# ekarpp/lumo

Measured on AMD Instinct MI355X. Metric: Mrays/s, higher is better.
Workload: dtype f64

## Files before the change

lumo_amd/csrc/device/dscene.h:

```cpp
#pragma once
#include <hip/hip_runtime.h>

#include "../../../include/lumo_amd.h"
#include "../common/lmath.h"
#include "../common/rng.h"
#include "../common/vec.h"
#include "../common/wbvh.h"

#ifndef LUMO_WHILE_WHILE
#define LUMO_WHILE_WHILE 1
#endif

namespace lumo {
namespace dev {

constexpr double DINF = __builtin_huge_val();
constexpr int NS = 4;
constexpr double Y_INTEGRAL = 106.856895;
constexpr double SVI = 253.819;

struct alignas(16) DKd {
    union {
        double point;
        struct {
            int32_t first, count;
        } leaf;
    } u;
    int32_t meta;
    int32_t left;
};
constexpr int TV_STRIDE = 10;

struct DBvh {
    double bmin[3], bmax[3];
    int32_t escape, first, count, left;
};

struct DObj {
    double bmin[3], bmax[3];
    int32_t kd_root, tri_base, item_base, tx;
    __device__ __forceinline__ int type() const { return tx & 3; }
    __device__ __forceinline__ int xform() const { return (tx >> 2) - 1; }
};
__device__ __forceinline__ double obj_radius(const DObj& o) { return o.bmin[0]; }
__device__ __forceinline__ double obj_radius(const lumo_object& o) { return o.radius; }

struct DScene {
    const double* vertices;
    const double* tv;
    const DKd* kdp;
    const double* normals;
    const double* uvs;
    const lumo_triangle* tris;
    const lumo_kd_node* kd;
    const int32_t* kd_items;
    const lumo_object* objs;
    const DObj* tobjs;
    const DBvh* onodes;
    const int32_t* oitems;
    const lumo_object* lights;
    const DObj* tlights;
    const DBvh* lnodes;
    const int32_t* litems;
    const double* alias_prob;
    const int32_t* alias_idx;
    const double* alias_pdf;
    const lumo_material* mats;
    const double* dense;
    const lumo_transform* xforms;
    const lumo_texture* textures;
    const lumo_spectrum* texels;
    const lumo_normal_map* nmaps;
    const double* ntexels;
    const lumo_perlin* perlin;
    int32_t n_onodes, n_lnodes, n_lights, n_shadow, stack_class, full, n_objs, pad_n;
    const char* hot;
    uint32_t hot_bytes;
    uint32_t off_onodes, off_oitems, off_lnodes, off_litems, off_objs, off_lights, off_kd_items, off_tris, off_xforms,
        off_tv, off_kdp, off_tobjs, off_tlights;
    const char* top;
    uint32_t top_bytes, off_top_onodes, off_top_lnodes, off_top_oitems, off_top_tobjs;
    int32_t top_onodes, top_lnodes;
    const DBvh* onodes_lds;
    const DBvh* lnodes_lds;
    int32_t n_onodes_lds, n_lnodes_lds;
    int32_t kst_n, kst_stride;
    int32_t* kst_node;
    double* kst_ts;
    int32_t kst_cfg;
    uint32_t top_shm;
    uint32_t off_top_kd;
    int32_t top_kd_lo, top_kd_n;
    const DKd* kd_lds;
    int32_t accel, w_oroot, w_lroot, wn_lds;
    double w_maxabs;
    const wbvh::Node* wnodes;
    const double* wtv;
    const int32_t* w_oblas;
    const int32_t* w_lblas;
    const wbvh::Node* wnodes_lds;
    uint32_t off_wnodes, off_wtv, off_woblas, off_wlblas;
    uint32_t off_top_wnodes;
    int32_t top_wnodes;
};

__device__ __forceinline__ DScene stage_top_lds(const DScene& sc, char* lds) {
    const uint4* src = reinterpret_cast<const uint4*>(sc.top);
    uint4* dst = reinterpret_cast<uint4*>(lds);
    for (uint32_t i = threadIdx.x; i < sc.top_bytes / 16; i += blockDim.x) dst[i] = src[i];
    __syncthreads();
    DScene v = sc;
    v.onodes_lds = reinterpret_cast<const DBvh*>(lds + sc.off_top_onodes);
    v.lnodes_lds = reinterpret_cast<const DBvh*>(lds + sc.off_top_lnodes);
    v.n_onodes_lds = sc.top_onodes;
    v.n_lnodes_lds = sc.top_lnodes;
    v.oitems = reinterpret_cast<const int32_t*>(lds + sc.off_top_oitems);
    v.tobjs = reinterpret_cast<const DObj*>(lds + sc.off_top_tobjs);
    v.kd_lds = reinterpret_cast<const DKd*>(lds + sc.off_top_kd);
    v.wnodes_lds = reinterpret_cast<const wbvh::Node*>(lds + sc.off_top_wnodes);
    v.wn_lds = sc.top_wnodes;
    v.kst_n = sc.kst_cfg;
    if (sc.kst_cfg > 0) {
        char* base = lds + ((sc.top_bytes + 15u) & ~15u);
        v.kst_stride = (int32_t)blockDim.x;
        v.kst_ts = reinterpret_cast<double*>(base) + threadIdx.x;
        v.kst_node = reinterpret_cast<int32_t*>(base + (size_t)8 * sc.kst_cfg * blockDim.x) + threadIdx.x;
    }
    return v;
}

__device__ __forceinline__ DScene stage_scene_lds(const DScene& sc, char* lds) {
    const uint4* src = reinterpret_cast<const uint4*>(sc.hot);
    uint4* dst = reinterpret_cast<uint4*>(lds);
    for (uint32_t i = threadIdx.x; i < sc.hot_bytes / 16; i += blockDim.x) dst[i] = src[i];
    __syncthreads();
    DScene v = sc;
    v.onodes = reinterpret_cast<const DBvh*>(lds + sc.off_onodes);
    v.oitems = reinterpret_cast<const int32_t*>(lds + sc.off_oitems);
    v.lnodes = reinterpret_cast<const DBvh*>(lds + sc.off_lnodes);
    v.litems = reinterpret_cast<const int32_t*>(lds + sc.off_litems);
    v.objs = reinterpret_cast<const lumo_object*>(lds + sc.off_objs);
    v.lights = reinterpret_cast<const lumo_object*>(lds + sc.off_lights);
    v.kd_items = reinterpret_cast<const int32_t*>(lds + sc.off_kd_items);
    v.tris = reinterpret_cast<const lumo_triangle*>(lds + sc.off_tris);
    v.xforms = reinterpret_cast<const lumo_transform*>(lds + sc.off_xforms);
    v.tv = reinterpret_cast<const double*>(lds + sc.off_tv);
    v.kdp = reinterpret_cast<const DKd*>(lds + sc.off_kdp);
    v.tobjs = reinterpret_cast<const DObj*>(lds + sc.off_tobjs);
    v.tlights = reinterpret_cast<const DObj*>(lds + sc.off_tlights);
    if (sc.accel) {
        v.wnodes = reinterpret_cast<const wbvh::Node*>(lds + sc.off_wnodes);
        v.wtv = reinterpret_cast<const double*>(lds + sc.off_wtv);
        v.w_oblas = reinterpret_cast<const int32_t*>(lds + sc.off_woblas);
        v.w_lblas = reinterpret_cast<const int32_t*>(lds + sc.off_wlblas);
    }
    return v;
}

struct Counters {
    uint32_t aabb, kd, tri;
    uint32_t resolved;
};

struct Ray {
    V3 o, d;
};
__device__ __forceinline__ Ray ray_new(V3 o, V3 d) { return Ray{o, normalize(d)}; }

struct RayX {
    V3 o, d, inv, wi, shear;
    int kz;
};
__device__ __forceinline__ V3 perm_kz(int kz, V3 v) {
    return kz == 0 ? V3{v.y, v.z, v.x} : (kz == 1 ? V3{v.z, v.x, v.y} : v);
}
__device__ __forceinline__ RayX rayx(const Ray& r) {
    RayX x;
    x.o = r.o;
    x.d = r.d;
    x.inv = 1.0 / r.d;
    const V3 wa = vabs(r.d);
    x.kz = (wa.x > wa.y && wa.x > wa.z) ? 0 : (wa.y > wa.z ? 1 : 2);
    x.wi = perm_kz(x.kz, r.d);
    x.shear = V3{-x.wi.x, -x.wi.y, 0.0} / x.wi.z;
    return x;
}

struct DColor {
    double s[NS];
};
__device__ __forceinline__ DColor cfill(double v) { return DColor{{v, v, v, v}}; }
__device__ __forceinline__ DColor operator+(DColor a, const DColor& b) {
#pragma unroll
    for (int i = 0; i < NS; ++i) a.s[i] = a.s[i] + b.s[i];
    return a;
}
__device__ __forceinline__ DColor operator-(DColor a, const DColor& b) {
#pragma unroll
    for (int i = 0; i < NS; ++i) a.s[i] = a.s[i] - b.s[i];
    return a;
}
__device__ __forceinline__ DColor operator*(DColor a, const DColor& b) {
#pragma unroll
    for (int i = 0; i < NS; ++i) a.s[i] = a.s[i] * b.s[i];
    return a;
}
__device__ __forceinline__ DColor operator*(DColor a, double v) {
#pragma unroll
    for (int i = 0; i < NS; ++i) a.s[i] = a.s[i] * v;
    return a;
}
__device__ __forceinline__ DColor operator*(double v, DColor a) {
#pragma unroll
    for (int i = 0; i < NS; ++i) a.s[i] = v * a.s[i];
    return a;
}
__device__ __forceinline__ DColor operator/(DColor a, const DColor& b) {
#pragma unroll
    for (int i = 0; i < NS; ++i) a.s[i] = b.s[i] == 0.0 ? 0.0 : a.s[i] / b.s[i];
    return a;
}
__device__ __forceinline__ DColor operator/(DColor a, double v) {
#pragma unroll
    for (int i = 0; i < NS; ++i) a.s[i] = v == 0.0 ? 0.0 : a.s[i] / v;
    return a;
}
__device__ __forceinline__ double cmean(const DColor& c) {
    double sum = 0.0;
#pragma unroll
    for (int i = 0; i < NS; ++i) sum += c.s[i];
    return sum / NS;
}

__device__ __forceinline__ double wl_sample_one(double v) {
    const double x = 0.85691062 - SVI * v * 0.0072;
    return 538.0 - 138.888889 * (0.5 * lm_log1p((2.0 * x) / (1.0 - x)));
}
__device__ __forceinline__ void wl_sample(double u, double* L) {
#pragma unroll
    for (int i = 0; i < NS; ++i) {
        double v = u + (double)i / (double)NS;
        v = v > 1.0 ? v - 1.0 : v;
        L[i] = wl_sample_one(v);
    }
}
__device__ __forceinline__ double wl_pdf_one(double l) {
    if (l < 360.0 || l > 830.0) return 0.0;
    const double c = lm_cosh(0.0072 * (l - 538.05));
    return 1.0 / (SVI * (c * c));
}
__device__ __forceinline__ DColor wl_pdf(const double* L) {
    DColor c;
#pragma unroll
    for (int i = 0; i < NS; ++i) c.s[i] = wl_pdf_one(L[i]);
    if (L[1] == 0.0 && L[2] == 0.0 && L[3] == 0.0) c.s[0] /= (double)NS;
    return c;
}
__device__ __forceinline__ double dense_one(const double* v, double lambda) {
    const double STEP = (830.0 - 360.0) / (95.0 - 1.0);
    const double fb = ceil((lambda - 360.0) / STEP);
    int b1 = fb > 0.0 ? (int)fmin(fb, 1e9) : 0;
    const double l1 = 360.0 + STEP * (double)b1;
    if (lambda == 0.0) return 0.0;
    if (b1 > 94) b1 = 94;
    if (lambda == l1) return v[b1];
    const int b0 = b1 == 0 ? 0 : b1 - 1;
    const double l0 = l1 - STEP;
    const double x1 = (lambda - l0) / STEP;
    const double x0 = 1.0 - x1;
    return v[b0] * x0 + v[b1] * x1;
}
__device__ __forceinline__ DColor dense_sample(const double* v, const double* L) {
    DColor c;
#pragma unroll
    for (int i = 0; i < NS; ++i) c.s[i] = dense_one(v, L[i]);
    return c;
}
__device__ __forceinline__ double spec_one(const lumo_spectrum& s, double lambda) {
    const float l = (float)lambda;
    const float x = s.c0 * l * l + s.c1 * l + s.c2;
    const float sig = 0.5f + x / (2.0f * sqrtf(1.0f + x * x));
    return (double)(s.scale * sig);
}
__device__ __forceinline__ DColor spec_sample(const lumo_spectrum& s, const double* L) {
    DColor c;
#pragma unroll
    for (int i = 0; i < NS; ++i) c.s[i] = spec_one(s, L[i]);
    return c;
}
__device__ __forceinline__ double luminance(const DScene& sc, const DColor& c, const double* L) {
    const DColor pdf = wl_pdf(L);
    return cmean(dense_sample(sc.dense + 95 * 1, L) * c / pdf) / Y_INTEGRAL;
}
__device__ __forceinline__ void dense_three(const double* v, double lambda, double* out) {
    const double STEP = (830.0 - 360.0) / (95.0 - 1.0);
    const double fb = ceil((lambda - 360.0) / STEP);
    int b1 = fb > 0.0 ? (int)fmin(fb, 1e9) : 0;
    const double l1 = 360.0 + STEP * (double)b1;
    if (lambda == 0.0) {
        out[0] = out[1] = out[2] = 0.0;
        return;
    }
    if (b1 > 94) b1 = 94;
    if (lambda == l1) {
        for (int k = 0; k < 3; ++k) out[k] = v[95 * k + b1];
        return;
    }
    const int b0 = b1 == 0 ? 0 : b1 - 1;
    const double l0 = l1 - STEP;
    const double x1 = (lambda - l0) / STEP;
    const double x0 = 1.0 - x1;
    for (int k = 0; k < 3; ++k) out[k] = v[95 * k + b0] * x0 + v[95 * k + b1] * x1;
}
__device__ __forceinline__ V3 color_xyz(const DScene& sc, const DColor& c, const double* L) {
    const DColor pdf = wl_pdf(L);
    DColor cx, cy, cz;
#pragma unroll
    for (int i = 0; i < NS; ++i) {
        double o[3];
        dense_three(sc.dense, L[i], o);
        cx.s[i] = o[0];
        cy.s[i] = o[1];
        cz.s[i] = o[2];
    }
    return V3{cmean(cx * c / pdf), cmean(cy * c / pdf), cmean(cz * c / pdf)} / Y_INTEGRAL;
}

__device__ __forceinline__ uint32_t sat_u32(double x) { return x != x || x <= 0.0 ? 0u : (x >= 4294967295.0 ? 4294967295u : (uint32_t)x); }
__device__ __forceinline__ uint64_t sat_u64(double x) {
    return x != x || x <= 0.0 ? 0ull : (x >= 18446744073709551615.0 ? ~0ull : (uint64_t)x);
}
struct Bilin {
    uint32_t i00, i10, i01, i11;
    double wx, wy;
};
__device__ __forceinline__ Bilin bilin(int32_t width, int32_t height, V2 uv) {
    const double w = (double)width, h = (double)height;
    const V2 xy{uv.x * w, (1.0 - uv.y) * h};
    const V2 xoyo{floor(xy.x - 0.5), floor(xy.y - 0.5)};
    const V2 x1y1{xy.x - xoyo.x - 0.5, xy.y - xoyo.y - 0.5};
    const uint32_t W = (uint32_t)width, H = (uint32_t)height;
    const uint32_t xo = sat_u32(xoyo.x + w) % W, yo = sat_u32(xoyo.y + h) % H;
    const uint32_t xi = (xo + 1) % W, yi = (yo + 1) % H;
    return Bilin{xo + yo * W, xi + yo * W, xo + yi * W, xi + yi * W, 1.0 - x1y1.x, 1.0 - x1y1.y};
}
__device__ __forceinline__ DColor image_at(const DScene& sc, const lumo_texture& T, V2 uv, const double* L) {
    const Bilin b = bilin(T.width, T.height, uv);
    const lumo_spectrum* tx = sc.texels + T.first;
    const DColor y0 = spec_sample(tx[b.i00], L) * b.wx + spec_sample(tx[b.i10], L) * (1.0 - b.wx);
    const DColor y1 = spec_sample(tx[b.i01], L) * b.wx + spec_sample(tx[b.i11], L) * (1.0 - b.wx);
    return y0 * b.wy + y1 * (1.0 - b.wy);
}
__device__ __forceinline__ V3 vfract(V3 v) { return V3{v.x - trunc(v.x), v.y - trunc(v.y), v.z - trunc(v.z)}; }
__device__ double perlin_noise(const lumo_perlin& P, V3 p) {
    const V3 w0 = vfract(p);
    const V3 fl{floor(p.x), floor(p.y), floor(p.z)};
    auto smoother = [](double x) { return ((6.0 * x - 15.0) * x + 10.0) * x * x * x; };
    const V3 w{smoother(w0.x), smoother(w0.y), smoother(w0.z)};
    const uint64_t bx = sat_u64(fl.x), by = sat_u64(fl.y), bz = sat_u64(fl.z);
    double acc = 0.0;
    for (int c = 0; c < 8; ++c) {
        const int i = c >> 2, j = (c >> 1) & 1, k = c & 1;
        const int hsh = P.perm[0][(bx + i) % 256] ^ P.perm[1][(by + j) % 256] ^ P.perm[2][(bz + k) % 256];
        const V3 nrm{P.lattice[hsh][0], P.lattice[hsh][1], P.lattice[hsh][2]};
        const V3 idx{(double)i, (double)j, (double)k};
        const V3 widx{2.0 * w.x * idx.x + 1.0 - w.x - idx.x, 2.0 * w.y * idx.y + 1.0 - w.y - idx.y,
                      2.0 * w.z * idx.z + 1.0 - w.z - idx.z};
        acc = acc + widx.x * widx.y * widx.z * dot(nrm, w - idx);
    }
    return acc;
}
__device__ __forceinline__ double powi6(double x) {
    const double x2 = x * x;
    return x2 * (x2 * x2);
}
__device__ DColor tex_at(const DScene& sc, int tex, const lumo_spectrum& solid, V2 uv, const double* L) {
    if (tex < 0) return spec_sample(solid, L);
    for (;;) {
        const lumo_texture& T = sc.textures[tex];
        if (T.kind == LUMO_TEX_SOLID) return spec_sample(T.spec, L);
        if (T.kind == LUMO_TEX_IMAGE) return image_at(sc, T, uv, L);
        if (T.kind == LUMO_TEX_CHECKERBOARD) {
            const V2 uvs{uv.x * T.scale, uv.y * T.scale};
            tex = sat_u64(floor(uvs.x) + floor(uvs.y)) % 2 == 0 ? T.first : T.second;
            continue;
        }
        if (T.kind == LUMO_TEX_MARBLE) {
            const lumo_perlin& P = sc.perlin[T.first];
            V3 p = 4.0 * V3{fabs(uv.x), fabs(uv.y), 0.0};
            double turb = 0.0;
            double gain = 1.0;
            for (int d = 0; d < 6; ++d) {
                turb = turb + gain * fabs(perlin_noise(P, p));
                p = 2.0 * p;
                gain = gain * 0.5;
            }
            const double scaled = 1.0 - powi6(0.5 + 0.5 * lm_sin(60.0 * uv.x + 20.0 * turb));
            return spec_sample(T.spec, L) * scaled;
        }
        const double cr = 2.0 * (uv.x - 0.75), ci = 2.0 * (uv.y - 0.5);
        double zr = 0.0, zi = 0.0;
        int depth = 0;
        while (depth < 256 && zr * zr + zi * zi < 4096.0) {
            const double nr = zr * zr - zi * zi + cr;
            const double ni = zr * zi + zi * zr + ci;
            zr = nr;
            zi = ni;
            depth++;
        }
        return cfill(depth == 256 ? 1.0 : 0.0);
    }
}
__device__ __forceinline__ V3 nmap_at(const DScene& sc, const lumo_normal_map& M, V2 uv) {
    const Bilin b = bilin(M.width, M.height, uv);
    const double* t = sc.ntexels + 3 * (size_t)M.first;
    auto n = [&](uint32_t i) { return V3{t[3 * i], t[3 * i + 1], t[3 * i + 2]}; };
    auto lerp = [](V3 n0, V3 n1, double v) { return normalize(n0 * v + n1 * (1.0 - v)); };
    return lerp(lerp(n(b.i00), n(b.i10), b.wx), lerp(n(b.i01), n(b.i11), b.wx), b.wy);
}

struct DHit {
    double t;
    int material;
    V3 p, err, ns, ng;
    V2 uv;
    bool backface;
};
__device__ __forceinline__ V2 wrap_uv(V2 uv) {
    const V2 f{rfract(uv.x), rfract(uv.y)};
    return V2{f.x < 0.0 ? f.x + 1.0 : f.x, f.y < 0.0 ? f.y + 1.0 : f.y};
}
__device__ __forceinline__ V3 ray_origin(const DHit& h, bool outside) {
    const V3 ne = h.ng;
    const double scaled_err = dot(h.err, vabs(ne));
    const V3 offset = outside ? ne * scaled_err : (-ne) * scaled_err;
    const V3 xi = h.p + offset;
    auto mv = [](double v, double n) { return n > 0.0 ? next_float(v) : (n < 0.0 ? previous_float(v) : v); };
    return V3{mv(xi.x, offset.x), mv(xi.y, offset.y), mv(xi.z, offset.z)};
}
__device__ __forceinline__ Ray spawn(const DHit& h, V3 wi) { return ray_new(ray_origin(h, dot(wi, h.ng) >= 0.0), wi); }

__device__ __forceinline__ V3 ld3(const double* p) { return V3{p[0], p[1], p[2]}; }

__device__ __forceinline__ void slab(const double* bmin, const double* bmax, V3 o, V3 inv, double& ts, double& te) {
    const V3 ro_min = (ld3(bmin) - o) * inv;
    const V3 ro_max = (ld3(bmax) - o) * inv;
    ts = max_element(vmin(ro_min, ro_max));
    te = min_element(vmax(ro_max, ro_min)) * (1.0 + 2.0 * gamma_n(3));
}

__device__ __forceinline__ double tri_hit_t_at(const double* tv, const RayX& r, double t_min, double t_max,
                                               Counters& C) {
    C.tri++;
    const V3 A = ld3(tv), B = ld3(tv + 3), Cv = ld3(tv + 6);
    const int kz = r.kz;
    const V3 wi = r.wi;
    V3 at = perm_kz(kz, A - r.o), bt = perm_kz(kz, B - r.o), ct = perm_kz(kz, Cv - r.o);
    const V3 shear = r.shear;
    at = at + shear * at.z;
    bt = bt + shear * bt.z;
    ct = ct + shear * ct.z;
    const V3 e = V3{bt.x * ct.y - bt.y * ct.x, ct.x * at.y - ct.y * at.x, at.x * bt.y - at.y * bt.x};
    if (min_element(e) < 0.0 && max_element(e) > 0.0) return DINF;
    const double det = dot(e, V3{1.0, 1.0, 1.0});
    if (det == 0.0) return DINF;
    const double t_scaled = dot(e, V3{at.z, bt.z, ct.z}) / wi.z;
    const bool b1 = det < 0.0 && (t_scaled > t_min * det || t_scaled < t_max * det);
    const bool b2 = det > 0.0 && (t_scaled < t_min * det || t_scaled > t_max * det);
    if (b1 || b2) return DINF;
    return t_scaled / det;
}
__device__ __forceinline__ double tri_hit_t(const DScene& sc, int ti, const RayX& r, double t_min, double t_max,
                                            Counters& C) {
    return tri_hit_t_at(sc.tv + TV_STRIDE * ti, r, t_min, t_max, C);
}

template <bool FULL>
__device__ bool tri_hit_geo_at(const DScene& sc, const double* tv, int ti, const RayX& r, double t_min, double t_max,
                               DHit& out) {
    const V3 A = ld3(tv), B = ld3(tv + 3), Cv = ld3(tv + 6);
    const int kz = r.kz;
    const V3 wi = r.wi;
    V3 at = perm_kz(kz, A - r.o), bt = perm_kz(kz, B - r.o), ct = perm_kz(kz, Cv - r.o);
    const V3 shear = r.shear;
    at = at + shear * at.z;
    bt = bt + shear * bt.z;
    ct = ct + shear * ct.z;
    const V3 e = V3{bt.x * ct.y - bt.y * ct.x, ct.x * at.y - ct.y * at.x, at.x * bt.y - at.y * bt.x};
    if (min_element(e) < 0.0 && max_element(e) > 0.0) return false;
    const double det = dot(e, V3{1.0, 1.0, 1.0});
    if (det == 0.0) return false;
    const double t_scaled = dot(e, V3{at.z, bt.z, ct.z}) / wi.z;
    const bool b1 = det < 0.0 && (t_scaled > t_min * det || t_scaled < t_max * det);
    const bool b2 = det > 0.0 && (t_scaled < t_min * det || t_scaled > t_max * det);
    if (b1 || b2) return false;
    const double t = t_scaled / det;
    const double max_z_v = rmax(rmax(fabs(at.z), fabs(bt.z)), fabs(ct.z));
    const double delta_z = gamma_n(3) * max_z_v;
    const double max_y_v = rmax(rmax(fabs(at.y), fabs(bt.y)), fabs(ct.y));
    const double delta_y = gamma_n(5) * (max_y_v + max_z_v);
    const double max_x_v = rmax(rmax(fabs(at.x), fabs(bt.x)), fabs(ct.x));
    const double delta_x = gamma_n(5) * (max_x_v + max_z_v);
    const double delta_e = 2.0 * (gamma_n(2) * max_x_v * max_y_v + delta_y * max_x_v + delta_x * max_y_v);
    const double max_e = rmax(rmax(fabs(e.x), fabs(e.y)), fabs(e.z));
    const double delta_t = 3.0 * (gamma_n(3) * max_e * max_z_v + delta_e * max_z_v + delta_z * max_e) / fabs(det);
    if (t <= t_min + delta_t) return false;
    out.t = t;
    if (!FULL) return true;
    const V3 bary = e / det;
    const lumo_triangle T = sc.tris[ti];
    const V3 ng = normalize(cross(B - A, Cv - A));
    V3 ns = ng;
    if (T.n[0] >= 0)
        ns = normalize(bary.x * ld3(sc.normals + 3 * T.n[0]) + bary.y * ld3(sc.normals + 3 * T.n[1]) +
                       bary.z * ld3(sc.normals + 3 * T.n[2]));
    const V3 xi = bary.x * A + bary.y * B + bary.z * Cv;
    V2 ta{0, 0}, tb{1, 0}, tc{1, 1};
    if (T.t[0] >= 0) {
        ta = V2{sc.uvs[2 * T.t[0]], sc.uvs[2 * T.t[0] + 1]};
        tb = V2{sc.uvs[2 * T.t[1]], sc.uvs[2 * T.t[1] + 1]};
        tc = V2{sc.uvs[2 * T.t[2]], sc.uvs[2 * T.t[2] + 1]};
    }
    const V2 uv = bary.x * ta + bary.y * tb + bary.z * tc;
    out.err = gamma_n(7) * V3{dot(vabs(bary * V3{A.x, B.x, Cv.x}), V3{1, 1, 1}),
                              dot(vabs(bary * V3{A.y, B.y, Cv.y}), V3{1, 1, 1}),
                              dot(vabs(bary * V3{A.z, B.z, Cv.z}), V3{1, 1, 1})};
    out.t = t;
    out.material = T.material;
    out.backface = dot(r.d, ng) > 0.0;
    out.p = xi;
    out.ns = ns;
    out.ng = ng;
    out.uv = wrap_uv(uv);
    return true;
}
template <bool FULL>
__device__ __forceinline__ bool tri_hit_geo(const DScene& sc, int ti, const RayX& r, double t_min, double t_max,
                                            DHit& out) {
    return tri_hit_geo_at<FULL>(sc, sc.tv + TV_STRIDE * ti, ti, r, t_min, t_max, out);
}

#ifdef LUMO_NOINLINE_KD
#define KD_INLINE __noinline__
#else
#define KD_INLINE
#endif
template <bool KL>
__device__ __forceinline__ void kst_push(const DScene& sc, int* st_node, double* st_ts, int k, int node, double t) {
    if (KL && k < sc.kst_n) {
        sc.kst_node[k * sc.kst_stride] = node;
        sc.kst_ts[k * sc.kst_stride] = t;
    } else {
        st_node[k] = node;
        st_ts[k] = t;
    }
}
template <bool KL>
__device__ __forceinline__ int kst_node(const DScene& sc, const int* st_node, int k) {
    return (KL && k < sc.kst_n) ? sc.kst_node[k * sc.kst_stride] : st_node[k];
}
template <bool KL>
__device__ __forceinline__ double kst_t(const DScene& sc, const double* st_ts, int k) {
    return (KL && k < sc.kst_n) ? sc.kst_ts[k * sc.kst_stride] : st_ts[k];
}

template <bool KL>
__device__ __forceinline__ DKd kd_at(const DScene& sc, int i) {
    if (KL) {
        const uint32_t k = (uint32_t)(i - sc.top_kd_lo);
        if (k < (uint32_t)sc.top_kd_n) return sc.kd_lds[k];
    }
    return sc.kdp[i];
}

template <bool GEO, int STK, bool KL = false>
__device__ KD_INLINE double kd_traverse(const DScene& sc, const DObj& ob, const RayX& r, double t_min, double t_max,
                              int* idx_out, Counters& C) {
    const double origin[3] = {r.o.x, r.o.y, r.o.z};
    const double inv_dir[3] = {r.inv.x, r.inv.y, r.inv.z};
    int st_node[STK];
    double st_ts[STK];
    int sp = 0;
    double t_hit = DINF;
    int curr = ob.kd_root;
    int idx = -1;
    double ts, te;
    C.aabb++;
    slab(ob.bmin, ob.bmax, r.o, r.inv, ts, te);
    double t_start = rmax(ts, t_min), t_end = rmin(te, t_max);
    const double t_end0 = t_end;
    for (;;) {
        if (t_hit < t_start) break;
        DKd node = kd_at<KL>(sc, curr);
#if LUMO_WHILE_WHILE
        while ((node.meta & 3) != 3) {
            C.kd++;
            const int ax = node.meta & 3;
            const double point = node.u.point;
            const int right = node.meta >> 2;
            const double t_split = (point - origin[ax]) * inv_dir[ax];
            const bool left_first = origin[ax] < point || (origin[ax] == point && inv_dir[ax] <= 0.0);
            const int first = left_first ? node.left : right;
            const int second = left_first ? right : node.left;
            if (t_split > t_end || t_split <= 0.0) {
                curr = first;
            } else if (t_split < t_start) {
                curr = second;
            } else {
                curr = first;
                kst_push<KL>(sc, st_node, st_ts, sp, second, t_split);
                t_end = t_split;
                sp++;
            }
            node = kd_at<KL>(sc, curr);
        }
#endif
        const int axis = node.meta & 3;
        if (axis == 3) {
            const int first = node.u.leaf.first, count = node.u.leaf.count;
            for (int k = 0; k < count; ++k) {
                const int i = sc.kd_items[ob.item_base + first + k];
                const double t = tri_hit_t(sc, ob.tri_base + i, r, t_min, t_end, C);
                if (GEO) {
                    if (t < t_end) {
                        t_end = t;
                        t_hit = t;
                        idx = i;
                    }
                } else if (t < t_end) {
                    return t;
                }
            }
            if (sp == 0) break;
            sp--;
            curr = kst_node<KL>(sc, st_node, sp);
            t_start = kst_t<KL>(sc, st_ts, sp);
            t_end = sp == 0 ? t_end0 : kst_t<KL>(sc, st_ts, sp - 1);
        } else {
            C.kd++;
            const int ax = axis;
            const double point = node.u.point;
            const int right = node.meta >> 2;
            const double t_split = (point - origin[ax]) * inv_dir[ax];
            const bool left_first = origin[ax] < point || (origin[ax] == point && inv_dir[ax] <= 0.0);
            const int first = left_first ? node.left : right;
            const int second = left_first ? right : node.left;
            if (t_split > t_end || t_split <= 0.0) {
                curr = first;
            } else if (t_split < t_start) {
                curr = second;
            } else {
                curr = first;
                kst_push<KL>(sc, st_node, st_ts, sp, second, t_split);
                t_end = t_split;
                sp++;
            }
        }
    }
    if (GEO) {
        *idx_out = idx;
        return idx < 0 ? DINF : t_hit;
    }
    return DINF;
}

__device__ __forceinline__ V3 xrow3(const double* m, int r, V3 v) { return V3{m[4 * r], m[4 * r + 1], m[4 * r + 2]}; }
__device__ __forceinline__ V3 xf_apply(const double* m, V3 v, double w) {
    const V4 in{v.x, v.y, v.z, w};
    const V4 o{dot4(V4{m[0], m[1], m[2], m[3]}, in), dot4(V4{m[4], m[5], m[6], m[7]}, in),
               dot4(V4{m[8], m[9], m[10], m[11]}, in), dot4(V4{m[12], m[13], m[14], m[15]}, in)};
    return project(o);
}
__device__ __forceinline__ V3 xf_abs_apply(const double* m, V3 v, double w) {
    const V4 in{v.x, v.y, v.z, w};
    auto r = [&](int i) { return V4{fabs(m[4 * i]), fabs(m[4 * i + 1]), fabs(m[4 * i + 2]), fabs(m[4 * i + 3])}; };
    return project(V4{dot4(r(0), in), dot4(r(1), in), dot4(r(2), in), dot4(r(3), in)});
}
__device__ __forceinline__ V3 m3_apply(const double* n, V3 v) {
    return V3{dot(V3{n[0], n[1], n[2]}, v), dot(V3{n[3], n[4], n[5]}, v), dot(V3{n[6], n[7], n[8]}, v)};
}
__device__ __forceinline__ RayX ray_local(const lumo_transform& T, const RayX& r) {
    return rayx(Ray{xf_apply(T.inv, r.o, 1.0), xf_apply(T.inv, r.d, 0.0)});
}
__device__ void instance_fix_hit(const lumo_transform& T, int material_override, DHit& h) {
    h.ns = normalize(m3_apply(T.nrm, h.ns));
    h.ng = normalize(m3_apply(T.nrm, h.ng));
    const V3 e3 = vabs(h.err), p3 = vabs(h.p);
    V3 err = gamma_n(3) * xf_abs_apply(T.m, p3, 1.0);
    if (!(e3.x == 0.0 && e3.y == 0.0 && e3.z == 0.0))
        err = err + (gamma_n(3) + 1.0) * xf_abs_apply(T.m, e3, 0.0);
    h.err = err;
    if (material_override >= 0) h.material = material_override;
    h.p = xf_apply(T.m, h.p, 1.0);
}

struct EF {
    double v, lo, hi;
};
__device__ __forceinline__ EF ef(double x) { return EF{x, x, x}; }
__device__ __forceinline__ EF ef_add(EF a, EF b) { return EF{a.v + b.v, previous_float(a.lo + b.lo), next_float(a.hi + b.hi)}; }
__device__ __forceinline__ EF ef_sub(EF a, EF b) { return EF{a.v - b.v, previous_float(a.lo - b.hi), next_float(a.hi - b.lo)}; }
__device__ __forceinline__ EF ef_mul(EF a, EF b) {
    const double p0 = a.lo * b.lo, p1 = a.lo * b.hi, p2 = a.hi * b.lo, p3 = a.hi * b.hi;
    return EF{a.v * b.v, previous_float(rmin(rmin(rmin(p0, p1), p2), p3)), next_float(rmax(rmax(rmax(p0, p1), p2), p3))};
}
__device__ __forceinline__ EF ef_div(EF a, EF b) {
    if (b.lo < 0.0 && b.hi > 0.0) return EF{a.v / b.v, -DINF, DINF};
    const double d0 = a.lo / b.lo, d1 = a.lo / b.hi, d2 = a.hi / b.lo, d3 = a.hi / b.hi;
    return EF{a.v / b.v, previous_float(rmin(rmin(rmin(d0, d1), d2), d3)), next_float(rmax(rmax(rmax(d0, d1), d2), d3))};
}
template <bool FULL, class OB>
__device__ bool sphere_hit(const OB& ob, const RayX& r, double t_min, double t_max, DHit& out) {
    const double radius = obj_radius(ob);
    const EF dx = ef(r.d.x), dy = ef(r.d.y), dz = ef(r.d.z), ox = ef(r.o.x), oy = ef(r.o.y), oz = ef(r.o.z);
    const EF radius2 = ef_mul(ef(radius), ef(radius));
    const EF a = ef_add(ef_add(ef_mul(dx, dx), ef_mul(dy, dy)), ef_mul(dz, dz));
    const EF b = ef_mul(ef(2.0), ef_add(ef_add(ef_mul(dx, ox), ef_mul(dy, oy)), ef_mul(dz, oz)));
    const EF c = ef_sub(ef_add(ef_add(ef_mul(ox, ox), ef_mul(oy, oy)), ef_mul(oz, oz)), radius2);
    const double disc = b.v * b.v - 4.0 * a.v * c.v;
    if (disc < 0.0) return false;
    const double sd = sqrt(disc);
    const EF root{sd, previous_float(sqrt(disc)), next_float(sqrt(disc))};
    const EF nb{-b.v, -b.lo, -b.hi};
    const EF a2 = ef_mul(ef(2.0), a);
    EF t0 = ef_div(ef_sub(nb, root), a2), t1 = ef_div(ef_add(nb, root), a2);
    if (t0.v > t1.v) {
        const EF tmp = t0;
        t0 = t1;
        t1 = tmp;
    }
    if (t0.hi >= t_max || t1.lo <= t_min) return false;
    EF t = t0;
    if (!(t0.lo > t_min)) {
        if (t1.hi >= t_max) return false;
        t = t1;
    }
    out.t = t.v;
    if constexpr (!FULL) {
        return true;
    } else {
    V3 xi = r.o + t.v * r.d;
    xi = xi * radius / length(xi);
    const V3 ni = xi / radius;
    out.err = gamma_n(5) * vabs(xi);
    out.material = ob.material;
    out.backface = dot(r.d, ni) > 0.0;
    out.p = xi;
    out.ns = ni;
    out.ng = ni;
    out.uv = wrap_uv(V2{(lm_atan2(-ni.z, ni.x) + PI) / (2.0 * PI), lm_acos(-ni.y) / PI});
    return true;
    }
}
__device__ double sphere_hit_t(const DObj& ob, const RayX& r, double t_min, double t_max) {
    const double a = dot(r.d, r.d);
    const double b = 2.0 * dot(r.d, r.o);
    const double radius = obj_radius(ob);
    const double c = dot(r.o, r.o) - radius * radius;
    const double disc = b * b - 4.0 * a * c;
    if (disc < 0.0) return DINF;
    const double root = sqrt(disc);
    double t0 = (-b - root) / (2.0 * a), t1 = (-b + root) / (2.0 * a);
    if (t0 > t1) {
        const double tmp = t0;
        t0 = t1;
        t1 = tmp;
    }
    if (t0 >= t_max || t1 <= t_min) return DINF;
    if (t0 > t_min) return t0;
    if (t1 >= t_max) return DINF;
    return t1;
}
constexpr int PRIM_SPHERE = -2;

template <int STK, int FX, bool KL = false>
__device__ __forceinline__ double shape_hit_t(const DScene& sc, const DObj& ob, const RayX& r, double t_min,
                                              double t_max, Counters& C) {
    if constexpr (FX) {
        if (ob.type() == LUMO_OBJ_TRIANGLE) return tri_hit_t(sc, ob.tri_base, r, t_min, t_max, C);
        if (ob.type() == LUMO_OBJ_SPHERE) return sphere_hit_t(ob, r, t_min, t_max);
    }
    return kd_traverse<false, STK, KL>(sc, ob, r, t_min, t_max, nullptr, C);
}
template <int STK, int FX, bool KL = false>
__device__ __forceinline__ double object_hit_t(const DScene& sc, const DObj& ob, const RayX& r, double t_min,
                                               double t_max, Counters& C) {
    if constexpr (FX) {
        if (ob.xform() >= 0)
            return shape_hit_t<STK, FX, KL>(sc, ob, ray_local(sc.xforms[ob.xform()], r), t_min, t_max, C);
    }
    return shape_hit_t<STK, FX, KL>(sc, ob, r, t_min, t_max, C);
}

template <int STK, int FX, bool KL = false>
__device__ __forceinline__ int shape_hit_tri(const DScene& sc, const DObj& ob, const RayX& r, double t_min,
                                             double t_max, Counters& C, DHit& out) {
    if constexpr (FX) {
        if (ob.type() == LUMO_OBJ_TRIANGLE) {
            C.tri++;
            return tri_hit_geo<false>(sc, ob.tri_base, r, t_min, t_max, out) ? ob.tri_base : -1;
        }
        if (ob.type() == LUMO_OBJ_SPHERE) return sphere_hit<false>(ob, r, t_min, t_max, out) ? PRIM_SPHERE : -1;
    }
    int idx = -1;
    kd_traverse<true, STK, KL>(sc, ob, r, t_min, t_max, &idx, C);
    if (idx < 0) return -1;
    C.tri++;
    if (!tri_hit_geo<false>(sc, ob.tri_base + idx, r, t_min, t_max, out)) return -1;
    return ob.tri_base + idx;
}
template <int STK, int FX, bool KL = false>
__device__ __forceinline__ int object_hit_tri(const DScene& sc, const DObj& ob, const RayX& r, double t_min,
                                              double t_max, Counters& C, DHit& out) {
    if constexpr (FX) {
        if (ob.xform() >= 0)
            return shape_hit_tri<STK, FX, KL>(sc, ob, ray_local(sc.xforms[ob.xform()], r), t_min, t_max, C, out);
    }
    return shape_hit_tri<STK, FX, KL>(sc, ob, r, t_min, t_max, C, out);
}

template <int FX>
__device__ void object_record(const DScene& sc, const lumo_object& ob, int tri, const RayX& r, DHit& h) {
    if constexpr (!FX) {
        tri_hit_geo<true>(sc, tri, r, 0.0, DINF, h);
        if (ob.type == LUMO_OBJ_RECTANGLE) h.uv = wrap_uv(V2{dot(ld3(ob.b0), h.p), dot(ld3(ob.b1), h.p)});
    } else {
        const RayX rl = ob.xform < 0 ? r : ray_local(sc.xforms[ob.xform], r);
        if (ob.type == LUMO_OBJ_SPHERE)
            sphere_hit<true>(ob, rl, 0.0, DINF, h);
        else
            tri_hit_geo<true>(sc, tri, rl, 0.0, DINF, h);
        if (ob.type == LUMO_OBJ_RECTANGLE) h.uv = wrap_uv(V2{dot(ld3(ob.b0), h.p), dot(ld3(ob.b1), h.p)});
        if (ob.xform >= 0) instance_fix_hit(sc.xforms[ob.xform], ob.material_override, h);
    }
}

template <bool GEO, int STK, int FX, bool TOP = false>
__device__ int bvh_traverse(const DScene& sc, const DBvh* nodes, int n_nodes, const int32_t* items,
                            const DObj* objs, const RayX& r, double t_min, double t_max, Counters& C,
                            double* t_found = nullptr, const DBvh* nodes_lds = nullptr, int n_lds = 0) {
    if (n_nodes == 0) return -1;
    const V3 inv_dir = r.inv;
    int curr = 0, idx = -1;
    double tt = t_max;
#if LUMO_WHILE_WHILE
    for (;;) {
        int count = 0;
        while (curr >= 0) {
            const DBvh& node = (TOP && curr < n_lds) ? nodes_lds[curr] : nodes[curr];
            double ts, te;
            C.aabb++;
            slab(node.bmin, node.bmax, r.o, inv_dir, ts, te);
            ts = rmax(ts, t_min);
            te = rmin(te, tt);
            if (ts <= te) {
                count = node.count;
                if (count == 0) {
                    curr = node.left;
                    continue;
                }
                break;
            }
            curr = node.escape;
        }
        if (curr < 0) break;
        const DBvh& node = (TOP && curr < n_lds) ? nodes_lds[curr] : nodes[curr];
        {
#else
    while (curr >= 0) {
        const DBvh& node = (TOP && curr < n_lds) ? nodes_lds[curr] : nodes[curr];
        double ts, te;
        C.aabb++;
        slab(node.bmin, node.bmax, r.o, inv_dir, ts, te);
        ts = rmax(ts, t_min);
        te = rmin(te, tt);
        if (ts <= te) {
            const int count = node.count;
            if (count == 0) {
                curr = node.left;
                continue;
            }
#endif
            for (int k = 0; k < count; ++k) {
                const int i = items[node.first + k];
                const double t = object_hit_t<STK, FX, TOP>(sc, objs[i], r, t_min, tt, C);
                if (GEO) {
                    if (t < tt) {
                        tt = t;
                        idx = i;
                    }
                } else if (t < tt) {
                    if (t_found) *t_found = t;
                    return i;
                }
            }
        }
        curr = node.escape;
    }
    return idx;
}

template <int STK, int FX, bool TOP = false>
__device__ __forceinline__ double bvh_hit_t(const DScene& sc, const DBvh* nodes, int n, const int32_t* items,
                                            const DObj* objs, const RayX& r, double t_min, double t_max,
                                            Counters& C, const DBvh* nodes_lds = nullptr, int n_lds = 0) {
    double t = DINF;
    const int idx = bvh_traverse<false, STK, FX, TOP>(sc, nodes, n, items, objs, r, t_min, t_max, C, &t, nodes_lds, n_lds);
    if (idx < 0) return DINF;
    return t;
}

struct HitRef {
    double t;
    int kind, obj, tri;
};

constexpr int WL_STK = wbvh::LIGHT_KD_STACK;
template <int STK>
constexpr int kd_stk() {
    return STK == 0 ? WL_STK : STK;
}

struct WHit {
    double t;
    int32_t tri, obj;
};

typedef __attribute__((address_space(1))) const uint4 g_uint4;
typedef __attribute__((address_space(3))) const uint4 l_uint4;
template <bool TOP>
__device__ __forceinline__ void wnode_load(const DScene& sc, int32_t i, wbvh::Node& nd) {
    uint4 v[8];
#if defined(__HIP_DEVICE_COMPILE__)
    if constexpr (TOP) {
        if (i < sc.wn_lds) {
            extern __shared__ __attribute__((aligned(16))) char lds_scene[];
            l_uint4* p = (l_uint4*)(lds_scene + sc.off_top_wnodes) + 8 * i;
#pragma unroll
            for (int k = 0; k < 8; ++k) v[k] = p[k];
        } else {
            g_uint4* p = (g_uint4*)sc.wnodes + 8 * (size_t)i;
#pragma unroll
            for (int k = 0; k < 8; ++k) v[k] = p[k];
        }
    } else
#endif
    {
        const uint4* p = reinterpret_cast<const uint4*>(sc.wnodes) + 8 * (size_t)i;
#pragma unroll
        for (int k = 0; k < 8; ++k) v[k] = p[k];
    }
    __builtin_memcpy(&nd, v, sizeof(nd));
}

struct RayW {
    float inv[3], clo[3], chi[3];
};
__device__ __forceinline__ float f32_up(double x) {
    const float f = (float)x;
    return (double)f < x ? nextafterf(f, __builtin_huge_valf()) : f;
}
__device__ __forceinline__ float f32_down(double x) {
    const float f = (float)x;
    return (double)f > x ? nextafterf(f, -__builtin_huge_valf()) : f;
}
__device__ __forceinline__ RayW rayw(const RayX& r, double M) {
    RayW w;
    const double o[3] = {r.o.x, r.o.y, r.o.z}, inv[3] = {r.inv.x, r.inv.y, r.inv.z};
#pragma unroll
    for (int a = 0; a < 3; ++a) {
        const double e = (M + fabs(o[a])) * fabs(inv[a]);
        if (e <= 1e36) {
            w.inv[a] = (float)inv[a];
            const double c = -(o[a] * inv[a]), E = e * 0x1p-23;
            const float lo = f32_down(c - E), hi = f32_up(c + E);
            w.clo[a] = inv[a] >= 0.0 ? lo : hi;
            w.chi[a] = inv[a] >= 0.0 ? hi : lo;
        } else {
            w.inv[a] = 0.0f;
            w.clo[a] = -__builtin_huge_valf();
            w.chi[a] = __builtin_huge_valf();
        }
    }
    return w;
}
constexpr float WREL_LO = 1.0f - 0x1p-21f, WREL_HI = 1.0f + 0x1p-21f;
#ifndef LUMO_WIDE_ANY_SORT
#define LUMO_WIDE_ANY_SORT 0
#endif
__device__ __forceinline__ bool wslab32(const wbvh::Node& nd, int i, const RayW& w, float tmin, float tmax, float& k) {
    float ts, te;
#pragma unroll
    for (int a = 0; a < 3; ++a) {
        const float t0 = fmaf(nd.lo[a][i], w.inv[a], w.clo[a]);
        const float t1 = fmaf(nd.hi[a][i], w.inv[a], w.chi[a]);
        const float lo = fminf(t0, t1), hi = fmaxf(t0, t1);
        ts = a == 0 ? lo : fmaxf(ts, lo);
        te = a == 0 ? hi : fminf(te, hi);
    }
    k = fmaxf(ts * WREL_LO, tmin);
    return k <= fminf(te * WREL_HI, tmax);
}

template <bool BY_T = true>
__device__ __forceinline__ void wcx(float& ka, int32_t& ra, bool& ha, float& kb, int32_t& rb, bool& hb) {
    const bool sw = hb && (!ha || (BY_T && ka > kb));
    const float k = sw ? kb : ka;
    kb = sw ? ka : kb;
    ka = k;
    const int32_t x = sw ? rb : ra;
    rb = sw ? ra : rb;
    ra = x;
    const bool f = sw ? hb : ha;
    hb = sw ? ha : hb;
    ha = f;
}

template <class OB>
__device__ __forceinline__ double wide_sphere_t(const OB& ob, const lumo_transform* xforms, RayX rw, double t_min,
                                                double t_max) {
    const RayX rl = ob.xform() >= 0 ? ray_local(xforms[ob.xform()], rw) : rw;
    DHit g;
    return sphere_hit<false>(ob, rl, t_min, t_max, g) ? g.t : DINF;
}
template <class OB>
__device__ __noinline__ double wide_sphere_t_call(const OB& ob, const lumo_transform* xforms, RayX rw, double t_min,
                                                  double t_max) {
    return wide_sphere_t(ob, xforms, rw, t_min, t_max);
}
__device__ __noinline__ RayX wide_inst_ray_call(const lumo_transform* xforms, int x, RayX rw) {
    return ray_local(xforms[x], rw);
}

#ifndef LUMO_WIDE_NOINLINE
#define LUMO_WIDE_NOINLINE 0
#endif
#if LUMO_WIDE_NOINLINE
#define WIDE_INLINE __noinline__
#else
#define WIDE_INLINE
#endif
template <bool ANY, int FX, bool TOP, bool OC = false>
__device__ WIDE_INLINE WHit wide_walk(const DScene& sc, int32_t root, const DObj* objs, const int32_t* blas,
                                      const RayX& rw, double t_min, double t_max, Counters& C,
                                      double t_stop = -DINF) {
    WHit h{t_max, -1, -1};
    if (root == wbvh::NONE) return h;
    int32_t st_ref[wbvh::STACK];
    float st_t[wbvh::STACK];
    int sp = 0;
    bool top_ok = false;
    int32_t top_ref = 0;
    float top_t = 0.0f;
    auto push = [&](int32_t ref, float t) {
        if (top_ok) {
            st_ref[sp] = top_ref;
            st_t[sp] = top_t;
            sp++;
        }
        top_ok = true;
        top_ref = ref;
        top_t = t;
    };
    RayX r = rw;
    const double wM = sc.w_maxabs;
    RayW w = rayw(rw, wM);
    const float tmin32 = f32_down(t_min);
    float tmax32 = f32_up(t_max);
    int inst = -1;
    int32_t cur = root;
    auto pop = [&]() -> bool {
        for (;;) {
            int32_t x;
            float xt;
            if (top_ok) {
                top_ok = false;
                x = top_ref;
                xt = top_t;
            } else {
                if (sp == 0) return false;
                --sp;
                x = st_ref[sp];
                xt = st_t[sp];
            }
            if (FX && x == wbvh::MARK) {
                r = rw;
                w = rayw(rw, wM);
                inst = -1;
                continue;
            }
            if (!ANY && (double)xt > h.t) continue;
            cur = x;
            return true;
        }
    };
    for (;;) {
        while (cur >= 0) {
            wbvh::Node nd;
            wnode_load<TOP>(sc, cur, nd);
            C.kd++;
            const int n = nd.n;
            C.aabb += n;
            float k0, k1, k2, k3;
            bool h0 = wslab32(nd, 0, w, tmin32, tmax32, k0);
            bool h1 = wslab32(nd, 1, w, tmin32, tmax32, k1);
            bool h2 = wslab32(nd, 2, w, tmin32, tmax32, k2) && n > 2;
            bool h3 = wslab32(nd, 3, w, tmin32, tmax32, k3) && n > 3;
            int32_t r0 = nd.ref[0], r1 = nd.ref[1], r2 = nd.ref[2], r3 = nd.ref[3];
            if (!ANY || LUMO_WIDE_ANY_SORT) {
                wcx(k0, r0, h0, k1, r1, h1);
                wcx(k2, r2, h2, k3, r3, h3);
                wcx(k0, r0, h0, k2, r2, h2);
                wcx(k1, r1, h1, k3, r3, h3);
                wcx(k1, r1, h1, k2, r2, h2);
            } else {
                wcx<false>(k0, r0, h0, k1, r1, h1);
                wcx<false>(k2, r2, h2, k3, r3, h3);
                wcx<false>(k0, r0, h0, k2, r2, h2);
                wcx<false>(k1, r1, h1, k3, r3, h3);
                wcx<false>(k1, r1, h1, k2, r2, h2);
            }
            if (!h0) {
                if (!pop()) return h;
                continue;
            }
            if (h3) push(r3, k3);
            if (h2) push(r2, k2);
            if (h1) push(r1, k1);
            cur = r0;
        }
        const int cnt = wbvh::leaf_count(cur), first = wbvh::leaf_first(cur);
        if (FX && cnt == 0) {
            const DObj& ob = objs[first];
            if (ob.type() == LUMO_OBJ_SPHERE) {
                const double gt = OC ? wide_sphere_t_call(ob, sc.xforms, rw, t_min, h.t)
                                     : wide_sphere_t(ob, sc.xforms, rw, t_min, h.t);
                if (gt < h.t) {
                    h = WHit{gt, PRIM_SPHERE, first};
                    if (ANY || h.t < t_stop) return h;
                    tmax32 = f32_up(h.t);
                }
            } else {
                push(wbvh::MARK, -__builtin_huge_valf());
                r = OC ? wide_inst_ray_call(sc.xforms, ob.xform(), rw) : ray_local(sc.xforms[ob.xform()], rw);
                w = rayw(r, wM);
                inst = first;
                cur = blas[first];
                continue;
            }
        } else {
            for (int k = 0; k < cnt; ++k) {
                const double* tv = sc.wtv + wbvh::TV * (size_t)(first + k);
                C.tri++;
                DHit g;
                if (tri_hit_geo_at<false>(sc, tv, -1, r, t_min, h.t, g) && g.t < h.t) {
                    const int32_t* ids = reinterpret_cast<const int32_t*>(tv + 9);
                    h = WHit{g.t, ids[0], inst >= 0 ? inst : ids[1]};
                    if (ANY || h.t < t_stop) return h;
                    tmax32 = f32_up(h.t);
                }
            }
        }
        if (!pop()) return h;
    }
}

template <int FX, bool TOP, bool OC = false>
__device__ HitRef wide_scene_hit(const DScene& sc, const RayX& r, Counters& C) {
    HitRef h{DINF, 0, -1, -1};
    const WHit o = wide_walk<false, FX, TOP, OC>(sc, sc.w_oroot, sc.tobjs, sc.w_oblas, r, 0.0, DINF, C);
    if (o.obj >= 0) h = HitRef{o.t, 1, o.obj, o.tri};
    const WHit l = wide_walk<false, FX, TOP, OC>(sc, sc.w_lroot, sc.tlights, sc.w_lblas, r, 0.0, h.t, C);
    if (l.obj >= 0) h = HitRef{l.t, 2, l.obj, l.tri};
    return h;
}

template <int FX, bool TOP, bool OC = false>
__device__ __forceinline__ bool wide_occluded(const DScene& sc, const RayX& r, double t_max, Counters& C) {
    if (wide_walk<true, FX, TOP, OC>(sc, sc.w_oroot, sc.tobjs, sc.w_oblas, r, 0.0, t_max, C).t < t_max) return true;
    return wide_walk<true, FX, TOP, OC>(sc, sc.w_lroot, sc.tlights, sc.w_lblas, r, 0.0, t_max, C).t < t_max;
}
template <int STK, int FX, bool TOP = false, bool OC = false>
__device__ HitRef scene_hit(const DScene& sc, const RayX& r, Counters& C) {
    if constexpr (STK == 0) {
        return wide_scene_hit<FX, TOP, OC>(sc, r, C);
    } else {
    HitRef h{DINF, 0, -1, -1};
    double t_max = DINF;
    DHit g;
    int oi = bvh_traverse<true, STK, FX, TOP>(sc, sc.onodes, sc.n_onodes, sc.oitems, sc.tobjs, r, 0.0, t_max, C, nullptr,
                                              sc.onodes_lds, sc.n_onodes_lds);
    if (oi >= 0) {
        const int tri = object_hit_tri<STK, FX, TOP>(sc, sc.tobjs[oi], r, 0.0, t_max, C, g);
        if (tri != -1) {
            h = HitRef{g.t, 1, oi, tri};
            t_max = g.t;
        }
    }
    const int li = bvh_traverse<true, STK, FX, TOP>(sc, sc.lnodes, sc.n_lnodes, sc.litems, sc.tlights, r, 0.0, t_max, C,
                                                    nullptr, sc.lnodes_lds, sc.n_lnodes_lds);
    if (li >= 0) {
        const int tri = object_hit_tri<STK, FX, TOP>(sc, sc.tlights[li], r, 0.0, t_max, C, g);
        if (tri != -1) h = HitRef{g.t, 2, li, tri};
    }
    return h;
    }
}

template <int FX>
__device__ __forceinline__ void hit_record(const DScene& sc, const HitRef& hr, const RayX& r, DHit& h) {
    const lumo_object& ob = hr.kind == 1 ? sc.objs[hr.obj] : sc.lights[hr.obj];
    object_record<FX>(sc, ob, hr.tri, r, h);
}

template <int STK, int FX, bool TOP = false>
__device__ bool scene_hit_light(const DScene& sc, const RayX& r, int light, DHit& lh, Counters& C) {
    if constexpr (STK == 0) {
        const int tri = object_hit_tri<kd_stk<STK>(), FX, false>(sc, sc.tlights[light], r, 0.0, DINF, C, lh);
        if (tri == -1 || wide_occluded<FX, TOP>(sc, r, lh.t - EPSILON, C)) return false;
        object_record<FX>(sc, sc.lights[light], tri, r, lh);
        return true;
    } else {
    const int tri = object_hit_tri<STK, FX, TOP>(sc, sc.tlights[light], r, 0.0, DINF, C, lh);
    if (tri == -1) return false;
    const double t_max = lh.t - EPSILON;
    if (bvh_hit_t<STK, FX, TOP>(sc, sc.onodes, sc.n_onodes, sc.oitems, sc.tobjs, r, 0.0, t_max, C, sc.onodes_lds,
                                sc.n_onodes_lds) < t_max)
        return false;
    if (bvh_hit_t<STK, FX, TOP>(sc, sc.lnodes, sc.n_lnodes, sc.litems, sc.tlights, r, 0.0, t_max, C, sc.lnodes_lds,
                                sc.n_lnodes_lds) < t_max)
        return false;
    object_record<FX>(sc, sc.lights[light], tri, r, lh);
    return true;
    }
}

template <int STK, int FX, bool TOP = false, bool OC = false>
__device__ int scene_hit_light_tri(const DScene& sc, const RayX& r, int light, Counters& C) {
    DHit lh;
    if constexpr (STK == 0) {
        const int tri = object_hit_tri<kd_stk<STK>(), FX, false>(sc, sc.tlights[light], r, 0.0, DINF, C, lh);
        if (tri == -1 || wide_occluded<FX, TOP, OC>(sc, r, lh.t - EPSILON, C)) return -1;
        return tri;
    } else {
    const int tri = object_hit_tri<STK, FX, TOP>(sc, sc.tlights[light], r, 0.0, DINF, C, lh);
    if (tri == -1) return -1;
    const double t_max = lh.t - EPSILON;
    if (bvh_hit_t<STK, FX, TOP>(sc, sc.onodes, sc.n_onodes, sc.oitems, sc.tobjs, r, 0.0, t_max, C, sc.onodes_lds,
                                sc.n_onodes_lds) < t_max)
        return -1;
    if (bvh_hit_t<STK, FX, TOP>(sc, sc.lnodes, sc.n_lnodes, sc.litems, sc.tlights, r, 0.0, t_max, C, sc.lnodes_lds,
                                sc.n_lnodes_lds) < t_max)
        return -1;
    return tri;
    }
}

struct Onb {
    V3 u, v, w;
};
__device__ __forceinline__ Onb onb_new(V3 w) {
    const double sgn = rsignum(w.z);
    const double a = -1.0 / (sgn + w.z);
    const double b = w.x * w.y * a;
    return Onb{V3{1.0 + sgn * w.x * w.x * a, sgn * b, -sgn * w.x}, V3{b, sgn + w.y * w.y * a, -w.y}, w};
}
__device__ __forceinline__ V3 onb_world(const Onb& o, V3 v) { return v.x * o.u + v.y * o.v + v.z * o.w; }
__device__ __forceinline__ V3 onb_local(const Onb& o, V3 v) { return V3{dot(v, o.u), dot(v, o.v), dot(v, o.w)}; }

struct Mf {
    double a;
    const double* eta;
    const double* k;
};
__device__ __forceinline__ Mf mf_of(const DScene& sc, const lumo_material& m) {
    return Mf{m.roughness, sc.dense + 95 * m.eta_idx, sc.dense + 95 * m.k_idx};
}
__device__ __forceinline__ bool mf_delta(const Mf& d) { return (d.a + d.a) / 2.0 < 1e-3; }
__device__ __forceinline__ bool mf_specular(const Mf& d) { return (d.a + d.a) / 2.0 < 0.01; }
__device__ __forceinline__ double sq(double x) { return x * x; }
__device__ __forceinline__ double pow5(double x) {
    const double x2 = x * x;
    const double x4 = x2 * x2;
    return x * x4;
}
__device__ __forceinline__ double clampd(double x, double lo, double hi) {
    if (x < lo) x = lo;
    if (x > hi) x = hi;
    return x;
}
__device__ __forceinline__ double schlick(double f0, double f90, double c) { return f0 + (f90 - f0) * pow5(1.0 - c); }
__device__ __forceinline__ void cs_phi(V3 w, double& cp, double& sp) {
    const double st = sqrt(rmax(1.0 - w.z * w.z, 0.0));
    cp = st == 0.0 ? 1.0 : clampd(w.x / st, -1.0, 1.0);
    sp = st == 0.0 ? 0.0 : clampd(w.y / st, -1.0, 1.0);
}
__device__ __forceinline__ double tan2_theta(V3 w) { return rmax(1.0 - w.z * w.z, 0.0) / (w.z * w.z); }
__device__ __forceinline__ bool is_inf(double x) { return x == DINF || x == -DINF; }
__device__ double mf_D(const Mf& d, V3 wh) {
    const double tan2 = tan2_theta(wh);
    if (is_inf(tan2)) return 0.0;
    const double cos4 = sq(wh.z * wh.z);
    if (cos4 < EPSILON * EPSILON) return 0.0;
    double cp, sp;
    cs_phi(wh, cp, sp);
    const double e = tan2 * (sq(cp / d.a) + sq(sp / d.a));
    return 1.0 / (PI * (d.a * d.a) * cos4 * sq(1.0 + e));
}
__device__ double mf_Lambda(const Mf& d, V3 w) {
    const double tan2 = tan2_theta(w);
    if (is_inf(tan2)) return 0.0;
    double cp, sp;
    cs_phi(w, cp, sp);
    const double alpha2 = sq(d.a * cp) + sq(d.a * sp);
    return (sqrt(rmax(1.0 + alpha2 * tan2, 0.0)) - 1.0) / 2.0;
}
__device__ __forceinline__ bool chi(V3 wo, V3 wh) { return rsignum(wh.z) * dot(wo, wh) * wo.z > EPSILON; }
__device__ __forceinline__ double mf_G(const Mf& d, V3 wo, V3 wi, V3 wh) {
    return chi(wo, wh) ? 1.0 / (1.0 + mf_Lambda(d, wo) + mf_Lambda(d, wi)) : 0.0;
}
__device__ __forceinline__ double mf_G1(const Mf& d, V3 wo, V3 wh) {
    return chi(wo, wh) ? 1.0 / (1.0 + mf_Lambda(d, wo)) : 0.0;
}
__device__ __forceinline__ double mf_normal_pdf(const Mf& d, V3 wh, V3 wo) {
    return rmax(mf_G1(d, wo, wh) * mf_D(d, wh) * fabs(dot(wh, wo)) / fabs(wo.z), 0.0);
}
__device__ V3 mf_sample_normal(const Mf& d, V3 wo, V2 u) {
    V3 ws = normalize(V3{wo.x * d.a, wo.y * d.a, wo.z});
    if (ws.z < 0.0) ws = -ws;
    const V3 t1 = (1.0 - ws.z < EPSILON) ? V3{1.0, 0.0, 0.0} : normalize(cross(ws, V3{0.0, 0.0, 1.0}));
    const V3 t2 = cross(t1, ws);
    const double r = sqrt(u.x);
    const double theta = 2.0 * PI * u.y;
    const double x = r * lm_cos(theta);
    const double h = sqrt(rmax(1.0 - x * x, 0.0));
    const double lerp = (1.0 + ws.z) / 2.0;
    const double y = (1.0 - lerp) * h + lerp * r * lm_sin(theta);
    const V3 wm{x, y, sqrt(rmax(1.0 - x * x - y * y, 0.0))};
    const V3 w = wm.x * t1 + wm.y * t2 + wm.z * ws;
    return normalize(V3{d.a * w.x, d.a * w.y, rmax(w.z, EPSILON)});
}
__device__ double fresnel_real(V3 wo, V3 wh, double eta) {
    double c = dot(wo, wh);
    const double e = c < 0.0 ? 1.0 / eta : eta;
    c = fabs(c);
    const double sin2_i = (1.0 - c * c) / (e * e);
    if (sin2_i >= 1.0) return 1.0;
    const double ci = sqrt(rmax(1.0 - sin2_i, 0.0));
    const double rpa = (e * c - ci) / (e * c + ci);
    const double rpe = (c - e * ci) / (c + e * ci);
    return (rpa * rpa + rpe * rpe) / 2.0;
}
struct Cx {
    double re, im;
};
__device__ __forceinline__ Cx cmul(Cx a, Cx b) { return Cx{a.re * b.re - a.im * b.im, a.re * b.im + a.im * b.re}; }
__device__ __forceinline__ double cnorm2(Cx a) { return a.re * a.re + a.im * a.im; }
__device__ __forceinline__ Cx cdivf(Cx a, double v) { return v == 0.0 ? Cx{NAN, NAN} : Cx{a.re / v, a.im / v}; }
__device__ __forceinline__ Cx cdiv(Cx a, Cx b) {
    if (b.re == 0.0 && b.im == 0.0) return Cx{NAN, NAN};
    return cdivf(cmul(a, Cx{b.re, -b.im}), cnorm2(b));
}
__device__ double fresnel_complex(V3 wo, V3 wh, double n, double k) {
    const Cx eta{n, k};
    const double c = clampd(dot(wo, wh), 0.0, 1.0);
    const double sin2_o = 1.0 - c * c;
    const Cx e2 = cmul(eta, eta);
    const Cx sin2_i = (e2.re == 0.0 && e2.im == 0.0)
                          ? Cx{NAN, NAN}
                          : cdivf(Cx{sin2_o * e2.re, sin2_o * -e2.im}, cnorm2(e2));
    const Cx z{1.0 - sin2_i.re, -sin2_i.im};
    const double rn = sqrt(sqrt(cnorm2(z)));
    const double half = lm_atan2(z.im, z.re) / 2.0;
    const Cx ci{rn * lm_cos(half), rn * lm_sin(half)};
    const Cx ec{eta.re * c, eta.im * c};
    const Cx rpa = cdiv(Cx{ec.re - ci.re, ec.im - ci.im}, Cx{ec.re + ci.re, ec.im + ci.im});
    const Cx eci = cmul(eta, ci);
    const Cx rpe = cdiv(Cx{c - eci.re, -eci.im}, Cx{c + eci.re, eci.im});
    return (cnorm2(rpa) + cnorm2(rpe)) / 2.0;
}
__device__ double fresnel_at(const Mf& d, V3 wo, V3 wh, double wl) {
    const double eta = dense_one(d.eta, wl);
    const double k = dense_one(d.k, wl);
    if (k == 0.0) return eta == 0.0 ? 0.0 : fresnel_real(wo, wh, eta);
    return fresnel_complex(wo, wh, eta, k);
}
__device__ __forceinline__ DColor fresnel(const Mf& d, V3 wo, V3 wh, const double* L) {
    DColor c;
    for (int i = 0; i < NS; ++i) c.s[i] = fresnel_at(d, wo, wh, L[i]);
    return c;
}
__device__ __forceinline__ bool reflect_about(V3 wo, V3 n, V3& wi) {
    const V3 w = 2.0 * (n * dot(wo, n) / length_squared(n)) - wo;
    if (!(w.z * wo.z > 0.0)) return false;
    wi = w;
    return true;
}
__device__ __forceinline__ bool refract_about(double eta, V3 wo, V3 no, V3& wi) {
    const bool flip = dot(no, wo) < 0.0;
    const double cos_to = flip ? -dot(no, wo) : dot(no, wo);
    const double er = flip ? 1.0 / eta : eta;
    const V3 n = flip ? -no : no;
    const double sin2_ti = (1.0 - cos_to * cos_to) / (er * er);
    if (sin2_ti >= 1.0) return false;
    const double cos_ti = sqrt(rmax(1.0 - sin2_ti, 0.0));
    const V3 w = -wo / er + (cos_to / er - cos_ti) * n;
    if (w.z * wo.z > 0.0) return false;
    wi = w;
    return true;
}
__device__ DColor reflect_coeff(const Mf& d, V3 wo, V3 wi, const double* L) {
    const V3 wh = normalize(wi + wo);
    return mf_D(d, wh) * fresnel(d, wo, wh, L) * mf_G(d, wo, wi, wh) / (4.0 * fabs(wo.z) * fabs(wi.z));
}
__device__ __forceinline__ double cos_hemisphere_pdf(V3 wo, V3 wi) {
    if (!(wo.z * wi.z > 0.0)) return 0.0;
    return wi.z > 0.0 ? wi.z / PI : 0.0;
}
__device__ __forceinline__ bool standard_kind(int k) {
    return k == LUMO_MAT_LAMBERTIAN || k == LUMO_MAT_MF_DIFFUSE || k == LUMO_MAT_MF_CONDUCTOR ||
           k == LUMO_MAT_MF_DIELECTRIC;
}

template <int FX>
__device__ __forceinline__ V3 mapped_ns(const DScene& sc, const lumo_material& m, const DHit& h) {
    if constexpr (FX >= 2) {
        if (m.normal_map >= 0) return normalize(onb_world(onb_new(h.ns), nmap_at(sc, sc.nmaps[m.normal_map], h.uv)));
    }
    return h.ns;
}
template <int FX>
__device__ __forceinline__ DColor mat_kd(const DScene& sc, const lumo_material& m, V2 uv, const double* L) {
    if constexpr (FX >= 2) return tex_at(sc, m.albedo_tex, m.albedo, uv, L);
    return spec_sample(m.albedo, L);
}
template <int FX>
__device__ __forceinline__ DColor mat_ks(const DScene& sc, const lumo_material& m, V2 uv, const double* L) {
    if constexpr (FX >= 2) return tex_at(sc, m.ks_tex, m.ks, uv, L);
    return spec_sample(m.ks, L);
}
template <int FX>
__device__ __forceinline__ DColor mat_tf(const DScene& sc, const lumo_material& m, V2 uv, const double* L) {
    if constexpr (FX >= 2) return tex_at(sc, m.tf_tex, m.tf, uv, L);
    return spec_sample(m.tf, L);
}

template <int FX>
__device__ bool bsdf_sample(const DScene& sc, const lumo_material& m, const DHit& h, V3 wo, double* L,
                            double rand_u, V2 rs, V3& wi) {
    if constexpr (!FX) {
        if (m.kind != LUMO_MAT_LAMBERTIAN || h.backface) return false;
        wi = onb_world(onb_new(h.ns), square_to_cos_hemisphere(rs));
        return true;
    }
    if (!standard_kind(m.kind)) return false;
    const Onb uvw = onb_new(mapped_ns<FX>(sc, m, h));
    const V3 o = onb_local(uvw, wo);
    if (h.backface && m.kind != LUMO_MAT_MF_DIELECTRIC) return false;
    V3 w;
    if (m.kind == LUMO_MAT_LAMBERTIAN) {
        w = square_to_cos_hemisphere(rs);
    } else {
        const Mf d = mf_of(sc, m);
        if (m.kind == LUMO_MAT_MF_DIFFUSE) {
            const double pr = schlick(0.04, 1.0, o.z);
            const double ps = 1.0 - pr;
            if (rand_u < pr / (pr + ps)) {
                if (!reflect_about(o, mf_delta(d) ? V3{0.0, 0.0, 1.0} : mf_sample_normal(d, o, rs), w)) return false;
            } else {
                w = square_to_cos_hemisphere(rs);
            }
        } else if (m.kind == LUMO_MAT_MF_CONDUCTOR) {
            if (mf_delta(d)) {
                w = V3{-o.x, -o.y, o.z};
            } else if (!reflect_about(o, mf_sample_normal(d, o, rs), w)) {
                return false;
            }
        } else {
            if (!(m.flags & LUMO_MATF_CONSTANT_ETA)) {
                L[1] = 0.0;
                L[2] = 0.0;
                L[3] = 0.0;
            }
            const double wl = L[0];
            const double eta = dense_one(d.eta, wl);
            const V3 wh = (eta == 1.0 || mf_delta(d)) ? V3{0.0, 0.0, 1.0} : mf_sample_normal(d, o, rs);
            const double pr = fresnel_at(d, o, wh, wl);
            const double pt = 1.0 - pr;
            const bool ok = rand_u < pr / (pr + pt) ? reflect_about(o, wh, w) : refract_about(eta, o, wh, w);
            if (!ok) return false;
        }
    }
    wi = onb_world(uvw, w);
    return true;
}
template <int FX>
__device__ double bsdf_pdf(const DScene& sc, const lumo_material& m, const DHit& h, V3 wo, V3 wi, const double* L) {
    if constexpr (!FX) {
        if (m.kind != LUMO_MAT_LAMBERTIAN) return 0.0;
        if (!(dot(h.ng, wi) * dot(h.ng, wo) >= 0.0)) return 0.0;
        const Onb uvw = onb_new(h.ns);
        return cos_hemisphere_pdf(onb_local(uvw, wo), onb_local(uvw, wi));
    }
    if (!standard_kind(m.kind)) return 0.0;
    const bool reflection = dot(h.ng, wi) * dot(h.ng, wo) >= 0.0;
    const Onb uvw = onb_new(mapped_ns<FX>(sc, m, h));
    const V3 o = onb_local(uvw, wo), i = onb_local(uvw, wi);
    if (!reflection && m.kind != LUMO_MAT_MF_DIELECTRIC) return 0.0;
    if (m.kind == LUMO_MAT_LAMBERTIAN) return cos_hemisphere_pdf(o, i);
    const Mf d = mf_of(sc, m);
    if (m.kind == LUMO_MAT_MF_DIFFUSE) {
        if (!(i.z * o.z > 0.0)) return 0.0;
        const V3 wh = normalize(o + i);
        const double pr = schlick(0.04, 1.0, o.z);
        const double ps = 1.0 - pr;
        const double p_ref = mf_delta(d) ? (1.0 - wh.z < EPSILON ? 1.0 : 0.0)
                                         : mf_normal_pdf(d, wh, o) / (4.0 * fabs(dot(o, wh)));
        return pr * p_ref + ps * cos_hemisphere_pdf(o, i);
    }
    if (m.kind == LUMO_MAT_MF_CONDUCTOR) {
        if (!(i.z * o.z > 0.0)) return 0.0;
        V3 wh = normalize(o + i);
        if (wh.z < 0.0) wh = -wh;
        if (mf_delta(d)) return 1.0 - wh.z < EPSILON ? 1.0 : 0.0;
        return mf_normal_pdf(d, wh, o) / (4.0 * fabs(dot(o, wh)));
    }
    const double wl = L[0];
    const double eta = dense_one(d.eta, wl);
    const double er = reflection ? 1.0 : (o.z < 0.0 ? 1.0 / eta : eta);
    V3 wh = eta == 1.0 ? V3{0.0, 0.0, 1.0} : normalize(o + i * er);
    if (wh.z < 0.0) wh = -wh;
    const double hwo = dot(o, wh), hwi = dot(i, wh);
    if (hwo == 0.0 || hwi == 0.0) return 0.0;
    if (hwo * o.z < 0.0 || hwi * i.z < 0.0) return 0.0;
    const double pr = fresnel_at(d, o, wh, wl);
    const double pt = 1.0 - pr;
    const bool flat = eta == 1.0 || mf_delta(d);
    if (reflection && flat) return 1.0 - wh.z < EPSILON ? pr / (pr + pt) : 0.0;
    if (reflection) return mf_normal_pdf(d, wh, o) / (4.0 * fabs(hwo)) * pr / (pr + pt);
    if (flat) return 1.0 - wh.z < EPSILON ? pt / (pr + pt) : 0.0;
    return mf_normal_pdf(d, wh, o) * fabs(hwi) / sq(hwi + hwo / er) * pt / (pr + pt);
}
template <int FX>
__device__ DColor bsdf_f(const DScene& sc, const lumo_material& m, const DHit& h, V3 wo, V3 wi, const double* L,
                         bool importance = false) {
    if constexpr (!FX) {
        if (m.kind != LUMO_MAT_LAMBERTIAN) return cfill(0.0);
        if (!(dot(h.ng, wi) * dot(h.ng, wo) >= 0.0) || h.backface) return cfill(0.0);
        return spec_sample(m.albedo, L) / PI;
    }
    if (!standard_kind(m.kind)) return cfill(0.0);
    const bool reflection = dot(h.ng, wi) * dot(h.ng, wo) >= 0.0;
    const Onb uvw = onb_new(mapped_ns<FX>(sc, m, h));
    const V3 o = onb_local(uvw, wo), i = onb_local(uvw, wi);
    if ((!reflection || h.backface) && m.kind != LUMO_MAT_MF_DIELECTRIC) return cfill(0.0);
    if (m.kind == LUMO_MAT_LAMBERTIAN) return spec_sample(m.albedo, L) / PI;
    const Mf d = mf_of(sc, m);
    if (m.kind == LUMO_MAT_MF_DIFFUSE) {
        const V3 wh = normalize(o + i);
        const DColor F = fresnel(d, o, wh, L);
        const DColor fr = mf_D(d, wh) * F * mf_G(d, o, i, wh) / (4.0 * fabs(o.z) * fabs(i.z));
        const double r2 = sq(d.a);
        const double fd90 = 0.5 * r2 + 2.0 * sq(wh.z) * r2;
        const double fd = schlick(1.0, fd90, o.z) * schlick(1.0, fd90, i.z) * (1.0 + r2 * (1.0 / 1.51 - 1.0));
        return fr * mat_ks<FX>(sc, m, h.uv, L) + mat_kd<FX>(sc, m, h.uv, L) * (cfill(1.0) - F) * fd / PI;
    }
    if (m.kind == LUMO_MAT_MF_CONDUCTOR) {
        const DColor ks = mat_ks<FX>(sc, m, h.uv, L);
        if (mf_delta(d)) return ks * fresnel(d, o, V3{0.0, 0.0, 1.0}, L) / fabs(i.z);
        return ks * reflect_coeff(d, o, i, L);
    }
    const double eta = dense_one(d.eta, L[0]);
    const double er = reflection ? 1.0 : (o.z < 0.0 ? 1.0 / eta : eta);
    const bool flat = eta == 1.0 || mf_delta(d);
    V3 wh = flat ? V3{0.0, 0.0, 1.0} : normalize(i * er + o);
    if (reflection) {
        const DColor ks = mat_ks<FX>(sc, m, h.uv, L);
        if (flat) return ks * fresnel(d, o, wh, L) / fabs(i.z);
        return ks * reflect_coeff(d, o, i, L);
    }
    const DColor F = fresnel(d, o, wh, L);
    if (wh.z < 0.0) wh = -wh;
    const double scale = importance ? 1.0 : er * er;
    const DColor tf = mat_tf<FX>(sc, m, h.uv, L);
    if (flat) return tf * (cfill(1.0) - F) / (scale * fabs(i.z));
    const double hwo = dot(wh, o), hwi = dot(wh, i);
    return tf * mf_D(d, wh) * (cfill(1.0) - F) * mf_G(d, o, i, wh) / scale * fabs(hwi * hwo / (i.z * o.z)) /
           sq(er * hwi + hwo);
}
__device__ __forceinline__ double shading_cosine(const lumo_material& m, V3 wi, V3 ns) {
    return standard_kind(m.kind) ? fabs(dot(ns, wi)) : 1.0;
}
template <int FX>
__device__ __forceinline__ bool mat_is_specular(const lumo_material& m) {
    if constexpr (!FX) return false;
    if (m.kind == LUMO_MAT_MF_DIELECTRIC) return true;
    if (m.kind == LUMO_MAT_MF_CONDUCTOR) return (m.roughness + m.roughness) / 2.0 < 0.01;
    return false;
}
template <int FX>
__device__ __forceinline__ bool mat_is_delta(const DScene& sc, const lumo_material& m, const double* L) {
    if constexpr (!FX) return false;
    if (m.kind == LUMO_MAT_MF_CONDUCTOR) return (m.roughness + m.roughness) / 2.0 < 1e-3;
    if (m.kind == LUMO_MAT_MF_DIELECTRIC)
        return (m.roughness + m.roughness) / 2.0 < 1e-3 || dense_one(sc.dense + 95 * m.eta_idx, L[0]) == 1.0;
    return false;
}
template <int FX>
__device__ __forceinline__ DColor emit(const DScene& sc, const lumo_material& m, const double* L, bool backface, V2 uv) {
    if (m.kind != LUMO_MAT_LIGHT) return cfill(0.0);
    if (!m.two_sided && backface) return cfill(0.0);
    return m.scale * mat_kd<FX>(sc, m, uv, L) * dense_sample(sc.dense + 95 * m.illuminant, L);
}

__device__ __forceinline__ int sample_light(const DScene& sc, double u) {
    const double x = u * (double)sc.n_lights;
    const double fl = floor(x);
    const int idx = fl > 0.0 ? (int)fl : 0;
    const double fr = rfract(x);
    return fr < sc.alias_prob[idx] ? idx : sc.alias_idx[idx];
}
__device__ __forceinline__ V3 shape_sample_on(const DScene& sc, const lumo_object& L, V2 rs) {
    if (L.type == LUMO_OBJ_TRIANGLE) {
        const double* tv = sc.tv + TV_STRIDE * L.tri_base;
        const V3 A = ld3(tv), B = ld3(tv + 3), Cv = ld3(tv + 6);
        const double gam = 1.0 - sqrt(1.0 - rs.x);
        const double beta = rs.y * (1.0 - gam);
        return A + beta * (B - A) + gam * (Cv - A);
    }
    return ld3(L.origin) + rs.x * ld3(L.b0) + rs.y * ld3(L.b1);
}
__device__ __forceinline__ double shape_pdf(const lumo_object& L, V3 xo, V3 wi, V3 xi, V3 ng) {
    if (L.type == LUMO_OBJ_SPHERE) {
        const double radius2 = L.radius * L.radius;
        const double d2 = length_squared(xo);
        if (!(d2 < radius2)) {
            const double cos_theta_max = sqrt(rmax(1.0 - radius2 / d2, 0.0));
            return 1.0 / (2.0 * PI * (1.0 - cos_theta_max));
        }
    }
    const double p_area = 1.0 / L.area;
    return p_area * distance_squared(xo, xi) / fabs(dot(ng, wi));
}
__device__ V3 shape_sample_towards(const DScene& sc, const lumo_object& L, V3 xo, V2 rs) {
    if (L.type != LUMO_OBJ_SPHERE) return normalize(shape_sample_on(sc, L, rs) - xo);
    const double d2 = length_squared(xo);
    const double radius2 = L.radius * L.radius;
    V3 xi;
    if (d2 < radius2) {
        const V3 p = L.radius * square_to_sphere(rs);
        xi = p * L.radius / length(p);
    } else {
        const Onb uvw = onb_new(-normalize(xo));
        const double d = sqrt(d2);
        const double cos_theta_max = sqrt(rmax(1.0 - radius2 / d2, 0.0));
        const double cos_theta = (1.0 - rs.x) + rs.x * cos_theta_max;
        const double sin_theta = sqrt(rmax(1.0 - cos_theta * cos_theta, 0.0));
        const double phi = 2.0 * PI * rs.y;
        const double ds = d * cos_theta - sqrt(rmax(radius2 - d2 * sin_theta * sin_theta, 0.0));
        const double cos_alpha = (d2 + radius2 - ds * ds) / (2.0 * d * L.radius);
        const double sin_alpha = sqrt(rmax(1.0 - cos_alpha * cos_alpha, 0.0));
        const V3 ngl{lm_cos(phi) * sin_alpha, lm_sin(phi) * sin_alpha, cos_alpha};
        xi = normalize(onb_world(uvw, -ngl)) * L.radius;
    }
    return normalize(xi - xo);
}
template <int FX>
__device__ V3 light_sample_towards(const DScene& sc, const lumo_object& L, V3 xo, V2 rs) {
    if constexpr (!FX) return normalize(ld3(L.origin) + rs.x * ld3(L.b0) + rs.y * ld3(L.b1) - xo);
    if (L.xform < 0) return shape_sample_towards(sc, L, xo, rs);
    const lumo_transform& T = sc.xforms[L.xform];
    const V3 xl = xf_apply(T.inv, xo, 1.0);
    const V3 dl = shape_sample_towards(sc, L, xl, rs);
    return normalize(xf_apply(T.m, dl, 0.0));
}
template <int FX>
__device__ double light_pdf(const DScene& sc, const lumo_object& L, const RayX& ri, V3 xi, V3 ng) {
    if constexpr (!FX) {
        const double p_area = 1.0 / L.area;
        return p_area * distance_squared(ri.o, xi) / fabs(dot(ng, ri.d));
    }
    if (L.xform < 0) return shape_pdf(L, ri.o, ri.d, xi, ng);
    const lumo_transform& T = sc.xforms[L.xform];
    const M3 N{V3{T.nrm[0], T.nrm[1], T.nrm[2]}, V3{T.nrm[3], T.nrm[4], T.nrm[5]}, V3{T.nrm[6], T.nrm[7], T.nrm[8]}};
    const M3 nti = m3_transpose(m3_inv(N));
    const V3 ng_l = normalize(m3_mul_vec(nti, ng));
    const V3 xi_l = xf_apply(T.inv, xi, 1.0);
    const V3 xo_l = xf_apply(T.inv, ri.o, 1.0);
    const V3 wi_l = normalize(xf_apply(T.inv, ri.d, 0.0));
    const double pdf_l = shape_pdf(L, xo_l, wi_l, xi_l, ng_l);
    const double height = fabs(dot(ng, xf_apply(T.m, ng_l, 0.0)));
    const M3 m3{V3{T.m[0], T.m[1], T.m[2]}, V3{T.m[4], T.m[5], T.m[6]}, V3{T.m[8], T.m[9], T.m[10]}};
    const double jacobian = fabs(m3_det(m3)) / height;
    const double sa_conv = distance_squared(ri.o, xi) * fabs(dot(wi_l, ng_l)) /
                           (distance_squared(xo_l, xi_l) * fabs(dot(ri.d, ng)));
    return pdf_l * sa_conv / jacobian;
}

}
}
```

lumo_amd/csrc/device/pt.h:

```cpp
#pragma once
#include "state.h"

namespace lumo {
namespace dev {

template <int STK, int LDS, int FX>
__global__ __launch_bounds__(LDS == 2 ? TOP_BLOCK : BLOCK, LUMO_WALK_WAVES) void k_closest(DScene sc0, Paths S,
                                                                                             const int32_t* queue,
                                                                                             uint32_t tail_below) {
    extern __shared__ __attribute__((aligned(16))) char lds_scene[];
    const uint32_t count = S.counts[CNT_CUR];
    if (count < tail_below) return;
    if (count <= blockIdx.x * blockDim.x) return;
    const DScene sc = LDS == 1 ? stage_scene_lds(sc0, lds_scene) : (LDS == 2 ? stage_top_lds(sc0, lds_scene) : sc0);
    Counters C{0, 0, 0};
    for (uint32_t q = blockIdx.x * blockDim.x + threadIdx.x; q < count; q += gridDim.x * blockDim.x) {
        const int s = queue[q];
        const RayX r = rayx(Ray{ldv3(S.ro, s), ldv3(S.rd, s)});
        const HitRef h = scene_hit<STK, FX, LDS == 2>(sc, r, C);
        S.hit_t[s] = h.t;
        S.hit_kind[s] = h.kind;
        S.hit_obj[s] = h.obj;
        S.hit_tri[s] = h.tri;
        S.queries[s] += 1;
    }
    flush_counters(C, S.tcount);
}


__device__ __forceinline__ V3 qv3(const QState& Q, int k, size_t q) { return V3{Q.D(k, q), Q.D(k + 1, q), Q.D(k + 2, q)}; }
__device__ __forceinline__ void qv3(const QState& Q, int k, size_t q, V3 v) {
    Q.D(k, q) = v.x;
    Q.D(k + 1, q) = v.y;
    Q.D(k + 2, q) = v.z;
}
__device__ __forceinline__ DColor qc(const QState& Q, int k, size_t q) {
    return DColor{{Q.D(k, q), Q.D(k + 1, q), Q.D(k + 2, q), Q.D(k + 3, q)}};
}
__device__ __forceinline__ void qc(const QState& Q, int k, size_t q, const DColor& c) {
    for (int i = 0; i < NS; ++i) Q.D(k + i, q) = c.s[i];
}

template <int STK, int LDS, int FX>
__global__ __launch_bounds__(LDS == 2 ? TOP_BLOCK : BLOCK, LUMO_CLOSEST_WAVES) void k_closest_q(DScene sc0, Paths S,
                                                                                               QState cur,
                                                                                               uint32_t skip_below) {
    extern __shared__ __attribute__((aligned(16))) char lds_scene[];
    const uint32_t count = S.counts[CNT_CUR];
    if (count < skip_below) return;
    if (count <= blockIdx.x * blockDim.x) return;
    const DScene sc = LDS == 1 ? stage_scene_lds(sc0, lds_scene) : (LDS == 2 ? stage_top_lds(sc0, lds_scene) : sc0);
    const HitQ hq = S.hq;
    Counters C{0, 0, 0};
    for (uint32_t w0 = wave_fetch(S.counts + CNT_FETCH_C); w0 < count; w0 = wave_fetch(S.counts + CNT_FETCH_C)) {
        const uint32_t q0 = w0 + lane_id();
        if (q0 >= count) continue;
        const uint32_t q = hq.perm ? hq.perm[q0] : q0;
        const RayX r = rayx(Ray{qv3(cur, QD_O, q), qv3(cur, QD_D, q)});
        const HitRef h = scene_hit<STK, FX, LDS == 2>(sc, r, C);
        hq.t[q] = h.t;
        hq.i[q] = h.kind;
        hq.i[hq.cap + q] = h.obj;
        hq.i[2 * hq.cap + q] = h.tri;
    }
    flush_counters(C, S.tcount);
}

__device__ __forceinline__ void put_record(const ShadowQ& Q, int b, size_t r, const Ray& ri, const DColor& f, double pdf,
                                           double cosv) {
    Q.D(b + 0, r) = ri.o.x;
    Q.D(b + 1, r) = ri.o.y;
    Q.D(b + 2, r) = ri.o.z;
    Q.D(b + 3, r) = ri.d.x;
    Q.D(b + 4, r) = ri.d.y;
    Q.D(b + 5, r) = ri.d.z;
    for (int k = 0; k < NS; ++k) Q.D(b + 6 + k, r) = f.s[k];
    Q.D(b + 10, r) = pdf;
    Q.D(b + 11, r) = cosv;
}

template <int FX>
__device__ __forceinline__ DColor record_f(const DScene& sc, const lumo_material& m, const DHit& ho, V3 wo, V3 w,
                                           const double* L, double pdf) {
    if (LUMO_SKIP_DEAD && pdf == 0.0) return cfill(0.0);
    return bsdf_f<FX>(sc, m, ho, wo, w, L);
}

template <int FX>
__device__ __forceinline__ bool nee_pair(const DScene& sc, const ShadowQ& sq, size_t r, const DHit& ho,
                                         const lumo_material& m, V3 wo, double* L, Xorshift& rng) {
    const int li = sample_light(sc, xs_float(rng));
    const lumo_object& Lo = sc.lights[li];
    sq.D(SD_PDFL, r) = sc.alias_pdf[li];
    sq.I(SI_LIGHT, r) = li;
    {
        const V2 rs = xs_vec2(rng);
        const V3 w = light_sample_towards<FX>(sc, Lo, ho.p, rs);
        const double pdf = bsdf_pdf<FX>(sc, m, ho, wo, w, L);
        put_record(sq, SD_LO, r, spawn(ho, w), record_f<FX>(sc, m, ho, wo, w, L, pdf), pdf, shading_cosine(m, w, ho.ns));
    }
    const double ru = xs_float(rng);
    const V2 rsq = xs_vec2(rng);
    V3 w;
    const bool ok = bsdf_sample<FX>(sc, m, ho, wo, L, ru, rsq, w);
    sq.I(SI_BVALID, r) = ok ? 1 : 0;
    if (ok) {
        const double pdf = bsdf_pdf<FX>(sc, m, ho, wo, w, L);
        put_record(sq, SD_BO, r, spawn(ho, w), record_f<FX>(sc, m, ho, wo, w, L, pdf), pdf, shading_cosine(m, w, ho.ns));
    }
    return ok;
}
constexpr int NEE_DRAWS = 6;

__device__ __forceinline__ int hit_material(const DScene& sc, int kind, int obj, int tri) {
    const lumo_object& ob = kind == 1 ? sc.objs[obj] : sc.lights[obj];
    int mat = ob.type == LUMO_OBJ_SPHERE ? ob.material : sc.tris[tri].material;
    if (ob.xform >= 0 && ob.material_override >= 0) mat = ob.material_override;
    return mat;
}
__device__ __forceinline__ uint32_t block_by_material(const DScene& sc, const HitQ& hq, uint32_t base, uint32_t count) {
    constexpr int NK = 8, NW = BLOCK / 64;
    __shared__ uint32_t cnt[NK][NW];
    __shared__ uint32_t order[BLOCK];
    const uint32_t q0 = base + threadIdx.x;
    const bool live = q0 < count;
    int k = 0;
    if (live) {
        const int kind = hq.i[q0];
        if (kind != 0) k = 1 + sc.mats[hit_material(sc, kind, hq.i[hq.cap + q0], hq.i[2 * hq.cap + q0])].kind % (NK - 1);
    }
    const int lane = lane_id(), w = threadIdx.x >> 6;
    uint32_t rank = 0;
#pragma unroll
    for (int b = 0; b < NK; ++b) {
        const uint64_t m = __ballot(live && k == b);
        if (live && k == b) rank = mbcnt64(m);
        if (lane == 0) cnt[b][w] = (uint32_t)__popcll(m);
    }
    __syncthreads();
    if (threadIdx.x == 0) {
        uint32_t t = 0;
        for (int b = 0; b < NK; ++b)
            for (int i = 0; i < (int)(blockDim.x >> 6); ++i) {
                const uint32_t c = cnt[b][i];
                cnt[b][i] = t;
                t += c;
            }
    }
    __syncthreads();
    const uint32_t rem = count > base ? count - base : 0u, n = rem < blockDim.x ? rem : blockDim.x;
    if (live) order[cnt[k][w] + rank] = q0;
    __syncthreads();
    const uint32_t q = threadIdx.x < n ? order[threadIdx.x] : count;
    __syncthreads();
    return q;
}

template <int FX, bool SPLIT>
__global__ __launch_bounds__(BLOCK, FX == 0 ? LUMO_SHADE_WAVES_LEAN : LUMO_SHADE_WAVES) void k_shade_q(DScene sc, Paths S, Tasks T, QState cur, QState nxt,
                                                                      uint32_t skip_below) {
    const uint32_t count = S.counts[CNT_CUR];
    if (count < skip_below) return;
    const int ns = sc.n_shadow;
    const HitQ hq = S.hq;
    const ShadowQ sq = S.sq;
    for (uint32_t base = blockIdx.x * blockDim.x; base < count; base += gridDim.x * blockDim.x) {
        const uint32_t q = block_by_material(sc, hq, base, count);
        const bool live = q < count;
        int slot = 0, task = 0, key = 0;
        uint32_t depth = 0, flags = 0, queries = 0;
        double L[NS] = {0.0, 0.0, 0.0, 0.0};
        DColor gathered = cfill(0.0), radiance = cfill(0.0);
        Xorshift rng{0, 0};
        Ray ro{V3{0, 0, 0}, V3{0, 0, 0}};
        DHit ho;
        lumo_material m{};
        V3 wo{0, 0, 0}, wi{0, 0, 0};
        bool sampled = false, resolve = false, alive = false;
        if (live) {
            slot = cur.I(QI_SLOT, q);
            task = cur.I(QI_TASK, q);
            depth = (uint32_t)cur.I(QI_DEPTH, q);
            flags = (uint32_t)cur.I(QI_FLAGS, q);
            queries = (uint32_t)cur.I(QI_QUERIES, q) + 1u;
            ro = Ray{qv3(cur, QD_O, q), qv3(cur, QD_D, q)};
            gathered = qc(cur, QD_G, q);
            radiance = qc(cur, QD_R, q);
            if (flags & QF_PENDING) radiance = radiance + qc(cur, QD_P, q);
            for (int i = 0; i < NS; ++i) L[i] = cur.D(QD_L + i, q);
            rng = Xorshift{cur.R(0, q), cur.R(1, q)};
            const int kind = hq.i[q];
            if (kind != 0) {
                const HitRef hr{hq.t[q], kind, hq.i[hq.cap + q], hq.i[2 * hq.cap + q]};
                hit_record<FX>(sc, hr, rayx(ro), ho);
                m = sc.mats[ho.material];
                wo = -ro.d;
                const double rand_u = xs_float(rng);
                const V2 rsq = xs_vec2(rng);
                sampled = bsdf_sample<FX>(sc, m, ho, wo, L, rand_u, rsq, wi);
                if (!sampled) {
                    if (flags & QF_SPECULAR) radiance = radiance + gathered * emit<FX>(sc, m, L, ho.backface, ho.uv);
                } else {
                    resolve = !mat_is_delta<FX>(sc, m, L);
                    if (resolve) key = m.kind % NB;
                }
            }
        }
        const uint32_t sp = key * sq.seg + block_slot_bucket(resolve, key, S.counts + CNT_BUCKET0);
        if (resolve) {
            uint32_t n_sh = 0;
            if constexpr (SPLIT) {
                for (int k = 0; k < 3; ++k) {
                    sq.HD(SH_P + k, sp) = (&ho.p.x)[k];
                    sq.HD(SH_E + k, sp) = (&ho.err.x)[k];
                    sq.HD(SH_NS + k, sp) = (&ho.ns.x)[k];
                    sq.HD(SH_NG + k, sp) = (&ho.ng.x)[k];
                    sq.HD(SH_WO + k, sp) = (&wo.x)[k];
                }
                sq.HD(SH_UV, sp) = ho.uv.x;
                sq.HD(SH_UV + 1, sp) = ho.uv.y;
                sq.HI(SHI_MAT, sp) = ho.material;
                sq.HI(SHI_BACK, sp) = ho.backface ? 1 : 0;
                for (int i = 0; i < ns; ++i) {
                    const size_t r = (size_t)i * sq.hcap + sp;
                    sq.HR(0, r) = rng.hi;
                    sq.HR(1, r) = rng.lo;
                    for (int k = 0; k < NEE_DRAWS; ++k) xs_step(rng);
                }
                n_sh = (uint32_t)ns;
            } else {
                for (int i = 0; i < ns; ++i)
                    n_sh += 1u + (nee_pair<FX>(sc, sq, (size_t)i * sq.hcap + sp, ho, m, wo, L, rng) ? 1u : 0u);
            }
            for (int k = 0; k < NS; ++k) {
                sq.HD(SH_G + k, sp) = gathered.s[k];
                sq.HD(SH_L + k, sp) = L[k];
            }
            sq.HI(SHI_SLOT, sp) = slot;
            queries += n_sh;
        }
        Ray rn = ro;
        if (sampled) {
            rn = spawn(ho, wi);
            const V3 wi2 = rn.d;
            const double p_scatter = bsdf_pdf<FX>(sc, m, ho, wo, wi2, L);
            if (!(p_scatter <= 0.0)) {
                const DColor bsdf = bsdf_f<FX>(sc, m, ho, wo, wi2, L);
                gathered = gathered * (bsdf * shading_cosine(m, wi2, ho.ns) / p_scatter);
                bool cont = true;
                if ((int)depth >= RR_DEPTH) {
                    const double lum = luminance(sc, gathered, L);
                    const double rr_prob = rmin(lum / T.delta[task], 1.0);
                    if (xs_float(rng) > rr_prob)
                        cont = false;
                    else
                        gathered = gathered / rr_prob;
                }
                alive = cont;
            }
        }
        const uint32_t np = block_slot(alive, S.counts + CNT_NEXT);
        if (alive) {
            qv3(nxt, QD_O, np, rn.o);
            qv3(nxt, QD_D, np, rn.d);
            qc(nxt, QD_G, np, gathered);
            qc(nxt, QD_R, np, radiance);
            for (int i = 0; i < NS; ++i) nxt.D(QD_L + i, np) = L[i];
            nxt.R(0, np) = rng.hi;
            nxt.R(1, np) = rng.lo;
            nxt.I(QI_SLOT, np) = slot;
            nxt.I(QI_TASK, np) = task;
            nxt.I(QI_DEPTH, np) = (int32_t)(depth + 1);
            nxt.I(QI_FLAGS, np) = (mat_is_specular<FX>(m) ? QF_SPECULAR : 0) | (resolve ? QF_PENDING : 0);
            nxt.I(QI_QUERIES, np) = (int32_t)queries;
        }
        if (resolve) {
            sq.HI(SHI_NEXT, sp) = alive ? (int32_t)np : -1;
            if (!alive)
                for (int k = 0; k < NS; ++k) sq.HD(SH_R + k, sp) = radiance.s[k];
        }
        if (live && !alive) {
            for (int i = 0; i < NS; ++i) S.lam[4 * slot + i] = L[i];
            S.depth[slot] = depth;
            S.queries[slot] = queries;
            if (!resolve) stc(S.rad, slot, radiance);
        }
    }
}

__device__ __forceinline__ RayX shadow_ray(const ShadowQ& Q, int b, size_t r) {
    return rayx(Ray{V3{Q.D(b, r), Q.D(b + 1, r), Q.D(b + 2, r)}, V3{Q.D(b + 3, r), Q.D(b + 4, r), Q.D(b + 5, r)}});
}
template <int FX>
__device__ __forceinline__ DColor shadow_mis(const DScene& sc, const ShadowQ& Q, int b, size_t r, bool li_mode,
                                             uint32_t p, const RayX& ri, int li, const DHit& hi) {
    DColor out = cfill(0.0);
    const lumo_object& Lo = sc.lights[li];
    const double p_lig = light_pdf<FX>(sc, Lo, ri, hi.p, hi.ng);
    const double p_sct = Q.D(b + 10, r);
    if (!(p_lig == 0.0 || p_sct == 0.0)) {
        double L[NS];
        for (int k = 0; k < NS; ++k) L[k] = Q.HD(SH_L + k, p);
        const double denom = p_lig * p_lig + p_sct * p_sct;
        const double weight = li_mode ? (p_lig * p_lig) / denom : (p_sct * p_sct) / denom;
        const double p_denom = li_mode ? p_lig : p_sct;
        const lumo_material hm = sc.mats[hi.material];
        const DColor f{{Q.D(b + 6, r), Q.D(b + 7, r), Q.D(b + 8, r), Q.D(b + 9, r)}};
        out = f * cfill(1.0) * emit<FX>(sc, hm, L, hi.backface, hi.uv) * Q.D(b + 11, r) * weight / p_denom;
    }
    return out;
}

template <int STK, int FX, bool TOP = false>
__device__ __forceinline__ DColor shadow_record_q(const DScene& sc, const ShadowQ& Q, int b, size_t r, bool li_mode,
                                                  uint32_t p, Counters& C, bool* visible = nullptr) {
#if LUMO_SKIP_DEAD
    if (Q.D(b + 10, r) == 0.0) {
        C.resolved++;
        return cfill(0.0);
    }
#endif
    const RayX ri = shadow_ray(Q, b, r);
    const int li = Q.I(SI_LIGHT, r);
    DHit hi;
    DColor out = cfill(0.0);
    if (scene_hit_light<STK, FX, TOP>(sc, ri, li, hi, C)) {
        if (visible) *visible = true;
        out = shadow_mis<FX>(sc, Q, b, r, li_mode, p, ri, li, hi);
    }
    return out;
}

__device__ __forceinline__ void deliver_nee(const Paths& S, const ShadowQ& Q, const QState& nxt, uint32_t p,
                                            const DColor& X) {
    const int next = Q.HI(SHI_NEXT, p);
    if (next >= 0) {
        qc(nxt, QD_P, (size_t)next, X);
    } else {
        const DColor R{{Q.HD(SH_R, p), Q.HD(SH_R + 1, p), Q.HD(SH_R + 2, p), Q.HD(SH_R + 3, p)}};
        stc(S.rad, Q.HI(SHI_SLOT, p), R + X);
    }
}

template <int STK, int LDS, int FX, bool NS1>
__global__ __launch_bounds__(LDS == 2 ? TOP_BLOCK : BLOCK, LUMO_SHADOW_WAVES) void k_shadow_q(DScene sc0, Paths S,
                                                                                              QState nxt) {
    extern __shared__ __attribute__((aligned(16))) char lds_scene[];
    const int ns = NS1 ? 1 : sc0.n_shadow;
    uint32_t count = 0;
    if (NS1) {
        for (int b = 0; b < NB; ++b) count += S.counts[CNT_BUCKET0 + b];
    } else {
        for (int k = 0; k < SHQ_CLASSES; ++k) count += S.counts[CNT_SHQ + k];
    }
    if (count <= blockIdx.x * blockDim.x) return;
    const DScene sc = LDS == 1 ? stage_scene_lds(sc0, lds_scene) : (LDS == 2 ? stage_top_lds(sc0, lds_scene) : sc0);
    const ShadowQ Q = S.sq;
    Counters C{0, 0, 0};
    if constexpr (!NS1) {
        for (uint32_t j = blockIdx.x * blockDim.x + threadIdx.x; j < count; j += gridDim.x * blockDim.x) {
            uint32_t k = j;
            int cl = 0;
            for (uint32_t c; k >= (c = S.counts[CNT_SHQ + cl]); ++cl) k -= c;
            const int32_t qv = Q.ql[(size_t)cl * Q.cap + k];
            const size_t r = (size_t)(qv >> 1);
            const int which = qv & 1;
            const int b = which ? SD_BO : SD_LO;
            const DColor x = shadow_record_q<STK, FX, LDS == 2>(sc, Q, b, r, which == 0, (uint32_t)(r % Q.hcap), C);
            for (int k = 0; k < NS; ++k) Q.D(b + 6 + k, r) = x.s[k];
        }
        flush_counters(C, S.tcount + TC_N);
        return;
    }
    for (uint32_t j = blockIdx.x * blockDim.x + threadIdx.x; j < count; j += gridDim.x * blockDim.x) {
        uint32_t lj = j;
        int bk = 0;
        for (;;) {
            const uint32_t c = S.counts[CNT_BUCKET0 + bk] * (uint32_t)ns;
            if (lj < c) break;
            lj -= c;
            bk++;
        }
        const size_t r = (size_t)bk * Q.seg + lj;
        const uint32_t p = (uint32_t)r;
#if LUMO_SHADOW_STATS
        uint32_t pc = 0;
        DColor a, b = cfill(0.0);
        for (int rec = 0; rec < 2; ++rec) {
            if (rec == 1 && !Q.I(SI_BVALID, r)) break;
            const uint32_t c0 = C.aabb + C.kd + C.tri, a0 = C.aabb;
            bool vis = false;
            const DColor x = shadow_record_q<STK, FX, LDS == 2>(sc, Q, rec ? SD_BO : SD_LO, r, rec == 0, p, C, &vis);
            if (rec) b = x; else a = x;
            const uint32_t cost = C.aabb + C.kd + C.tri - c0;
            pc += cost;
            const int env = sc.lights[Q.I(SI_LIGHT, r)].type == LUMO_OBJ_SPHERE;
            const int outc = vis ? 2 : (C.aabb == a0 ? 0 : 1);
            unsigned long long* st = S.tcount + TC_ALL + 18 * (rec * 6 + env * 3 + outc);
            atomicAdd(st, 1ull);
            atomicAdd(st + 1, (unsigned long long)cost);
            const int bin = 31 - __builtin_clz(cost | 1u);
            atomicAdd(st + 2 + (bin > 15 ? 15 : bin), 1ull);
        }
        {
            unsigned long long sum = pc, mx = pc;
            for (int off = 32; off > 0; off >>= 1) {
                sum += __shfl_xor(sum, off);
                const unsigned long long o = __shfl_xor(mx, off);
                mx = o > mx ? o : mx;
            }
            if (lane_id() == 0) {
                atomicAdd(S.tcount + TC_ALL + 216, sum);
                atomicAdd(S.tcount + TC_ALL + 217, 64ull * mx);
            }
        }
#else
        const DColor a = shadow_record_q<STK, FX, LDS == 2>(sc, Q, SD_LO, r, true, p, C);
        const DColor b = Q.I(SI_BVALID, r) ? shadow_record_q<STK, FX, LDS == 2>(sc, Q, SD_BO, r, false, p, C) : cfill(0.0);
#endif
        const DColor single = (cfill(0.0) + a + b) / Q.D(SD_PDFL, r);
        const DColor g{{Q.HD(SH_G, p), Q.HD(SH_G + 1, p), Q.HD(SH_G + 2, p), Q.HD(SH_G + 3, p)}};
        deliver_nee(S, Q, nxt, p, (cfill(0.0) + g * single) / 1.0);
    }
    flush_counters(C, S.tcount + TC_N);
    if (LUMO_SKIP_DEAD) flush_resolved(C.resolved, S.tcount + TC_RESOLVED);
}

template <int FX>
__global__ __launch_bounds__(BLOCK, LUMO_NEE_WAVES) void k_nee_gen(DScene sc, Paths S) {
    const int ns = sc.n_shadow;
    uint32_t pc[NB], paths = 0;
    for (int b = 0; b < NB; ++b) {
        pc[b] = S.counts[CNT_BUCKET0 + b];
        paths += pc[b];
    }
    const uint32_t count = paths * (uint32_t)ns;
    const ShadowQ sq = S.sq;
    uint32_t dead = 0;
    for (uint32_t j0 = blockIdx.x * blockDim.x; j0 < count; j0 += gridDim.x * blockDim.x) {
        const uint32_t j = j0 + threadIdx.x;
        size_t r = 0;
        bool live_l = false, live_b = false;
        int env = 0;
        if (j < count) {
        const int i = (int)(j / paths);
        uint32_t lj = j - (uint32_t)i * paths;
        int bk = 0;
        while (lj >= pc[bk]) lj -= pc[bk++];
        const uint32_t p = bk * sq.seg + lj;
        r = (size_t)i * sq.hcap + p;
        DHit ho;
        ho.t = 0.0;
        ho.p = V3{sq.HD(SH_P, p), sq.HD(SH_P + 1, p), sq.HD(SH_P + 2, p)};
        ho.err = V3{sq.HD(SH_E, p), sq.HD(SH_E + 1, p), sq.HD(SH_E + 2, p)};
        ho.ns = V3{sq.HD(SH_NS, p), sq.HD(SH_NS + 1, p), sq.HD(SH_NS + 2, p)};
        ho.ng = V3{sq.HD(SH_NG, p), sq.HD(SH_NG + 1, p), sq.HD(SH_NG + 2, p)};
        ho.uv = V2{sq.HD(SH_UV, p), sq.HD(SH_UV + 1, p)};
        ho.material = sq.HI(SHI_MAT, p);
        ho.backface = sq.HI(SHI_BACK, p) != 0;
        const V3 wo{sq.HD(SH_WO, p), sq.HD(SH_WO + 1, p), sq.HD(SH_WO + 2, p)};
        double L[NS];
        for (int k = 0; k < NS; ++k) L[k] = sq.HD(SH_L + k, p);
        Xorshift rng{sq.HR(0, r), sq.HR(1, r)};
        const lumo_material m = sc.mats[ho.material];
        const bool ok = nee_pair<FX>(sc, sq, r, ho, m, wo, L, rng);
        live_l = !LUMO_SKIP_DEAD || sq.D(SD_LPS, r) != 0.0;
        live_b = ok && (!LUMO_SKIP_DEAD || sq.D(SD_BPS, r) != 0.0);
        dead += (live_l ? 0u : 1u) + (ok && !live_b ? 1u : 0u);
        env = sc.lights[sq.I(SI_LIGHT, r)].type == LUMO_OBJ_SPHERE ? 1 : 0;
        }
        const int kl = env, kb = 2 + env;
        const uint32_t pl = block_slot_bucket(live_l, kl, S.counts + CNT_SHQ);
        const uint32_t pb = block_slot_bucket(live_b, kb, S.counts + CNT_SHQ);
        if (live_l) sq.ql[(size_t)kl * sq.cap + pl] = (int32_t)(2 * r);
        if (live_b) sq.ql[(size_t)kb * sq.cap + pb] = (int32_t)(2 * r + 1);
    }
    if (LUMO_SKIP_DEAD) flush_resolved(dead, S.tcount + TC_RESOLVED);
}

#ifdef LUMO_MAIN_TU
__global__ __launch_bounds__(BLOCK) void k_nee_fold(Paths S, QState nxt, int ns) {
    uint32_t bc[NB], count = 0;
    for (int b = 0; b < NB; ++b) {
        bc[b] = S.counts[CNT_BUCKET0 + b];
        count += bc[b];
    }
    const ShadowQ Q = S.sq;
    for (uint32_t j = blockIdx.x * blockDim.x + threadIdx.x; j < count; j += gridDim.x * blockDim.x) {
        uint32_t lj = j;
        int bk = 0;
        while (lj >= bc[bk]) lj -= bc[bk++];
        const uint32_t p = bk * Q.seg + lj;
        const DColor g{{Q.HD(SH_G, p), Q.HD(SH_G + 1, p), Q.HD(SH_G + 2, p), Q.HD(SH_G + 3, p)}};
        DColor acc = cfill(0.0);
        int32_t nb = 0;
        for (int i = 0; i < ns; ++i) {
            const size_t r = (size_t)i * Q.hcap + p;
            const bool bv = Q.I(SI_BVALID, r) != 0;
            const bool live_l = !LUMO_SKIP_DEAD || Q.D(SD_LPS, r) != 0.0;
            const bool live_b = bv && (!LUMO_SKIP_DEAD || Q.D(SD_BPS, r) != 0.0);
            const DColor a = live_l ? DColor{{Q.D(SD_LF, r), Q.D(SD_LF + 1, r), Q.D(SD_LF + 2, r), Q.D(SD_LF + 3, r)}}
                                    : cfill(0.0);
            const DColor b = live_b ? DColor{{Q.D(SD_BF, r), Q.D(SD_BF + 1, r), Q.D(SD_BF + 2, r), Q.D(SD_BF + 3, r)}}
                                    : cfill(0.0);
            const DColor single = (cfill(0.0) + a + b) / Q.D(SD_PDFL, r);
            acc = acc + g * single;
            nb += bv ? 1 : 0;
        }
        deliver_nee(S, Q, nxt, p, acc / (double)ns);
        const int next = Q.HI(SHI_NEXT, p);
        if (next >= 0)
            nxt.I(QI_QUERIES, (size_t)next) += nb;
        else
            S.queries[Q.HI(SHI_SLOT, p)] += (uint32_t)nb;
    }
}
#endif


struct NeeRec {
    Ray ray;
    DColor f;
    double pdf, cosv;
};
template <int FX>
__device__ __forceinline__ NeeRec nee_record(const DScene& sc, const lumo_material& m, const DHit& ho, V3 wo, V3 w,
                                             const double* L) {
    const double pdf = bsdf_pdf<FX>(sc, m, ho, wo, w, L);
    return NeeRec{spawn(ho, w), record_f<FX>(sc, m, ho, wo, w, L, pdf), pdf, shading_cosine(m, w, ho.ns)};
}

template <int STK, int FX>
__device__ __forceinline__ DColor shadow_record_r(const DScene& sc, const NeeRec& R, int li, bool li_mode,
                                                  const double* L, Counters& C) {
#if LUMO_SKIP_DEAD
    if (R.pdf == 0.0) {
        C.resolved++;
        return cfill(0.0);
    }
#endif
    const RayX ri = rayx(R.ray);
    DHit hi;
    DColor out = cfill(0.0);
    if (scene_hit_light<STK, FX>(sc, ri, li, hi, C)) {
        const lumo_object& Lo = sc.lights[li];
        const double p_lig = light_pdf<FX>(sc, Lo, ri, hi.p, hi.ng);
        const double p_sct = R.pdf;
        if (!(p_lig == 0.0 || p_sct == 0.0)) {
            const double denom = p_lig * p_lig + p_sct * p_sct;
            const double weight = li_mode ? (p_lig * p_lig) / denom : (p_sct * p_sct) / denom;
            const double p_denom = li_mode ? p_lig : p_sct;
            const lumo_material hm = sc.mats[hi.material];
            out = R.f * cfill(1.0) * emit<FX>(sc, hm, L, hi.backface, hi.uv) * R.cosv * weight / p_denom;
        }
    }
    return out;
}

template <int STK, int FX>
__device__ __forceinline__ DColor shadow_record_lds(const DScene& sc, const Ray& ray, double pdf, const double* fc,
                                                    int cos_at, uint32_t nt, int li, bool li_mode, const double* L,
                                                    Counters& C) {
#if LUMO_SKIP_DEAD
    if (pdf == 0.0) {
        C.resolved++;
        return cfill(0.0);
    }
#endif
    const RayX ri = rayx(ray);
    DHit hi;
    DColor out = cfill(0.0);
    if (scene_hit_light<STK, FX>(sc, ri, li, hi, C)) {
        const lumo_object& Lo = sc.lights[li];
        const double p_lig = light_pdf<FX>(sc, Lo, ri, hi.p, hi.ng);
        const double p_sct = pdf;
        if (!(p_lig == 0.0 || p_sct == 0.0)) {
            const double denom = p_lig * p_lig + p_sct * p_sct;
            const double weight = li_mode ? (p_lig * p_lig) / denom : (p_sct * p_sct) / denom;
            const double p_denom = li_mode ? p_lig : p_sct;
            const lumo_material hm = sc.mats[hi.material];
            const DColor f{{fc[0], fc[nt], fc[2 * nt], fc[3 * nt]}};
            out = f * cfill(1.0) * emit<FX>(sc, hm, L, hi.backface, hi.uv) * fc[cos_at * nt] * weight / p_denom;
        }
    }
    return out;
}

#ifndef LUMO_PARK_NEE
#define LUMO_PARK_NEE 1
#endif
constexpr int PARK_DOUBLES = LUMO_PARK_NEE ? 12 + 9 : 12;

struct PathReg {
    Ray ro;
    DColor g, rad;
    double L[NS];
    Xorshift rng;
    int32_t slot, task;
    uint32_t depth, flags, queries;
};

template <int STK, int FX>
__device__ __forceinline__ bool bounce_path(const DScene& sc, const double* delta, PathReg& P, Counters& Cc,
                                            Counters& Cs) {
    const RayX rx = rayx(P.ro);
    const HitRef hr = scene_hit<STK, FX>(sc, rx, Cc);
    P.queries += 1u;
    if (hr.kind == 0) return false;
    DHit ho;
    hit_record<FX>(sc, hr, rx, ho);
    const lumo_material m = sc.mats[ho.material];
    const V3 wo = -P.ro.d;
    const double rand_u = xs_float(P.rng);
    const V2 rsq = xs_vec2(P.rng);
    V3 wi;
    if (!bsdf_sample<FX>(sc, m, ho, wo, P.L, rand_u, rsq, wi)) {
        if (P.flags & QF_SPECULAR) P.rad = P.rad + P.g * emit<FX>(sc, m, P.L, ho.backface, ho.uv);
        return false;
    }
    const bool resolve = !mat_is_delta<FX>(sc, m, P.L);
    NeeRec RL, RB;
    int li = 0;
    double pdf_light = 1.0;
    bool ok = false;
    const DColor g_nee = P.g;
    if (resolve) {
        li = sample_light(sc, xs_float(P.rng));
        pdf_light = sc.alias_pdf[li];
        const V2 rs = xs_vec2(P.rng);
        RL = nee_record<FX>(sc, m, ho, wo, light_sample_towards<FX>(sc, sc.lights[li], ho.p, rs), P.L);
        const double ru = xs_float(P.rng);
        const V2 rsq2 = xs_vec2(P.rng);
        V3 wb;
        ok = bsdf_sample<FX>(sc, m, ho, wo, P.L, ru, rsq2, wb);
        if (ok) RB = nee_record<FX>(sc, m, ho, wo, wb, P.L);
        P.queries += 1u + (ok ? 1u : 0u);
    }
    const Ray rn = spawn(ho, wi);
    const double p_scatter = bsdf_pdf<FX>(sc, m, ho, wo, rn.d, P.L);
    bool alive = false;
    if (!(p_scatter <= 0.0)) {
        const DColor bsdf = bsdf_f<FX>(sc, m, ho, wo, rn.d, P.L);
        P.g = P.g * (bsdf * shading_cosine(m, rn.d, ho.ns) / p_scatter);
        alive = true;
        if ((int)P.depth >= RR_DEPTH) {
            const double lum = luminance(sc, P.g, P.L);
            const double rr_prob = rmin(lum / delta[P.task], 1.0);
            if (xs_float(P.rng) > rr_prob)
                alive = false;
            else
                P.g = P.g / rr_prob;
        }
    }
    if (resolve) {
        DColor a = cfill(0.0), b = cfill(0.0);
#pragma unroll 1
        for (int k = 0; k < (ok ? 2 : 1); ++k) {
            const NeeRec Rk = k == 0 ? RL : RB;
            const DColor x = shadow_record_r<STK, FX>(sc, Rk, li, k == 0, P.L, Cs);
            if (k == 0)
                a = x;
            else
                b = x;
        }
        const DColor single = (cfill(0.0) + a + b) / pdf_light;
        P.rad = P.rad + (cfill(0.0) + g_nee * single) / 1.0;
    }
    if (alive) {
        P.ro = rn;
        P.flags = mat_is_specular<FX>(m) ? QF_SPECULAR : 0u;
        P.depth += 1u;
    }
    return alive;
}

__device__ __forceinline__ PathReg load_path(const QState& cur, uint32_t q) {
    PathReg P;
    P.slot = cur.I(QI_SLOT, q);
    P.task = cur.I(QI_TASK, q);
    P.depth = (uint32_t)cur.I(QI_DEPTH, q);
    P.flags = (uint32_t)cur.I(QI_FLAGS, q);
    P.queries = (uint32_t)cur.I(QI_QUERIES, q);
    P.ro = Ray{qv3(cur, QD_O, q), qv3(cur, QD_D, q)};
    P.g = qc(cur, QD_G, q);
    P.rad = qc(cur, QD_R, q);
    if (P.flags & QF_PENDING) P.rad = P.rad + qc(cur, QD_P, q);
    for (int i = 0; i < NS; ++i) P.L[i] = cur.D(QD_L + i, q);
    P.rng = Xorshift{cur.R(0, q), cur.R(1, q)};
    return P;
}
__device__ __forceinline__ void store_final(const Paths& S, const PathReg& P) {
    for (int i = 0; i < NS; ++i) S.lam[4 * P.slot + i] = P.L[i];
    S.depth[P.slot] = P.depth;
    S.queries[P.slot] = P.queries;
    stc(S.rad, P.slot, P.rad);
}

#ifndef LUMO_BOUNCE_ARGPTR
#define LUMO_BOUNCE_ARGPTR 0
#endif
template <int STK>
__global__ void k_put_args(BounceArgs a, BounceArgs* out) {
    if (threadIdx.x == 0) *out = a;
}
template <int STK, bool LDS, int FX, bool TAIL>
__global__ __launch_bounds__(BLOCK, TAIL ? 2 : LUMO_BOUNCE_WAVES) void k_bounce_q(
#if LUMO_BOUNCE_ARGPTR
    const BounceArgs* __restrict__ A, uint32_t tail_below, int dyn) {
    const DScene& sc0 = A->sc;
    const Paths& S = A->S;
    const Tasks& T = A->T;
    const QState& cur = A->cur;
    const QState& nxt = A->nxt;
#else
    DScene sc0, Paths S, Tasks T, QState cur, QState nxt, uint32_t tail_below, int dyn) {
#endif
    extern __shared__ __attribute__((aligned(16))) char lds_scene[];
    const uint32_t count = S.counts[CNT_CUR];
    if ((count < tail_below) != TAIL) return;
    if (count <= blockIdx.x * blockDim.x) return;
    const DScene sc = LDS ? stage_scene_lds(sc0, lds_scene) : sc0;
    Counters Cc{0, 0, 0, 0}, Cs{0, 0, 0, 0};
    if constexpr (TAIL) {
        uint32_t tailq = 0;
        for (uint32_t w0 = wave_fetch(S.counts + CNT_FETCH_T); w0 < count; w0 = wave_fetch(S.counts + CNT_FETCH_T)) {
            const uint32_t q = w0 + lane_id();
            if (q >= count) continue;
            PathReg P = load_path(cur, q);
            while (bounce_path<STK, FX>(sc, T.delta, P, Cc, Cs)) tailq++;
            store_final(S, P);
        }
        flush_resolved(tailq, S.tcount + TC_TAILQ);
    } else {
        __shared__ uint32_t first_base;
        double* rb_lds = reinterpret_cast<double*>(lds_scene + (LDS ? (sc0.hot_bytes + 15u) / 16u * 16u : 0u));
        const uint32_t nt = blockDim.x;
        uint32_t base = blockIdx.x * blockDim.x;
#if LUMO_PHASE_CLOCKS
        uint64_t ph[6] = {0, 0, 0, 0, 0, 0}, tc0 = clock64(), tc1 = 0;
        uint64_t lanes[4] = {0, 0, 0, 0};
#define LUMO_PHASE(k) (tc1 = clock64(), ph[k] += tc1 - tc0, tc0 = tc1)
#else
#define LUMO_PHASE(k) ((void)0)
#endif
        if (dyn) {
            if (threadIdx.x == 0) first_base = atomicAdd(S.counts + CNT_FETCH_B, (uint32_t)blockDim.x);
            __syncthreads();
            base = first_base;
        }
        while (base < count) {
            const uint32_t q = base + threadIdx.x;
            const bool live = q < count;
            LUMO_PHASE(3);
            HitRef hr{DINF, 0, -1, -1};
            if (live) hr = scene_hit<STK, FX>(sc, rayx(Ray{qv3(cur, QD_O, q), qv3(cur, QD_D, q)}), Cc);
            LUMO_PHASE(0);
            PathReg P{};
            bool resolve = false, alive = false, ok = false;
            NeeRec RL;
            int li = 0;
            double pdf_light = 1.0;
            DColor g_nee = cfill(0.0);
            Ray rn{V3{0, 0, 0}, V3{0, 0, 0}};
            if (live) {
                P = load_path(cur, q);
                P.queries += 1u;
                if (hr.kind != 0) {
                    DHit ho;
                    hit_record<FX>(sc, hr, rayx(P.ro), ho);
                    const lumo_material m = sc.mats[ho.material];
                    const V3 wo = -P.ro.d;
                    const double rand_u = xs_float(P.rng);
                    const V2 rsq = xs_vec2(P.rng);
                    V3 wi;
                    if (!bsdf_sample<FX>(sc, m, ho, wo, P.L, rand_u, rsq, wi)) {
                        if (P.flags & QF_SPECULAR) P.rad = P.rad + P.g * emit<FX>(sc, m, P.L, ho.backface, ho.uv);
                    } else {
                        resolve = !mat_is_delta<FX>(sc, m, P.L);
                        g_nee = P.g;
                        if (resolve) {
                            li = sample_light(sc, xs_float(P.rng));
                            pdf_light = sc.alias_pdf[li];
                            const V2 rs = xs_vec2(P.rng);
                            RL = nee_record<FX>(sc, m, ho, wo, light_sample_towards<FX>(sc, sc.lights[li], ho.p, rs),
                                                P.L);
                            if (LUMO_PARK_NEE) {
                                double* rl = rb_lds + 12 * nt + threadIdx.x;
                                for (int k = 0; k < 4; ++k) rl[k * nt] = RL.f.s[k];
                                rl[4 * nt] = RL.cosv;
                                for (int k = 0; k < 4; ++k) rl[(5 + k) * nt] = g_nee.s[k];
                            }
                            const double ru = xs_float(P.rng);
                            const V2 rsq2 = xs_vec2(P.rng);
                            V3 wb;
                            ok = bsdf_sample<FX>(sc, m, ho, wo, P.L, ru, rsq2, wb);
                            if (ok) {
                                const NeeRec RB = nee_record<FX>(sc, m, ho, wo, wb, P.L);
                                const double v[12] = {RB.ray.o.x, RB.ray.o.y, RB.ray.o.z, RB.ray.d.x, RB.ray.d.y,
                                                      RB.ray.d.z, RB.f.s[0], RB.f.s[1], RB.f.s[2], RB.f.s[3],
                                                      RB.pdf, RB.cosv};
#pragma unroll
                                for (int k = 0; k < 12; ++k) rb_lds[k * nt + threadIdx.x] = v[k];
                            }
                            P.queries += 1u + (ok ? 1u : 0u);
                        }
                        rn = spawn(ho, wi);
                        const double p_scatter = bsdf_pdf<FX>(sc, m, ho, wo, rn.d, P.L);
                        if (!(p_scatter <= 0.0)) {
                            const DColor bsdf = bsdf_f<FX>(sc, m, ho, wo, rn.d, P.L);
                            P.g = P.g * (bsdf * shading_cosine(m, rn.d, ho.ns) / p_scatter);
                            alive = true;
                            if ((int)P.depth >= RR_DEPTH) {
                                const double lum = luminance(sc, P.g, P.L);
                                const double rr_prob = rmin(lum / T.delta[P.task], 1.0);
                                if (xs_float(P.rng) > rr_prob)
                                    alive = false;
                                else
                                    P.g = P.g / rr_prob;
                            }
                        }
                        P.flags = mat_is_specular<FX>(m) ? QF_SPECULAR : 0u;
                    }
                }
            }
            LUMO_PHASE(1);
            uint32_t next_base = 0;
            const uint32_t np = dyn ? block_slot_fetch(alive, S.counts + CNT_NEXT, S.counts + CNT_FETCH_B, &next_base)
                                    : block_slot(alive, S.counts + CNT_NEXT);
            LUMO_PHASE(5);
            if (alive) {
                qv3(nxt, QD_O, np, rn.o);
                qv3(nxt, QD_D, np, rn.d);
                qc(nxt, QD_G, np, P.g);
                qc(nxt, QD_R, np, P.rad);
                for (int i = 0; i < NS; ++i) nxt.D(QD_L + i, np) = P.L[i];
                nxt.R(0, np) = P.rng.hi;
                nxt.R(1, np) = P.rng.lo;
                nxt.I(QI_SLOT, np) = P.slot;
                nxt.I(QI_TASK, np) = P.task;
                nxt.I(QI_DEPTH, np) = (int32_t)(P.depth + 1u);
                nxt.I(QI_FLAGS, np) = (int32_t)(P.flags | (resolve ? (uint32_t)QF_PENDING : 0u));
                nxt.I(QI_QUERIES, np) = (int32_t)P.queries;
            } else if (live) {
                for (int i = 0; i < NS; ++i) S.lam[4 * P.slot + i] = P.L[i];
                S.depth[P.slot] = P.depth;
                S.queries[P.slot] = P.queries;
                stc(S.rad, P.slot, P.rad);
            }
            LUMO_PHASE(4);
#if LUMO_PHASE_CLOCKS
            lanes[0] += 1;
            lanes[1] += (uint64_t)__popcll(__ballot(live));
            lanes[2] += (uint64_t)__popcll(__ballot(resolve));
            lanes[3] += (uint64_t)__popcll(__ballot(resolve && ok));
#endif
            if (resolve) {
#if LUMO_PARK_NEE
                const double* rl = rb_lds + 12 * nt + threadIdx.x;
                const DColor a = shadow_record_lds<STK, FX>(sc, RL.ray, RL.pdf, rl, 4, nt, li, true, P.L, Cs);
                DColor b = cfill(0.0);
                if (ok) {
                    const double* v = rb_lds + threadIdx.x;
                    const Ray rbr{V3{v[0], v[nt], v[2 * nt]}, V3{v[3 * nt], v[4 * nt], v[5 * nt]}};
                    b = shadow_record_lds<STK, FX>(sc, rbr, v[10 * nt], v + 6 * nt, 5, nt, li, false, P.L, Cs);
                }
                const double pdf_l = sc.alias_pdf[li];
                const DColor g_n{{rl[5 * nt], rl[6 * nt], rl[7 * nt], rl[8 * nt]}};
                const DColor single = (cfill(0.0) + a + b) / pdf_l;
                const DColor X = (cfill(0.0) + g_n * single) / 1.0;
#else
                const DColor a = shadow_record_r<STK, FX>(sc, RL, li, true, P.L, Cs);
                DColor b = cfill(0.0);
                if (ok) {
                    NeeRec RB;
                    const double* v = rb_lds + threadIdx.x;
                    RB.ray = Ray{V3{v[0], v[nt], v[2 * nt]}, V3{v[3 * nt], v[4 * nt], v[5 * nt]}};
                    RB.f = DColor{{v[6 * nt], v[7 * nt], v[8 * nt], v[9 * nt]}};
                    RB.pdf = v[10 * nt];
                    RB.cosv = v[11 * nt];
                    b = shadow_record_r<STK, FX>(sc, RB, li, false, P.L, Cs);
                }
                const DColor single = (cfill(0.0) + a + b) / pdf_light;
                const DColor X = (cfill(0.0) + g_nee * single) / 1.0;
#endif
                if (alive)
                    qc(nxt, QD_P, np, X);
                else
                    stc(S.rad, P.slot, ldc(S.rad, P.slot) + X);
            }
            LUMO_PHASE(2);
            base = dyn ? next_base : base + gridDim.x * blockDim.x;
        }
#if LUMO_PHASE_CLOCKS
        if (lane_id() == 0) {
            for (int k = 0; k < 5; ++k) atomicAdd(S.tcount + TC_ALL + k, (unsigned long long)ph[k]);
            for (int k = 0; k < 4; ++k) atomicAdd(S.tcount + TC_ALL + 5 + k, (unsigned long long)lanes[k]);
            atomicAdd(S.tcount + TC_ALL + 9, (unsigned long long)ph[5]);
        }
#endif
    }
#undef LUMO_PHASE
    flush_counters(Cc, S.tcount);
    flush_counters(Cs, S.tcount + TC_N);
    if (LUMO_SKIP_DEAD) flush_resolved(Cs.resolved, S.tcount + TC_RESOLVED);
}

template <int STK, bool TOP>
__global__ __launch_bounds__(TOP ? TOP_BLOCK : BLOCK) void k_trace(DScene sc0, const double* o, const double* d,
                                                                 const int32_t* light, int n, int any_hit,
                                                                 double* t_out, int32_t* kind_out, int32_t* obj_out,
                                                                 int32_t* prim_out, unsigned long long* tcount) {
    extern __shared__ __attribute__((aligned(16))) char lds_scene[];
    if (n <= (int)(blockIdx.x * blockDim.x)) return;
    const DScene sc = TOP ? stage_top_lds(sc0, lds_scene) : sc0;
    Counters C{0, 0, 0};
    for (int i = blockIdx.x * blockDim.x + threadIdx.x; i < n; i += gridDim.x * blockDim.x) {
        const RayX r = rayx(Ray{ldv3(o, i), ldv3(d, i)});
        if (!any_hit) {
            const HitRef h = scene_hit<STK, true, TOP>(sc, r, C);
            t_out[i] = h.t;
            kind_out[i] = h.kind;
            obj_out[i] = h.obj;
            prim_out[i] = h.tri;
        } else {
            DHit lh;
            const int li = light[i];
            const bool vis = scene_hit_light<STK, true, TOP>(sc, r, li, lh, C);
            t_out[i] = vis ? lh.t : DINF;
            kind_out[i] = vis ? 2 : 0;
            obj_out[i] = vis ? li : -1;
            prim_out[i] = -1;
        }
    }
    flush_counters(C, tcount);
}

}
}
```

lumo_amd/csrc/device/upload.hip:

```cpp
#include <hip/hip_runtime.h>

#include <algorithm>
#include <cmath>
#include <cstdio>
#include <cstring>
#include <deque>
#include <vector>

#include "../host/wbvh.h"
#include "ctx.h"
#include "launch.h"

using namespace lumo;
using namespace lumo::dev;

extern "C" {

lumo_status lumo_scene_upload(void* ctx, const lumo_scene_desc* d) {
    Ctx* c = static_cast<Ctx*>(ctx);
    if (!c || !d) return LUMO_ERR_INVALID;
    if (d->num_lights <= 0 || d->num_light_nodes <= 0 || d->num_dense_spectra < 3 || !d->materials) return LUMO_ERR_INVALID;
    for (int i = 0; i < d->num_materials; ++i) {
        const lumo_material& m = d->materials[i];
        if (m.kind < LUMO_MAT_BLANK || m.kind > LUMO_MAT_MF_DIELECTRIC) return LUMO_ERR_UNSUPPORTED;
        if (m.kind >= LUMO_MAT_MF_DIFFUSE &&
            (m.eta_idx < 0 || m.eta_idx >= d->num_dense_spectra || m.k_idx < 0 || m.k_idx >= d->num_dense_spectra ||
             !(m.roughness > 0.0 && m.roughness <= 1.0)))
            return LUMO_ERR_INVALID;
        if (m.kind == LUMO_MAT_LIGHT && (m.illuminant < 0 || m.illuminant >= d->num_dense_spectra))
            return LUMO_ERR_INVALID;
        for (int t : {m.albedo_tex, m.ks_tex, m.tf_tex})
            if (t < -1 || t >= d->num_textures) return LUMO_ERR_INVALID;
        if (m.normal_map < -1 || m.normal_map >= d->num_normal_maps) return LUMO_ERR_INVALID;
    }
    for (int i = 0; i < d->num_textures; ++i) {
        const lumo_texture& t = d->textures[i];
        const bool ok = t.kind == LUMO_TEX_SOLID || t.kind == LUMO_TEX_MANDELBROT ||
                        (t.kind == LUMO_TEX_IMAGE && t.width > 0 && t.height > 0 && t.first >= 0 &&
                         (int64_t)t.first + (int64_t)t.width * t.height <= d->num_texels) ||
                        (t.kind == LUMO_TEX_CHECKERBOARD && t.first >= 0 && t.first < i && t.second >= 0 && t.second < i) ||
                        (t.kind == LUMO_TEX_MARBLE && t.first >= 0 && t.first < d->num_perlin);
        if (!ok) return LUMO_ERR_INVALID;
    }
    for (int i = 0; i < d->num_normal_maps; ++i) {
        const lumo_normal_map& n = d->normal_maps[i];
        if (!(n.width > 0 && n.height > 0 && n.first >= 0 &&
              (int64_t)n.first + (int64_t)n.width * n.height <= d->num_normal_texels))
            return LUMO_ERR_INVALID;
    }
    for (int i = 0; i < d->num_lights + d->num_objects; ++i) {
        const lumo_object& o = i < d->num_lights ? d->lights[i] : d->objects[i - d->num_lights];
        if (o.type < LUMO_OBJ_KDMESH || o.type > LUMO_OBJ_SPHERE) return LUMO_ERR_UNSUPPORTED;
        if (o.type == LUMO_OBJ_SPHERE && !(o.radius != 0.0 && o.area > 0.0)) return LUMO_ERR_INVALID;
        if (o.xform >= d->num_transforms || (o.xform >= 0 && !d->transforms)) return LUMO_ERR_INVALID;
        if (o.type == LUMO_OBJ_TRIANGLE && (o.tri_base < 0 || o.tri_base >= d->num_triangles)) return LUMO_ERR_INVALID;
    }
    HIPCHK(hipSetDevice(c->device));
    free_scene(*c);
    DScene& s = c->sc;
    lumo_status st = LUMO_OK;
    auto chk = [&](lumo_status x) {
        if (x && !st) st = x;
    };
    chk(upload(*c, d->vertices, (size_t)3 * d->num_vertices, &s.vertices));
    c->sort_lo = V3{0.0, 0.0, 0.0};
    c->sort_scale = V3{0.0, 0.0, 0.0};
    if (d->num_object_nodes > 0 && d->object_nodes) {
        const lumo_bvh_node& r = d->object_nodes[0];
        double lo[3], sc3[3];
        for (int a = 0; a < 3; ++a) {
            lo[a] = r.bmin[a];
            const double ext = r.bmax[a] - r.bmin[a];
            sc3[a] = ext > 0.0 && std::isfinite(ext) ? 8.0 / ext : 0.0;
        }
        c->sort_lo = V3{lo[0], lo[1], lo[2]};
        c->sort_scale = V3{sc3[0], sc3[1], sc3[2]};
    }
    chk(upload(*c, d->normals, (size_t)3 * d->num_normals, &s.normals));
    chk(upload(*c, d->uvs, (size_t)2 * d->num_uvs, &s.uvs));
    chk(upload(*c, d->triangles, (size_t)d->num_triangles, &s.tris));
    chk(upload(*c, d->kd_nodes, (size_t)d->num_kd_nodes, &s.kd));
    chk(upload(*c, d->kd_items, (size_t)d->num_kd_items, &s.kd_items));
    bool bvh_ok = true;
    auto escapes = [&](const lumo_bvh_node* nodes, int n, std::vector<DBvh>& out) {
        out.assign(n > 0 ? n : 0, DBvh{});
        if (n <= 0) return;
        std::vector<int32_t> esc(n, -1);
        for (int i = 0; i < n; ++i) {
            const lumo_bvh_node& b = nodes[i];
            if (b.count == 0) {
                if (i + 1 >= n || (b.right >= n)) {
                    bvh_ok = false;
                    return;
                }
                esc[i + 1] = b.right >= 0 ? b.right : esc[i];
                if (b.right >= 0) esc[b.right] = esc[i];
            }
        }
        std::vector<int32_t> order, at(n, -1);
        order.reserve(n);
        order.push_back(0);
        at[0] = 0;
        for (size_t h = 0; h < order.size(); ++h) {
            const int i = order[h];
            if (nodes[i].count != 0) continue;
            for (const int ch : {i + 1, nodes[i].right}) {
                if (ch < 0) continue;
                if (at[ch] >= 0) {
                    bvh_ok = false;
                    return;
                }
                at[ch] = (int32_t)order.size();
                order.push_back(ch);
            }
        }
        if ((int)order.size() != n) {
            bvh_ok = false;
            return;
        }
        for (int k = 0; k < n; ++k) {
            const int i = order[k];
            DBvh& o = out[k];
            for (int a = 0; a < 3; ++a) {
                o.bmin[a] = nodes[i].bmin[a];
                o.bmax[a] = nodes[i].bmax[a];
            }
            o.escape = esc[i] >= 0 ? at[esc[i]] : -1;
            o.left = nodes[i].count == 0 ? at[i + 1] : -1;
            o.first = nodes[i].first;
            o.count = nodes[i].count;
        }
    };
    std::vector<DBvh> obvh, lbvh;
    escapes(d->object_nodes, d->num_object_nodes, obvh);
    escapes(d->light_nodes, d->num_light_nodes, lbvh);
    if (!bvh_ok) {
        free_scene(*c);
        return LUMO_ERR_INVALID;
    }
    chk(upload(*c, obvh.data(), obvh.size(), &s.onodes));
    chk(upload(*c, d->object_items, (size_t)d->num_object_items, &s.oitems));
    chk(upload(*c, lbvh.data(), lbvh.size(), &s.lnodes));
    chk(upload(*c, d->light_items, (size_t)d->num_light_items, &s.litems));
    chk(upload(*c, d->alias_prob, (size_t)d->num_lights, &s.alias_prob));
    chk(upload(*c, d->alias_idx, (size_t)d->num_lights, &s.alias_idx));
    chk(upload(*c, d->alias_pdf, (size_t)d->num_lights, &s.alias_pdf));
    chk(upload(*c, d->materials, (size_t)d->num_materials, &s.mats));
    chk(upload(*c, d->dense_spectra, (size_t)95 * d->num_dense_spectra, &s.dense));
    chk(upload(*c, d->transforms, (size_t)d->num_transforms, &s.xforms));
    chk(upload(*c, d->textures, (size_t)d->num_textures, &s.textures));
    chk(upload(*c, d->texels, (size_t)d->num_texels, &s.texels));
    chk(upload(*c, d->normal_maps, (size_t)d->num_normal_maps, &s.nmaps));
    chk(upload(*c, d->normal_texels, (size_t)3 * d->num_normal_texels, &s.ntexels));
    chk(upload(*c, d->perlin, (size_t)d->num_perlin, &s.perlin));
    std::vector<double> tv((size_t)TV_STRIDE * d->num_triangles, 0.0);
    for (int i = 0; i < d->num_triangles; ++i)
        for (int k = 0; k < 3; ++k)
            for (int a = 0; a < 3; ++a) tv[(size_t)TV_STRIDE * i + 3 * k + a] = d->vertices[3 * d->triangles[i].v[k] + a];
    std::vector<int32_t> kd_new(d->num_kd_nodes, -1);
    std::vector<DKd> kdp;
    std::vector<std::pair<size_t, size_t>> kd_trees;
    {
        std::vector<int32_t> order;
        auto kid = [&](int i, int which) { return which == 0 ? i + 1 : d->kd_nodes[i].right; };
        auto valid = [&](int i) { return i >= 0 && i < d->num_kd_nodes; };
        auto place_tree = [&](int root) {
            if (!valid(root) || kd_new[root] >= 0) return;
            struct Extent {
                std::vector<std::pair<size_t, size_t>>& v;
                std::vector<int32_t>& o;
                size_t lo;
                ~Extent() { v.emplace_back(lo, o.size()); }
            } extent{kd_trees, order, order.size()};
            int size = 0;
            {
                std::vector<int32_t> st{root};
                while (!st.empty() && size <= 8) {
                    const int i = st.back();
                    st.pop_back();
                    size++;
                    if (!d->kd_nodes[i].leaf) {
                        for (int w = 0; w < 2; ++w)
                            if (valid(kid(i, w))) st.push_back(kid(i, w));
                    }
                }
            }
            std::deque<int32_t> groups{root};
            while (!groups.empty()) {
                const int g = groups.front();
                groups.pop_front();
                if (size > 8)
                    while (order.size() % 8) order.push_back(-1);
                std::deque<int32_t> bfs{g};
                int used = 0;
                while (!bfs.empty()) {
                    const int i = bfs.front();
                    bfs.pop_front();
                    if (used == 8) {
                        groups.push_back(i);
                        continue;
                    }
                    kd_new[i] = (int32_t)order.size();
                    order.push_back(i);
                    used++;
                    if (!d->kd_nodes[i].leaf)
                        for (int w = 0; w < 2; ++w)
                            if (valid(kid(i, w)) && kd_new[kid(i, w)] < 0) bfs.push_back(kid(i, w));
                }
            }
        };
        for (int i = 0; i < d->num_objects; ++i)
            if (d->objects[i].type == LUMO_OBJ_KDMESH || d->objects[i].type == LUMO_OBJ_RECTANGLE) place_tree(d->objects[i].kd_root);
        for (int i = 0; i < d->num_lights; ++i)
            if (d->lights[i].type == LUMO_OBJ_KDMESH || d->lights[i].type == LUMO_OBJ_RECTANGLE) place_tree(d->lights[i].kd_root);
        kdp.assign(order.size(), DKd{});
        for (size_t j = 0; j < order.size(); ++j) {
            const int i = order[j];
            if (i < 0) continue;
            const lumo_kd_node& n = d->kd_nodes[i];
            DKd k{};
            if (n.leaf) {
                k.u.leaf.first = n.first;
                k.u.leaf.count = n.count;
                k.meta = 3;
                k.left = -1;
            } else {
                if (!valid(n.right) || !valid(i + 1) || n.axis < 0 || n.axis > 2 || kd_new[n.right] >= (1 << 29))
                    chk(LUMO_ERR_INVALID);
                k.u.point = n.point;
                k.meta = (kd_new[n.right] << 2) | n.axis;
                k.left = kd_new[i + 1];
            }
            kdp[j] = k;
        }
    }
    auto relaid = [&](const lumo_object* src, int n) {
        std::vector<lumo_object> v(src, src + n);
        for (lumo_object& o : v)
            if ((o.type == LUMO_OBJ_KDMESH || o.type == LUMO_OBJ_RECTANGLE) && o.kd_root >= 0 &&
                o.kd_root < d->num_kd_nodes)
                o.kd_root = kd_new[o.kd_root];
        return v;
    };
    const std::vector<lumo_object> objs_dev = relaid(d->objects, d->num_objects);
    const std::vector<lumo_object> lights_dev = relaid(d->lights, d->num_lights);
    auto trav_view = [](const std::vector<lumo_object>& v) {
        std::vector<DObj> t(v.size());
        for (size_t i = 0; i < v.size(); ++i) {
            const lumo_object& o = v[i];
            DObj& x = t[i];
            for (int a = 0; a < 3; ++a) {
                x.bmin[a] = o.bmin[a];
                x.bmax[a] = o.bmax[a];
            }
            if (o.type == LUMO_OBJ_SPHERE) x.bmin[0] = o.radius;
            x.kd_root = o.kd_root;
            x.tri_base = o.tri_base;
            x.item_base = o.item_base;
            x.tx = ((o.xform + 1) << 2) | o.type;
        }
        return t;
    };
    const std::vector<DObj> tobjs = trav_view(objs_dev), tlights = trav_view(lights_dev);
    chk(upload(*c, objs_dev.data(), objs_dev.size(), &s.objs));
    chk(upload(*c, lights_dev.data(), lights_dev.size(), &s.lights));
    chk(upload(*c, tobjs.data(), tobjs.size(), &s.tobjs));
    chk(upload(*c, tlights.data(), tlights.size(), &s.tlights));
    chk(upload(*c, tv.data(), tv.size(), &s.tv));
    chk(upload(*c, kdp.data(), kdp.size(), &s.kdp));
    wbvh::Accel acc;
    s.accel = 0;
    s.w_oroot = s.w_lroot = wbvh::NONE;
    s.wnodes = s.wnodes_lds = nullptr;
    s.wtv = nullptr;
    s.w_oblas = s.w_lblas = nullptr;
    s.wn_lds = s.top_wnodes = 0;
    s.w_maxabs = 0.0;
    s.off_top_wnodes = 0;
    s.off_wnodes = s.off_wtv = s.off_woblas = s.off_wlblas = 0;
    c->w_nodes = c->w_tris = c->w_stack = c->w_depth = 0;
    if (c->o.accel && !st) {
        acc = wbvh::build_accel(*d);
        if (acc.ok) {
            s.accel = 1;
            s.w_oroot = acc.obj_root;
            s.w_lroot = acc.light_root;
            s.w_maxabs = (double)acc.max_abs;
            chk(upload(*c, acc.nodes.data(), acc.nodes.size(), &s.wnodes));
            chk(upload(*c, acc.tv.data(), acc.tv.size(), &s.wtv));
            chk(upload(*c, acc.obj_blas.data(), acc.obj_blas.size(), &s.w_oblas));
            chk(upload(*c, acc.light_blas.data(), acc.light_blas.size(), &s.w_lblas));
            c->w_nodes = (int)acc.nodes.size();
            c->w_tris = (int)(acc.tv.size() / wbvh::TV);
            c->w_stack = acc.max_stack;
            c->w_depth = acc.depth;
        } else {
            fprintf(stderr, "lumo_amd: the wide accel refused this scene (a light kd tree deeper than %d or a "
                    "walk stack of %d); walking lumo's structures\n", WL_STK, acc.max_stack);
        }
    }
    if (st) {
        free_scene(*c);
        return st;
    }
    s.n_onodes = d->num_object_nodes;
    s.n_lnodes = d->num_light_nodes;
    s.n_lights = d->num_lights;
    s.n_objs = d->num_objects;
    {
        std::vector<char> hot;
        auto put = [&](const void* p, size_t bytes) -> uint32_t {
            const size_t off = (hot.size() + 15) & ~(size_t)15;
            hot.resize(off + ((bytes + 15) & ~(size_t)15), 0);
            if (bytes) std::memcpy(hot.data() + off, p, bytes);
            return (uint32_t)off;
        };
        s.off_onodes = put(obvh.data(), sizeof(DBvh) * obvh.size());
        s.off_oitems = put(d->object_items, sizeof(int32_t) * d->num_object_items);
        s.off_lnodes = put(lbvh.data(), sizeof(DBvh) * lbvh.size());
        s.off_litems = put(d->light_items, sizeof(int32_t) * d->num_light_items);
        s.off_objs = put(objs_dev.data(), sizeof(lumo_object) * objs_dev.size());
        s.off_lights = put(lights_dev.data(), sizeof(lumo_object) * lights_dev.size());
        s.off_kdp = put(kdp.data(), sizeof(DKd) * kdp.size());
        s.off_kd_items = put(d->kd_items, sizeof(int32_t) * d->num_kd_items);
        s.off_tris = put(d->triangles, sizeof(lumo_triangle) * d->num_triangles);
        s.off_tv = put(tv.data(), sizeof(double) * tv.size());
        s.off_xforms = put(d->transforms, sizeof(lumo_transform) * d->num_transforms);
        s.off_tobjs = put(tobjs.data(), sizeof(DObj) * tobjs.size());
        s.off_tlights = put(tlights.data(), sizeof(DObj) * tlights.size());
        if (s.accel) {
            s.off_wnodes = put(acc.nodes.data(), sizeof(wbvh::Node) * acc.nodes.size());
            s.off_wtv = put(acc.tv.data(), sizeof(double) * acc.tv.size());
            s.off_woblas = put(acc.obj_blas.data(), sizeof(int32_t) * acc.obj_blas.size());
            s.off_wlblas = put(acc.light_blas.data(), sizeof(int32_t) * acc.light_blas.size());
        }
        s.hot_bytes = 0;
        if (hot.size() <= 48 * 1024) {
            const char* dp = nullptr;
            chk(upload(*c, hot.data(), hot.size(), &dp));
            if (st) {
                free_scene(*c);
                return st;
            }
            s.hot = dp;
            s.hot_bytes = (uint32_t)hot.size();
        }
    }
    {
        s.top = nullptr;
        s.top_bytes = 0;
        s.top_onodes = s.top_lnodes = 0;
        s.onodes_lds = s.lnodes_lds = nullptr;
        s.n_onodes_lds = s.n_lnodes_lds = 0;
        const size_t cap = std::min((size_t)c->o.top_kb * 1024, c->lds_cu);
        const size_t budget = cap > 256 ? cap - 256 : 0;
        const size_t objs_b = ((sizeof(int32_t) * d->num_object_items + 15) & ~(size_t)15) + sizeof(DObj) * tobjs.size();
        const size_t wobjs_b = ((sizeof(DObj) * tobjs.size() + 15) & ~(size_t)15);
        if (s.accel && s.hot_bytes == 0 && budget >= 4096 && wobjs_b + 16 * sizeof(wbvh::Node) <= budget) {
            std::vector<char> top;
            auto put = [&](const void* p, size_t bytes) -> uint32_t {
                const size_t off = (top.size() + 15) & ~(size_t)15;
                top.resize(off + ((bytes + 15) & ~(size_t)15), 0);
                if (bytes) std::memcpy(top.data() + off, p, bytes);
                return (uint32_t)off;
            };
            s.off_top_oitems = 0;
            s.off_top_tobjs = put(tobjs.data(), sizeof(DObj) * tobjs.size());
            const size_t left = budget - top.size();
            const size_t nw = std::min(acc.nodes.size(), left / sizeof(wbvh::Node));
            s.off_top_wnodes = put(acc.nodes.data(), sizeof(wbvh::Node) * nw);
            s.top_wnodes = (int32_t)nw;
            s.top_onodes = s.top_lnodes = 0;
            s.off_top_onodes = s.off_top_lnodes = 0;
            s.kst_cfg = 0;
            s.top_kd_lo = s.top_kd_n = 0;
            s.off_top_kd = 0;
            const char* dp = nullptr;
            chk(upload(*c, top.data(), top.size(), &dp));
            if (st) {
                free_scene(*c);
                return st;
            }
            s.top = dp;
            s.top_bytes = (uint32_t)top.size();
        } else if (!s.accel && s.hot_bytes == 0 && budget >= 4096 && objs_b + 64 * sizeof(DBvh) <= budget) {
            std::vector<char> top;
            auto put = [&](const void* p, size_t bytes) -> uint32_t {
                const size_t off = (top.size() + 15) & ~(size_t)15;
                top.resize(off + ((bytes + 15) & ~(size_t)15), 0);
                if (bytes) std::memcpy(top.data() + off, p, bytes);
                return (uint32_t)off;
            };
            s.off_top_oitems = put(d->object_items, sizeof(int32_t) * d->num_object_items);
            s.off_top_tobjs = put(tobjs.data(), sizeof(DObj) * tobjs.size());
            size_t left = budget - top.size();
            const size_t no = std::min(obvh.size(), left / sizeof(DBvh));
            s.off_top_onodes = put(obvh.data(), sizeof(DBvh) * no);
            left = budget - top.size();
            const size_t nl = std::min(lbvh.size(), left / sizeof(DBvh));
            s.off_top_lnodes = put(lbvh.data(), sizeof(DBvh) * nl);
            s.top_onodes = (int32_t)no;
            s.top_lnodes = (int32_t)nl;
            const size_t aligned = (top.size() + 15) & ~(size_t)15;
            const size_t lim = std::min(cap, c->lds_block);
            size_t room = lim > aligned + 256 ? lim - aligned - 256 : 0;
            s.kst_cfg = c->o.kd_lds > 0 ? (int32_t)std::min<size_t>((size_t)c->o.kd_lds, room / (12 * (size_t)TOP_BLOCK)) : 0;
            room -= 12 * (size_t)TOP_BLOCK * s.kst_cfg;
            s.top_kd_lo = s.top_kd_n = 0;
            s.off_top_kd = 0;
            size_t big = 0, big_lo = 0;
            for (const auto& tr : kd_trees)
                if (tr.second - tr.first > big) {
                    big = tr.second - tr.first;
                    big_lo = tr.first;
                }
            if (c->o.top_kd && big > 8 && room >= 16 * 64 + 16) {
                const size_t nk = std::min(big, (room - 16) / sizeof(DKd));
                s.off_top_kd = put(kdp.data() + big_lo, sizeof(DKd) * nk);
                s.top_kd_lo = (int32_t)big_lo;
                s.top_kd_n = (int32_t)nk;
            }
            const char* dp = nullptr;
            chk(upload(*c, top.data(), top.size(), &dp));
            if (st) {
                free_scene(*c);
                return st;
            }
            s.top = dp;
            s.top_bytes = (uint32_t)top.size();
        } else {
            s.kst_cfg = 0;
            s.top_kd_lo = s.top_kd_n = 0;
            s.off_top_kd = 0;
        }
        s.kst_n = 0;
        s.top_shm = ((s.top_bytes + 15u) & ~15u) + (uint32_t)(12 * (size_t)TOP_BLOCK * s.kst_cfg);
    }
    int n = d->num_lights, lg = 0;
    while (n > 1) {
        n >>= 1;
        lg++;
    }
    s.n_shadow = lg > 1 ? lg : 1;
    auto bvh_need = [&](const lumo_bvh_node* nodes, int n) {
        std::vector<int> pend(n > 0 ? n : 1, 0);
        int mx = 0;
        for (int i = 0; i < n; ++i) {
            if (nodes[i].count == 0) {
                const int p = pend[i] + (nodes[i].right >= 0 ? 1 : 0);
                if (i + 1 < n) pend[i + 1] = std::max(pend[i + 1], p);
                if (nodes[i].right >= 0 && nodes[i].right < n) pend[nodes[i].right] = std::max(pend[nodes[i].right], pend[i]);
                mx = std::max(mx, p);
            }
        }
        return mx;
    };
    const int need_b = std::max({1, bvh_need(d->object_nodes, d->num_object_nodes),
                                 bvh_need(d->light_nodes, d->num_light_nodes)});
    int need_k = 1;
    {
        std::vector<int> depth(d->num_kd_nodes > 0 ? d->num_kd_nodes : 1, 0);
        for (int i = 0; i < d->num_kd_nodes; ++i) {
            if (!d->kd_nodes[i].leaf) {
                if (i + 1 < d->num_kd_nodes) depth[i + 1] = std::max(depth[i + 1], depth[i] + 1);
                const int r = d->kd_nodes[i].right;
                if (r >= 0 && r < d->num_kd_nodes) depth[r] = std::max(depth[r], depth[i] + 1);
                need_k = std::max(need_k, depth[i] + 1);
            }
        }
    }
    if (need_b > 64 || need_k > 64) {
        free_scene(*c);
        return LUMO_ERR_UNSUPPORTED;
    }
    auto fits = [&](int cls) { return cls >= need_k; };
    s.stack_class = 64;
    for (int cls : STACK_CLASSES)
        if (fits(cls)) {
            s.stack_class = cls;
            break;
        }
    if (c->o.stack_class > 0 && fits(c->o.stack_class)) s.stack_class = c->o.stack_class;
    if (s.accel) s.stack_class = 0;
    bool full = d->num_transforms > 0;
    for (int i = 0; i < d->num_materials; ++i)
        full = full || (d->materials[i].kind != LUMO_MAT_LAMBERTIAN && d->materials[i].kind != LUMO_MAT_LIGHT &&
                        d->materials[i].kind != LUMO_MAT_BLANK);
    for (int i = 0; i < d->num_objects; ++i)
        full = full || (d->objects[i].type != LUMO_OBJ_KDMESH && d->objects[i].type != LUMO_OBJ_RECTANGLE);
    for (int i = 0; i < d->num_lights; ++i) full = full || d->lights[i].type != LUMO_OBJ_RECTANGLE;
    bool textured = false;
    for (int i = 0; i < d->num_materials; ++i) {
        const lumo_material& m = d->materials[i];
        textured = textured || m.albedo_tex >= 0 || m.ks_tex >= 0 || m.tf_tex >= 0 || m.normal_map >= 0;
    }
    full = full || c->o.full_kernels != 0;
    s.full = textured ? 2 : (full ? 1 : 0);
    c->has_scene = true;
    return LUMO_OK;
}

lumo_status lumo_camera_set(void* ctx, const lumo_camera_desc* d) {
    Ctx* c = static_cast<Ctx*>(ctx);
    if (!c || !d) return LUMO_ERR_INVALID;
    if (d->orthographic != 0 && d->orthographic != 1) return LUMO_ERR_INVALID;
    if (d->width <= 0 || d->height <= 0 || !(d->filter_radius > 0.0) || !(d->filter_sigma > 0.0)) return LUMO_ERR_INVALID;
    auto get = [](const double (&a)[2][16]) {
        Xform x;
        M4* ms[2] = {&x.m, &x.inv};
        for (int q = 0; q < 2; ++q) {
            V4* rows[4] = {&ms[q]->y0, &ms[q]->y1, &ms[q]->y2, &ms[q]->y3};
            for (int r = 0; r < 4; ++r) *rows[r] = V4{a[q][4 * r], a[q][4 * r + 1], a[q][4 * r + 2], a[q][4 * r + 3]};
        }
        return x;
    };
    auto m3 = [](const double* a) { return M3{V3{a[0], a[1], a[2]}, V3{a[3], a[4], a[5]}, V3{a[6], a[7], a[8]}}; };
    c->cam.wtc = get(d->world_to_camera);
    c->cam.sctr = get(d->screen_to_raster);
    c->cam.cts = get(d->camera_to_screen);
    c->cam.lens_radius = d->lens_radius;
    c->cam.focal_length = d->focal_length;
    c->cam.wb = m3(d->white_balance);
    c->cam.x2r = m3(d->xyz_to_rgb);
    c->cam.fr = d->filter_radius;
    c->cam.fsig = d->filter_sigma;
    c->cam.width = (double)d->width;
    c->cam.height = (double)d->height;
    c->cam.orthographic = d->orthographic;
    {
        const DCam& k = c->cam;
        V3 p_min3 = xf_pt_inv(k.sctr, V3{0.0, 0.0, 0.0});
        V3 p_max3 = xf_pt_inv(k.sctr, V3{k.width, k.height, 0.0});
        p_min3 = xf_pt_inv(k.cts, p_min3);
        p_max3 = xf_pt_inv(k.cts, p_max3);
        const V2 p_min = V2{p_min3.x, p_min3.y} / (p_min3.z == 0.0 ? 1.0 : p_min3.z);
        const V2 p_max = V2{p_max3.x, p_max3.y} / (p_max3.z == 0.0 ? 1.0 : p_max3.z);
        const V2 pd = p_max - p_min;
        c->cam.image_plane_area = fabs(pd.x * pd.y);
    }
    if ((uint64_t)std::ceil(d->filter_radius - 0.5) != 1) return LUMO_ERR_UNSUPPORTED;
    c->has_camera = true;
    return LUMO_OK;
}

lumo_status lumo_scene_info(void* ctx, lumo_scene_info_t* info) {
    Ctx* c = static_cast<Ctx*>(ctx);
    if (!c || !info) return LUMO_ERR_INVALID;
    if (!c->has_scene) return LUMO_ERR_NO_SCENE;
    info->stack_class = c->sc.stack_class;
    info->lds_bytes = c->o.lds ? (int32_t)c->sc.hot_bytes : 0;
    info->full_kernels = c->sc.full;
    info->n_shadow = c->sc.n_shadow;
    const bool top = c->o.top && c->sc.top_bytes > 0 && !(c->o.lds && c->sc.hot_bytes > 0);
    info->top_bytes = top ? (int32_t)c->sc.top_bytes : 0;
    info->top_object_nodes = c->sc.top_onodes;
    info->top_light_nodes = c->sc.top_lnodes;
    info->top_kd_nodes = top ? c->sc.top_kd_n : 0;
    info->top_shm = top ? (int32_t)c->sc.top_shm : 0;
    info->accel = c->sc.accel;
    info->wide_nodes = c->w_nodes;
    info->wide_tris = c->w_tris;
    info->wide_stack = c->w_stack;
    info->wide_depth = c->w_depth;
    info->top_wide_nodes = top ? c->sc.top_wnodes : 0;
    return LUMO_OK;
}

}
```

Measured before the change: 4921.

## Reuse BVH leaf slab, kd winner error bounds and barycentrics to skip recomputation

BVH leaves holding a single untransformed kd-mesh or rectangle whose bounds equal the leaf's are flagged at upload, so kd traversal reuses the leaf's slab interval instead of recomputing the object box test. The kd traversal also keeps the winning triangle's error bound and edge/determinant values. This avoids re-running the full triangle intersection for the winner and lets hit records be built from the stored barycentrics. It costs extra live registers during traversal and adds template paths that could raise register pressure and lower occupancy.

```diff
diff --git a/lumo_amd/csrc/device/dscene.h b/lumo_amd/csrc/device/dscene.h
--- a/lumo_amd/csrc/device/dscene.h
+++ b/lumo_amd/csrc/device/dscene.h
@@ -10,9 +10,20 @@
 #ifndef LUMO_WHILE_WHILE
 #define LUMO_WHILE_WHILE 1
 #endif
+#ifndef LUMO_REUSE_SLAB
+#define LUMO_REUSE_SLAB 1
+#endif
+#ifndef LUMO_REUSE_ACCEPT
+#define LUMO_REUSE_ACCEPT 1
+#endif
+#ifndef LUMO_REUSE_RECORD
+#define LUMO_REUSE_RECORD 1
+#endif
 
 namespace lumo {
 namespace dev {
+
+constexpr int RM_REC = LUMO_REUSE_ACCEPT ? (LUMO_REUSE_RECORD ? 2 : 1) : 0;
 
 constexpr double DINF = __builtin_huge_val();
 constexpr int NS = 4;
@@ -35,6 +46,7 @@
     double bmin[3], bmax[3];
     int32_t escape, first, count, left;
 };
+constexpr int32_t BVH_SAME_BOX = 1 << 30;
 
 struct DObj {
     double bmin[3], bmax[3];
@@ -449,35 +461,15 @@
     te = min_element(vmax(ro_max, ro_min)) * (1.0 + 2.0 * gamma_n(3));
 }
 
-__device__ __forceinline__ double tri_hit_t_at(const double* tv, const RayX& r, double t_min, double t_max,
-                                               Counters& C) {
+struct TriAcc {
+    V3 e;
+    double det;
+};
+
+template <bool DT, bool ACC>
+__device__ __forceinline__ bool tri_test_at(const double* tv, const RayX& r, double t_min, double t_max, Counters& C,
+                                            double& t_out, TriAcc& acc, double& delta_t) {
     C.tri++;
-    const V3 A = ld3(tv), B = ld3(tv + 3), Cv = ld3(tv + 6);
-    const int kz = r.kz;
-    const V3 wi = r.wi;
-    V3 at = perm_kz(kz, A - r.o), bt = perm_kz(kz, B - r.o), ct = perm_kz(kz, Cv - r.o);
-    const V3 shear = r.shear;
-    at = at + shear * at.z;
-    bt = bt + shear * bt.z;
-    ct = ct + shear * ct.z;
-    const V3 e = V3{bt.x * ct.y - bt.y * ct.x, ct.x * at.y - ct.y * at.x, at.x * bt.y - at.y * bt.x};
-    if (min_element(e) < 0.0 && max_element(e) > 0.0) return DINF;
-    const double det = dot(e, V3{1.0, 1.0, 1.0});
-    if (det == 0.0) return DINF;
-    const double t_scaled = dot(e, V3{at.z, bt.z, ct.z}) / wi.z;
-    const bool b1 = det < 0.0 && (t_scaled > t_min * det || t_scaled < t_max * det);
-    const bool b2 = det > 0.0 && (t_scaled < t_min * det || t_scaled > t_max * det);
-    if (b1 || b2) return DINF;
-    return t_scaled / det;
-}
-__device__ __forceinline__ double tri_hit_t(const DScene& sc, int ti, const RayX& r, double t_min, double t_max,
-                                            Counters& C) {
-    return tri_hit_t_at(sc.tv + TV_STRIDE * ti, r, t_min, t_max, C);
-}
-
-template <bool FULL>
-__device__ bool tri_hit_geo_at(const DScene& sc, const double* tv, int ti, const RayX& r, double t_min, double t_max,
-                               DHit& out) {
     const V3 A = ld3(tv), B = ld3(tv + 3), Cv = ld3(tv + 6);
     const int kz = r.kz;
     const V3 wi = r.wi;
@@ -494,20 +486,36 @@
     const bool b1 = det < 0.0 && (t_scaled > t_min * det || t_scaled < t_max * det);
     const bool b2 = det > 0.0 && (t_scaled < t_min * det || t_scaled > t_max * det);
     if (b1 || b2) return false;
-    const double t = t_scaled / det;
-    const double max_z_v = rmax(rmax(fabs(at.z), fabs(bt.z)), fabs(ct.z));
-    const double delta_z = gamma_n(3) * max_z_v;
-    const double max_y_v = rmax(rmax(fabs(at.y), fabs(bt.y)), fabs(ct.y));
-    const double delta_y = gamma_n(5) * (max_y_v + max_z_v);
-    const double max_x_v = rmax(rmax(fabs(at.x), fabs(bt.x)), fabs(ct.x));
-    const double delta_x = gamma_n(5) * (max_x_v + max_z_v);
-    const double delta_e = 2.0 * (gamma_n(2) * max_x_v * max_y_v + delta_y * max_x_v + delta_x * max_y_v);
-    const double max_e = rmax(rmax(fabs(e.x), fabs(e.y)), fabs(e.z));
-    const double delta_t = 3.0 * (gamma_n(3) * max_e * max_z_v + delta_e * max_z_v + delta_z * max_e) / fabs(det);
-    if (t <= t_min + delta_t) return false;
-    out.t = t;
-    if (!FULL) return true;
-    const V3 bary = e / det;
+    t_out = t_scaled / det;
+    if constexpr (DT) {
+        const double max_z_v = rmax(rmax(fabs(at.z), fabs(bt.z)), fabs(ct.z));
+        const double delta_z = gamma_n(3) * max_z_v;
+        const double max_y_v = rmax(rmax(fabs(at.y), fabs(bt.y)), fabs(ct.y));
+        const double delta_y = gamma_n(5) * (max_y_v + max_z_v);
+        const double max_x_v = rmax(rmax(fabs(at.x), fabs(bt.x)), fabs(ct.x));
+        const double delta_x = gamma_n(5) * (max_x_v + max_z_v);
+        const double delta_e = 2.0 * (gamma_n(2) * max_x_v * max_y_v + delta_y * max_x_v + delta_x * max_y_v);
+        const double max_e = rmax(rmax(fabs(e.x), fabs(e.y)), fabs(e.z));
+        delta_t = 3.0 * (gamma_n(3) * max_e * max_z_v + delta_e * max_z_v + delta_z * max_e) / fabs(det);
+    }
+    if constexpr (ACC) acc = TriAcc{e, det};
+    return true;
+}
+__device__ __forceinline__ double tri_hit_t_at(const double* tv, const RayX& r, double t_min, double t_max,
+                                               Counters& C) {
+    double t, dt;
+    TriAcc a;
+    return tri_test_at<false, false>(tv, r, t_min, t_max, C, t, a, dt) ? t : DINF;
+}
+__device__ __forceinline__ double tri_hit_t(const DScene& sc, int ti, const RayX& r, double t_min, double t_max,
+                                            Counters& C) {
+    return tri_hit_t_at(sc.tv + TV_STRIDE * ti, r, t_min, t_max, C);
+}
+
+__device__ __forceinline__ void tri_record_at(const DScene& sc, const double* tv, int ti, const TriAcc& acc, double t,
+                                              V3 d, DHit& out) {
+    const V3 A = ld3(tv), B = ld3(tv + 3), Cv = ld3(tv + 6);
+    const V3 bary = acc.e / acc.det;
     const lumo_triangle T = sc.tris[ti];
     const V3 ng = normalize(cross(B - A, Cv - A));
     V3 ns = ng;
@@ -527,11 +535,26 @@
                               dot(vabs(bary * V3{A.z, B.z, Cv.z}), V3{1, 1, 1})};
     out.t = t;
     out.material = T.material;
-    out.backface = dot(r.d, ng) > 0.0;
+    out.backface = dot(d, ng) > 0.0;
     out.p = xi;
     out.ns = ns;
     out.ng = ng;
     out.uv = wrap_uv(uv);
+}
+__device__ void tri_record(const DScene& sc, int ti, const TriAcc& acc, double t, V3 d, DHit& out) {
+    tri_record_at(sc, sc.tv + TV_STRIDE * ti, ti, acc, t, d, out);
+}
+
+template <bool FULL>
+__device__ bool tri_hit_geo_at(const DScene& sc, const double* tv, int ti, const RayX& r, double t_min, double t_max,
+                               DHit& out) {
+    Counters uncounted{0, 0, 0, 0};
+    double t, delta_t;
+    TriAcc acc;
+    if (!tri_test_at<true, FULL>(tv, r, t_min, t_max, uncounted, t, acc, delta_t)) return false;
+    if (t <= t_min + delta_t) return false;
+    out.t = t;
+    if constexpr (FULL) tri_record_at(sc, tv, ti, acc, t, r.d, out);
     return true;
 }
 template <bool FULL>
@@ -573,9 +596,15 @@
     return sc.kdp[i];
 }
 
-template <bool GEO, int STK, bool KL = false>
+struct KdWin {
+    int idx;
+    double delta_t;
+    TriAcc acc;
+};
+template <bool GEO, int STK, bool KL = false, int RM = 0>
 __device__ KD_INLINE double kd_traverse(const DScene& sc, const DObj& ob, const RayX& r, double t_min, double t_max,
-                              int* idx_out, Counters& C) {
+                              KdWin* win, Counters& C, bool have_box = false, double box_ts = 0.0,
+                              double box_te = 0.0) {
     const double origin[3] = {r.o.x, r.o.y, r.o.z};
     const double inv_dir[3] = {r.inv.x, r.inv.y, r.inv.z};
     int st_node[STK];
@@ -584,10 +613,16 @@
     double t_hit = DINF;
     int curr = ob.kd_root;
     int idx = -1;
-    double ts, te;
+    double win_dt = 0.0;
+    TriAcc win_acc{V3{0.0, 0.0, 0.0}, 0.0};
     C.aabb++;
-    slab(ob.bmin, ob.bmax, r.o, r.inv, ts, te);
-    double t_start = rmax(ts, t_min), t_end = rmin(te, t_max);
+    double t_start = box_ts, t_end = box_te;
+    if (!(LUMO_REUSE_SLAB && have_box)) {
+        double ts, te;
+        slab(ob.bmin, ob.bmax, r.o, r.inv, ts, te);
+        t_start = rmax(ts, t_min);
+        t_end = rmin(te, t_max);
+    }
     const double t_end0 = t_end;
     for (;;) {
         if (t_hit < t_start) break;
@@ -620,12 +655,17 @@
             const int first = node.u.leaf.first, count = node.u.leaf.count;
             for (int k = 0; k < count; ++k) {
                 const int i = sc.kd_items[ob.item_base + first + k];
-                const double t = tri_hit_t(sc, ob.tri_base + i, r, t_min, t_end, C);
+                double t = DINF, dt = 0.0;
+                TriAcc a{V3{0.0, 0.0, 0.0}, 0.0};
+                if (!tri_test_at<GEO && RM >= 1, GEO && RM == 2>(sc.tv + TV_STRIDE * (ob.tri_base + i), r, t_min, t_end, C, t, a, dt))
+                    t = DINF;
                 if (GEO) {
                     if (t < t_end) {
                         t_end = t;
                         t_hit = t;
                         idx = i;
+                        if (RM >= 1) win_dt = dt;
+                        if (RM == 2) win_acc = a;
                     }
                 } else if (t < t_end) {
                     return t;
@@ -658,7 +698,7 @@
         }
     }
     if (GEO) {
-        *idx_out = idx;
+        *win = KdWin{idx, win_dt, win_acc};
         return idx < 0 ? DINF : t_hit;
     }
     return DINF;
@@ -709,8 +749,8 @@
     const double d0 = a.lo / b.lo, d1 = a.lo / b.hi, d2 = a.hi / b.lo, d3 = a.hi / b.hi;
     return EF{a.v / b.v, previous_float(rmin(rmin(rmin(d0, d1), d2), d3)), next_float(rmax(rmax(rmax(d0, d1), d2), d3))};
 }
-template <bool FULL, class OB>
-__device__ bool sphere_hit(const OB& ob, const RayX& r, double t_min, double t_max, DHit& out) {
+template <bool FULL, class OB, class RY>
+__device__ bool sphere_hit(const OB& ob, const RY& r, double t_min, double t_max, DHit& out) {
     const double radius = obj_radius(ob);
     const EF dx = ef(r.d.x), dy = ef(r.d.y), dz = ef(r.d.z), ox = ef(r.o.x), oy = ef(r.o.y), oz = ef(r.o.z);
     const EF radius2 = ef_mul(ef(radius), ef(radius));
@@ -775,48 +815,90 @@
 
 template <int STK, int FX, bool KL = false>
 __device__ __forceinline__ double shape_hit_t(const DScene& sc, const DObj& ob, const RayX& r, double t_min,
-                                              double t_max, Counters& C) {
+                                              double t_max, Counters& C, bool have_box = false, double box_ts = 0.0,
+                                              double box_te = 0.0) {
     if constexpr (FX) {
         if (ob.type() == LUMO_OBJ_TRIANGLE) return tri_hit_t(sc, ob.tri_base, r, t_min, t_max, C);
         if (ob.type() == LUMO_OBJ_SPHERE) return sphere_hit_t(ob, r, t_min, t_max);
     }
-    return kd_traverse<false, STK, KL>(sc, ob, r, t_min, t_max, nullptr, C);
+    return kd_traverse<false, STK, KL>(sc, ob, r, t_min, t_max, nullptr, C, have_box, box_ts, box_te);
 }
 template <int STK, int FX, bool KL = false>
 __device__ __forceinline__ double object_hit_t(const DScene& sc, const DObj& ob, const RayX& r, double t_min,
-                                               double t_max, Counters& C) {
+                                               double t_max, Counters& C, bool have_box = false, double box_ts = 0.0,
+                                               double box_te = 0.0) {
     if constexpr (FX) {
         if (ob.xform() >= 0)
             return shape_hit_t<STK, FX, KL>(sc, ob, ray_local(sc.xforms[ob.xform()], r), t_min, t_max, C);
     }
-    return shape_hit_t<STK, FX, KL>(sc, ob, r, t_min, t_max, C);
-}
-
-template <int STK, int FX, bool KL = false>
+    return shape_hit_t<STK, FX, KL>(sc, ob, r, t_min, t_max, C, have_box, box_ts, box_te);
+}
+
+template <int STK, int FX, bool KL = false, int RM = 0>
 __device__ __forceinline__ int shape_hit_tri(const DScene& sc, const DObj& ob, const RayX& r, double t_min,
-                                             double t_max, Counters& C, DHit& out) {
+                                             double t_max, Counters& C, double& t_out, TriAcc& acc) {
     if constexpr (FX) {
         if (ob.type() == LUMO_OBJ_TRIANGLE) {
-            C.tri++;
-            return tri_hit_geo<false>(sc, ob.tri_base, r, t_min, t_max, out) ? ob.tri_base : -1;
+            double t, dt;
+            TriAcc a;
+            if (!tri_test_at<true, RM == 2>(sc.tv + TV_STRIDE * ob.tri_base, r, t_min, t_max, C, t, a, dt)) return -1;
+            if (t <= t_min + dt) return -1;
+            t_out = t;
+            if (RM == 2) acc = a;
+            return ob.tri_base;
         }
-        if (ob.type() == LUMO_OBJ_SPHERE) return sphere_hit<false>(ob, r, t_min, t_max, out) ? PRIM_SPHERE : -1;
-    }
-    int idx = -1;
-    kd_traverse<true, STK, KL>(sc, ob, r, t_min, t_max, &idx, C);
-    if (idx < 0) return -1;
+        if (ob.type() == LUMO_OBJ_SPHERE) {
+            DHit g;
+            if (!sphere_hit<false>(ob, r, t_min, t_max, g)) return -1;
+            t_out = g.t;
+            return PRIM_SPHERE;
+        }
+    }
+    KdWin w;
+    const double t = kd_traverse<true, STK, KL, RM>(sc, ob, r, t_min, t_max, &w, C);
+    if (w.idx < 0) return -1;
     C.tri++;
-    if (!tri_hit_geo<false>(sc, ob.tri_base + idx, r, t_min, t_max, out)) return -1;
-    return ob.tri_base + idx;
-}
-template <int STK, int FX, bool KL = false>
+    if constexpr (RM == 0) {
+        DHit g;
+        if (!tri_hit_geo<false>(sc, ob.tri_base + w.idx, r, t_min, t_max, g)) return -1;
+        t_out = g.t;
+        return ob.tri_base + w.idx;
+    }
+    if (t <= t_min + w.delta_t) return -1;
+    t_out = t;
+    if (RM == 2) acc = w.acc;
+    return ob.tri_base + w.idx;
+}
+template <int STK, int FX, bool KL = false, int RM = 0>
 __device__ __forceinline__ int object_hit_tri(const DScene& sc, const DObj& ob, const RayX& r, double t_min,
-                                              double t_max, Counters& C, DHit& out) {
+                                              double t_max, Counters& C, double& t_out, TriAcc& acc) {
     if constexpr (FX) {
         if (ob.xform() >= 0)
-            return shape_hit_tri<STK, FX, KL>(sc, ob, ray_local(sc.xforms[ob.xform()], r), t_min, t_max, C, out);
-    }
-    return shape_hit_tri<STK, FX, KL>(sc, ob, r, t_min, t_max, C, out);
+            return shape_hit_tri<STK, FX, KL, RM>(sc, ob, ray_local(sc.xforms[ob.xform()], r), t_min, t_max, C,
+                                                  t_out, acc);
+    }
+    return shape_hit_tri<STK, FX, KL, RM>(sc, ob, r, t_min, t_max, C, t_out, acc);
+}
+
+template <int FX>
+__device__ void object_record_acc(const DScene& sc, const lumo_object& ob, int tri, const Ray& r, double t,
+                                  const TriAcc& acc, DHit& h) {
+    if constexpr (!FX) {
+        tri_record(sc, tri, acc, t, r.d, h);
+        if (ob.type == LUMO_OBJ_RECTANGLE) h.uv = wrap_uv(V2{dot(ld3(ob.b0), h.p), dot(ld3(ob.b1), h.p)});
+    } else {
+        Ray rl = r;
+        if (ob.xform >= 0) {
+            const lumo_transform& T = sc.xforms[ob.xform];
+            rl = Ray{xf_apply(T.inv, r.o, 1.0), xf_apply(T.inv, r.d, 0.0)};
+        }
+        if (ob.type == LUMO_OBJ_SPHERE)
+            sphere_hit<true>(ob, rl, 0.0, DINF, h);
+        else
+            tri_record(sc, tri, acc, t, rl.d, h);
+        if (ob.type == LUMO_OBJ_RECTANGLE) h.uv = wrap_uv(V2{dot(ld3(ob.b0), h.p), dot(ld3(ob.b1), h.p)});
+        if (ob.xform >= 0) instance_fix_hit(sc.xforms[ob.xform], ob.material_override, h);
+    }
 }
 
 template <int FX>
@@ -835,7 +917,7 @@
     }
 }
 
-template <bool GEO, int STK, int FX, bool TOP = false>
+template <bool GEO, int STK, int FX, bool TOP = false, bool SLAB = false>
 __device__ int bvh_traverse(const DScene& sc, const DBvh* nodes, int n_nodes, const int32_t* items,
                             const DObj* objs, const RayX& r, double t_min, double t_max, Counters& C,
                             double* t_found = nullptr, const DBvh* nodes_lds = nullptr, int n_lds = 0) {
@@ -846,9 +928,9 @@
 #if LUMO_WHILE_WHILE
     for (;;) {
         int count = 0;
+        double ts = 0.0, te = 0.0;
         while (curr >= 0) {
             const DBvh& node = (TOP && curr < n_lds) ? nodes_lds[curr] : nodes[curr];
-            double ts, te;
             C.aabb++;
             slab(node.bmin, node.bmax, r.o, inv_dir, ts, te);
             ts = rmax(ts, t_min);
@@ -875,15 +957,17 @@
         ts = rmax(ts, t_min);
         te = rmin(te, tt);
         if (ts <= te) {
-            const int count = node.count;
+            int count = node.count;
             if (count == 0) {
                 curr = node.left;
                 continue;
             }
 #endif
+            const bool same_box = LUMO_REUSE_SLAB && SLAB && (count & BVH_SAME_BOX) != 0;
+            count &= ~BVH_SAME_BOX;
             for (int k = 0; k < count; ++k) {
                 const int i = items[node.first + k];
-                const double t = object_hit_t<STK, FX, TOP>(sc, objs[i], r, t_min, tt, C);
+                const double t = object_hit_t<STK, FX, TOP>(sc, objs[i], r, t_min, tt, C, same_box, ts, te);
                 if (GEO) {
                     if (t < tt) {
                         tt = t;
@@ -900,12 +984,12 @@
     return idx;
 }
 
-template <int STK, int FX, bool TOP = false>
+template <int STK, int FX, bool TOP = false, bool SLAB = false>
 __device__ __forceinline__ double bvh_hit_t(const DScene& sc, const DBvh* nodes, int n, const int32_t* items,
                                             const DObj* objs, const RayX& r, double t_min, double t_max,
                                             Counters& C, const DBvh* nodes_lds = nullptr, int n_lds = 0) {
     double t = DINF;
-    const int idx = bvh_traverse<false, STK, FX, TOP>(sc, nodes, n, items, objs, r, t_min, t_max, C, &t, nodes_lds, n_lds);
+    const int idx = bvh_traverse<false, STK, FX, TOP, SLAB>(sc, nodes, n, items, objs, r, t_min, t_max, C, &t, nodes_lds, n_lds);
     if (idx < 0) return DINF;
     return t;
 }
@@ -1180,31 +1264,39 @@
     if (wide_walk<true, FX, TOP, OC>(sc, sc.w_oroot, sc.tobjs, sc.w_oblas, r, 0.0, t_max, C).t < t_max) return true;
     return wide_walk<true, FX, TOP, OC>(sc, sc.w_lroot, sc.tlights, sc.w_lblas, r, 0.0, t_max, C).t < t_max;
 }
-template <int STK, int FX, bool TOP = false, bool OC = false>
-__device__ HitRef scene_hit(const DScene& sc, const RayX& r, Counters& C) {
+template <int STK, int FX, bool TOP = false, bool OC = false, int RM = 0>
+__device__ HitRef scene_hit(const DScene& sc, const RayX& r, Counters& C, TriAcc& acc) {
     if constexpr (STK == 0) {
         return wide_scene_hit<FX, TOP, OC>(sc, r, C);
     } else {
     HitRef h{DINF, 0, -1, -1};
     double t_max = DINF;
-    DHit g;
-    int oi = bvh_traverse<true, STK, FX, TOP>(sc, sc.onodes, sc.n_onodes, sc.oitems, sc.tobjs, r, 0.0, t_max, C, nullptr,
+    double gt = DINF;
+    TriAcc ga{V3{0.0, 0.0, 0.0}, 0.0};
+    int oi = bvh_traverse<true, STK, FX, TOP, RM != 0>(sc, sc.onodes, sc.n_onodes, sc.oitems, sc.tobjs, r, 0.0, t_max, C, nullptr,
                                               sc.onodes_lds, sc.n_onodes_lds);
     if (oi >= 0) {
-        const int tri = object_hit_tri<STK, FX, TOP>(sc, sc.tobjs[oi], r, 0.0, t_max, C, g);
+        const int tri = object_hit_tri<STK, FX, TOP, RM>(sc, sc.tobjs[oi], r, 0.0, t_max, C, gt, ga);
         if (tri != -1) {
-            h = HitRef{g.t, 1, oi, tri};
-            t_max = g.t;
+            h = HitRef{gt, 1, oi, tri};
+            t_max = gt;
         }
     }
-    const int li = bvh_traverse<true, STK, FX, TOP>(sc, sc.lnodes, sc.n_lnodes, sc.litems, sc.tlights, r, 0.0, t_max, C,
+    const int li = bvh_traverse<true, STK, FX, TOP, RM != 0>(sc, sc.lnodes, sc.n_lnodes, sc.litems, sc.tlights, r, 0.0, t_max, C,
                                                     nullptr, sc.lnodes_lds, sc.n_lnodes_lds);
     if (li >= 0) {
-        const int tri = object_hit_tri<STK, FX, TOP>(sc, sc.tlights[li], r, 0.0, t_max, C, g);
-        if (tri != -1) h = HitRef{g.t, 2, li, tri};
-    }
+        const int tri = object_hit_tri<STK, FX, TOP, RM>(sc, sc.tlights[li], r, 0.0, t_max, C, gt, ga);
+        if (tri != -1) h = HitRef{gt, 2, li, tri};
+    }
+    if (RM == 2) acc = ga;
     return h;
     }
+}
+
+template <int STK, int FX, bool TOP = false, bool OC = false>
+__device__ __forceinline__ HitRef scene_hit(const DScene& sc, const RayX& r, Counters& C) {
+    TriAcc unused;
+    return scene_hit<STK, FX, TOP, OC, 0>(sc, r, C, unused);
 }
 
 template <int FX>
@@ -1212,40 +1304,52 @@
     const lumo_object& ob = hr.kind == 1 ? sc.objs[hr.obj] : sc.lights[hr.obj];
     object_record<FX>(sc, ob, hr.tri, r, h);
 }
-
-template <int STK, int FX, bool TOP = false>
+template <int FX>
+__device__ __forceinline__ void hit_record_acc(const DScene& sc, const HitRef& hr, const TriAcc& acc, const Ray& r,
+                                               DHit& h) {
+    const lumo_object& ob = hr.kind == 1 ? sc.objs[hr.obj] : sc.lights[hr.obj];
+    object_record_acc<FX>(sc, ob, hr.tri, r, hr.t, acc, h);
+}
+
+template <int STK, int FX, bool TOP = false, int RM = 0>
 __device__ bool scene_hit_light(const DScene& sc, const RayX& r, int light, DHit& lh, Counters& C) {
+    double t = DINF;
+    TriAcc acc{V3{0.0, 0.0, 0.0}, 0.0};
     if constexpr (STK == 0) {
-        const int tri = object_hit_tri<kd_stk<STK>(), FX, false>(sc, sc.tlights[light], r, 0.0, DINF, C, lh);
-        if (tri == -1 || wide_occluded<FX, TOP>(sc, r, lh.t - EPSILON, C)) return false;
+        const int tri = object_hit_tri<kd_stk<STK>(), FX, false>(sc, sc.tlights[light], r, 0.0, DINF, C, t, acc);
+        if (tri == -1 || wide_occluded<FX, TOP>(sc, r, t - EPSILON, C)) return false;
         object_record<FX>(sc, sc.lights[light], tri, r, lh);
         return true;
     } else {
-    const int tri = object_hit_tri<STK, FX, TOP>(sc, sc.tlights[light], r, 0.0, DINF, C, lh);
+    const int tri = object_hit_tri<STK, FX, TOP, RM>(sc, sc.tlights[light], r, 0.0, DINF, C, t, acc);
     if (tri == -1) return false;
-    const double t_max = lh.t - EPSILON;
-    if (bvh_hit_t<STK, FX, TOP>(sc, sc.onodes, sc.n_onodes, sc.oitems, sc.tobjs, r, 0.0, t_max, C, sc.onodes_lds,
+    const double t_max = t - EPSILON;
+    if (bvh_hit_t<STK, FX, TOP, RM != 0>(sc, sc.onodes, sc.n_onodes, sc.oitems, sc.tobjs, r, 0.0, t_max, C, sc.onodes_lds,
                                 sc.n_onodes_lds) < t_max)
         return false;
-    if (bvh_hit_t<STK, FX, TOP>(sc, sc.lnodes, sc.n_lnodes, sc.litems, sc.tlights, r, 0.0, t_max, C, sc.lnodes_lds,
+    if (bvh_hit_t<STK, FX, TOP, RM != 0>(sc, sc.lnodes, sc.n_lnodes, sc.litems, sc.tlights, r, 0.0, t_max, C, sc.lnodes_lds,
                                 sc.n_lnodes_lds) < t_max)
         return false;
-    object_record<FX>(sc, sc.lights[light], tri, r, lh);
+    if constexpr (RM == 2)
+        object_record_acc<FX>(sc, sc.lights[light], tri, Ray{r.o, r.d}, t, acc, lh);
+    else
+        object_record<FX>(sc, sc.lights[light], tri, r, lh);
     return true;
     }
 }
 
 template <int STK, int FX, bool TOP = false, bool OC = false>
 __device__ int scene_hit_light_tri(const DScene& sc, const RayX& r, int light, Counters& C) {
-    DHit lh;
+    double t = DINF;
+    TriAcc acc;
     if constexpr (STK == 0) {
-        const int tri = object_hit_tri<kd_stk<STK>(), FX, false>(sc, sc.tlights[light], r, 0.0, DINF, C, lh);
-        if (tri == -1 || wide_occluded<FX, TOP, OC>(sc, r, lh.t - EPSILON, C)) return -1;
+        const int tri = object_hit_tri<kd_stk<STK>(), FX, false>(sc, sc.tlights[light], r, 0.0, DINF, C, t, acc);
+        if (tri == -1 || wide_occluded<FX, TOP, OC>(sc, r, t - EPSILON, C)) return -1;
         return tri;
     } else {
-    const int tri = object_hit_tri<STK, FX, TOP>(sc, sc.tlights[light], r, 0.0, DINF, C, lh);
+    const int tri = object_hit_tri<STK, FX, TOP, 0>(sc, sc.tlights[light], r, 0.0, DINF, C, t, acc);
     if (tri == -1) return -1;
-    const double t_max = lh.t - EPSILON;
+    const double t_max = t - EPSILON;
     if (bvh_hit_t<STK, FX, TOP>(sc, sc.onodes, sc.n_onodes, sc.oitems, sc.tobjs, r, 0.0, t_max, C, sc.onodes_lds,
                                 sc.n_onodes_lds) < t_max)
         return -1;
diff --git a/lumo_amd/csrc/device/pt.h b/lumo_amd/csrc/device/pt.h
--- a/lumo_amd/csrc/device/pt.h
+++ b/lumo_amd/csrc/device/pt.h
@@ -518,6 +518,9 @@
 #endif
 
 
+template <int FX>
+constexpr int RM_BOUNCE = FX == 0 ? RM_REC : 0;
+
 struct NeeRec {
     Ray ray;
     DColor f;
@@ -542,7 +545,7 @@
     const RayX ri = rayx(R.ray);
     DHit hi;
     DColor out = cfill(0.0);
-    if (scene_hit_light<STK, FX>(sc, ri, li, hi, C)) {
+    if (scene_hit_light<STK, FX, false, RM_BOUNCE<FX>>(sc, ri, li, hi, C)) {
         const lumo_object& Lo = sc.lights[li];
         const double p_lig = light_pdf<FX>(sc, Lo, ri, hi.p, hi.ng);
         const double p_sct = R.pdf;
@@ -570,7 +573,7 @@
     const RayX ri = rayx(ray);
     DHit hi;
     DColor out = cfill(0.0);
-    if (scene_hit_light<STK, FX>(sc, ri, li, hi, C)) {
+    if (scene_hit_light<STK, FX, false, RM_BOUNCE<FX>>(sc, ri, li, hi, C)) {
         const lumo_object& Lo = sc.lights[li];
         const double p_lig = light_pdf<FX>(sc, Lo, ri, hi.p, hi.ng);
         const double p_sct = pdf;
@@ -604,11 +607,15 @@
 __device__ __forceinline__ bool bounce_path(const DScene& sc, const double* delta, PathReg& P, Counters& Cc,
                                             Counters& Cs) {
     const RayX rx = rayx(P.ro);
-    const HitRef hr = scene_hit<STK, FX>(sc, rx, Cc);
+    TriAcc acc{V3{0.0, 0.0, 0.0}, 0.0};
+    const HitRef hr = scene_hit<STK, FX, false, false, RM_BOUNCE<FX>>(sc, rx, Cc, acc);
     P.queries += 1u;
     if (hr.kind == 0) return false;
     DHit ho;
-    hit_record<FX>(sc, hr, rx, ho);
+    if constexpr (STK == 0 || RM_BOUNCE<FX> != 2)
+        hit_record<FX>(sc, hr, rx, ho);
+    else
+        hit_record_acc<FX>(sc, hr, acc, P.ro, ho);
     const lumo_material m = sc.mats[ho.material];
     const V3 wo = -P.ro.d;
     const double rand_u = xs_float(P.rng);
@@ -753,7 +760,10 @@
             const bool live = q < count;
             LUMO_PHASE(3);
             HitRef hr{DINF, 0, -1, -1};
-            if (live) hr = scene_hit<STK, FX>(sc, rayx(Ray{qv3(cur, QD_O, q), qv3(cur, QD_D, q)}), Cc);
+            TriAcc hacc{V3{0.0, 0.0, 0.0}, 0.0};
+            if (live)
+                hr = scene_hit<STK, FX, false, false, RM_BOUNCE<FX>>(sc, rayx(Ray{qv3(cur, QD_O, q), qv3(cur, QD_D, q)}), Cc,
+                                                                hacc);
             LUMO_PHASE(0);
             PathReg P{};
             bool resolve = false, alive = false, ok = false;
@@ -767,7 +777,10 @@
                 P.queries += 1u;
                 if (hr.kind != 0) {
                     DHit ho;
-                    hit_record<FX>(sc, hr, rayx(P.ro), ho);
+                    if constexpr (STK == 0 || RM_BOUNCE<FX> != 2)
+                        hit_record<FX>(sc, hr, rayx(P.ro), ho);
+                    else
+                        hit_record_acc<FX>(sc, hr, hacc, P.ro, ho);
                     const lumo_material m = sc.mats[ho.material];
                     const V3 wo = -P.ro.d;
                     const double rand_u = xs_float(P.rng);
@@ -917,7 +930,8 @@
     for (int i = blockIdx.x * blockDim.x + threadIdx.x; i < n; i += gridDim.x * blockDim.x) {
         const RayX r = rayx(Ray{ldv3(o, i), ldv3(d, i)});
         if (!any_hit) {
-            const HitRef h = scene_hit<STK, true, TOP>(sc, r, C);
+            TriAcc acc;
+            const HitRef h = scene_hit<STK, true, TOP, false, RM_REC>(sc, r, C, acc);
             t_out[i] = h.t;
             kind_out[i] = h.kind;
             obj_out[i] = h.obj;
@@ -925,7 +939,7 @@
         } else {
             DHit lh;
             const int li = light[i];
-            const bool vis = scene_hit_light<STK, true, TOP>(sc, r, li, lh, C);
+            const bool vis = scene_hit_light<STK, true, TOP, RM_REC>(sc, r, li, lh, C);
             t_out[i] = vis ? lh.t : DINF;
             kind_out[i] = vis ? 2 : 0;
             obj_out[i] = vis ? li : -1;
diff --git a/lumo_amd/csrc/device/upload.hip b/lumo_amd/csrc/device/upload.hip
--- a/lumo_amd/csrc/device/upload.hip
+++ b/lumo_amd/csrc/device/upload.hip
@@ -82,7 +82,8 @@
     chk(upload(*c, d->kd_nodes, (size_t)d->num_kd_nodes, &s.kd));
     chk(upload(*c, d->kd_items, (size_t)d->num_kd_items, &s.kd_items));
     bool bvh_ok = true;
-    auto escapes = [&](const lumo_bvh_node* nodes, int n, std::vector<DBvh>& out) {
+    auto escapes = [&](const lumo_bvh_node* nodes, int n, const int32_t* items, int n_items, const lumo_object* objs,
+                       int n_objs, std::vector<DBvh>& out) {
         out.assign(n > 0 ? n : 0, DBvh{});
         if (n <= 0) return;
         std::vector<int32_t> esc(n, -1);
@@ -129,11 +130,17 @@
             o.left = nodes[i].count == 0 ? at[i + 1] : -1;
             o.first = nodes[i].first;
             o.count = nodes[i].count;
+            if (o.count == 1 && o.first >= 0 && o.first < n_items && items[o.first] >= 0 && items[o.first] < n_objs) {
+                const lumo_object& ob = objs[items[o.first]];
+                if ((ob.type == LUMO_OBJ_KDMESH || ob.type == LUMO_OBJ_RECTANGLE) && ob.xform < 0 &&
+                    std::memcmp(ob.bmin, o.bmin, sizeof(o.bmin)) == 0 && std::memcmp(ob.bmax, o.bmax, sizeof(o.bmax)) == 0)
+                    o.count |= BVH_SAME_BOX;
+            }
         }
     };
     std::vector<DBvh> obvh, lbvh;
-    escapes(d->object_nodes, d->num_object_nodes, obvh);
-    escapes(d->light_nodes, d->num_light_nodes, lbvh);
+    escapes(d->object_nodes, d->num_object_nodes, d->object_items, d->num_object_items, d->objects, d->num_objects, obvh);
+    escapes(d->light_nodes, d->num_light_nodes, d->light_items, d->num_light_items, d->lights, d->num_lights, lbvh);
     if (!bvh_ok) {
         free_scene(*c);
         return LUMO_ERR_INVALID;
```

After: 5159 (median of 6 runs). 4.8% higher.
